# XuyangBai/D3Feat

Measured on AMD Instinct MI355X. Metric: fragments/sec (30k-pt clouds), higher is better.
Workload: dtype f32; 1 GPU; SURVEY §8d config #2: synthetic 3DMatch room fragment, 300k raw pts -> grid subsample 0.03 m (~29k pts per cloud) -> self-pair -> 5-level pyramid -> full KPFCNN forward (random-init weights (reference initialiser, seed 42), 14.1M params)...; points_per_cloud=29369, fragments_per_gpu=2141, parallelism=fragment-dp1, fragments_per_replay=12, engine_fallbacks=0, engine_isolated_replays=0

## Files before the change

### d3feat_amd/_lib.py

```python
import ctypes as C
import os

_HERE = os.path.dirname(os.path.abspath(__file__))
LIB_PATH = os.environ.get("D3FEAT_AMD_LIB") or os.path.join(_HERE, "lib", "libd3feat_amd.so")

D3F_OK = 0
ERRORS = {-1: "HIP runtime / kernel launch failure", -2: "workspace too small", -3: "invalid argument"}
ST_EMPTY_ELEMENT, ST_NEG_CELL, ST_KEY_RANGE, ST_HIT_OVERFLOW, ST_OUT_OVERFLOW, ST_KEY_WIDTH = 1, 2, 4, 8, 16, 32
PAD_NUM_SUPPORTS = -2147483648
NEIGHBOR_CAP = 1024
MAX_BATCH = 255
TOPK_MAX = 8192
PAIRS_KMAX = 1024
REPEAT_COUNTS_MAX = 16
MATCH_KMAX = 8192
VALIDATION_NMAX = 1024
SCENES_MAX = 256
GRID_RESET_MAX = 8
VP_INDEX_RANGE, VP_COUNT_RANGE = 1, 2

_vp, _sz, _i, _f = C.c_void_p, C.c_size_t, C.c_int, C.c_float

SIGNATURES = {
    "d3f_version": (_i, []),
    "d3f_trace_marker": (_i, [_i, _vp]),
    "d3f_pack_status": (_i, [_vp, _vp, _i, _vp, _i, _vp, _i, _vp, _i, _vp, _i, _i, _i, _vp]),
    "d3f_grid_subsample_workspace_bytes": (_sz, [_i, _i, _i, _i]),
    "d3f_batch_grid_subsample": (_i, [_vp, _i, _vp, _i, _f, _vp, _i, _vp, _i, _vp, _vp, _vp, _vp, _vp, _vp, _sz, _vp]),
    "d3f_batch_grid_subsample_async": (_i, [_vp, _i, _vp, _i, _f, _vp, _i, _i, _i, _vp, _vp, _vp, _sz, _vp]),
    "d3f_batch_grid_subsample_async_inplace": (_i, [_vp, _i, _vp, _i, _f, _vp, _i, _i, _vp, _vp, _vp, _sz, _vp]),
    "d3f_stack_self_pair": (_i, [_vp, _i, _vp, _i, _vp, _vp, _vp, _vp]),
    "d3f_radius_neighbors_workspace_bytes": (_sz, [_i, _i, _i]),
    "d3f_batch_radius_neighbors": (_i, [_vp, _i, _vp, _i, _vp, _vp, _i, _f, _vp, _i, _i, _i, _vp, _vp, _sz, _vp]),
    "d3f_neighbor_grid_bytes": (_sz, [_i, _i]),
    "d3f_neighbor_grid_order_offset": (_sz, [_i, _i]),
    "d3f_neighbor_grid_build": (_i, [_vp, _i, _vp, _i, _f, _vp, _sz, _vp]),
    "d3f_neighbor_grid_boxed_form": (_i, [_i, _i]),
    "d3f_geometry_reset": (_i, [_vp, _i, _vp, _vp, _vp, _vp, _i, _vp]),
    "d3f_neighbor_grid_build_boxed": (_i, [_vp, _i, _vp, _i, _f, _vp, _vp, _sz, _vp]),
    "d3f_stack_self_pair_boxed": (_i, [_vp, _i, _vp, _i, _vp, _vp, _vp, _vp, _vp, _vp]),
    "d3f_batch_grid_subsample_async_boxed": (_i, [_vp, _vp, _i, _vp, _i, _f, _vp, _i, _i, _i, _vp, _vp, _vp, _vp, _vp, _sz, _vp]),
    "d3f_neighbor_grid_search": (_i, [_vp, _sz, _i, _vp, _i, _vp, _i, _f, _i, _vp, _i, _i, _i, _i, _i, _f, _i, _vp, _vp]),
    "d3f_neighbor_grid_search_ordered": (_i, [_vp, _sz, _i, _vp, _i, _vp, _i, _f, _vp, _sz, _vp, _i, _i, _i, _i, _i, _f, _i, _vp, _vp]),
    "d3f_neighbor_grid_inv_offset": (_sz, [_i, _i]),
    "d3f_neighbor_grid_xyz_offset": (_sz, [_i, _i]),
    "d3f_row_positive": (_i, [_vp, _i, _i, _i, _vp, _vp, _i, _vp]),
    "d3f_kpconv_aggregate": (_i, [_vp, _i, _vp, _i, _vp, _i, _i, _vp, _i, _i, _vp, _vp, _i, _f, _i, _i, _vp, _vp, _vp, _vp,
                                  _vp, _i, _vp]),
    "d3f_kpconv_deform_aggregate": (_i, [_vp, _i, _vp, _i, _vp, _i, _i, _vp, _i, _i, _vp, _i, _f, _vp, _i, _i, _vp, _i, _f, _i, _i, _vp,
                                         _vp, _vp, _vp, _i, _vp]),
    "d3f_kpconv_fused_c1": (_i, [_vp, _i, _vp, _i, _vp, _i, _i, _vp, _i, _vp, _i, _f, _i, _i, _vp, _i, _vp, _vp, _vp, _i, _i,
                                 _f, _vp, _i, _vp, _vp, _vp, _i, _vp]),
    "d3f_kpconv_fused32": (_i, [_vp, _i, _vp, _i, _vp, _i, _i, _vp, _i, _vp, _vp, _i, _f, _i, _i, _vp, _vp, _vp, _vp, _i, _i, _f, _vp,
                                _i, _vp, _vp, _vp, _i, _vp]),
    "d3f_kpconv_fused_supported": (_i, [_i, _i, _i, _i, _i]),
    "d3f_kpconv_pack_weights": (_i, [_vp, _i, _i, _vp, _vp]),
    "d3f_kpconv_fused": (_i, [_vp, _i, _vp, _i, _vp, _i, _i, _vp, _i, _i, _vp, _vp, _i, _f, _i, _i, _vp, _i, _vp, _vp, _vp, _i, _i,
                              _f, _vp, _i, _vp, _vp, _vp, _i, _vp]),
    "d3f_kpconv_fused32_x3": (_i, [_vp, _i, _vp, _i, _vp, _i, _i, _vp, _i, _vp, _vp, _i, _f, _i, _i, _vp, _vp, _vp, _vp, _i, _i, _f, _vp,
                                   _i, _vp, _vp, _vp, _i, _vp]),
    "d3f_kpconv_packed_x3_bytes": (_sz, [_i, _i]),
    "d3f_kpconv_pack_weights_x3": (_i, [_vp, _i, _i, _vp, _vp]),
    "d3f_kpconv_fused_x3": (_i, [_vp, _i, _vp, _i, _vp, _i, _i, _vp, _i, _i, _vp, _vp, _i, _f, _i, _i, _vp, _i, _vp, _vp, _vp, _i, _i,
                                 _f, _vp, _i, _vp, _vp, _vp, _i, _vp]),
    "d3f_gemm_workspace_bytes": (_sz, [_i, _i, _i, _i]),
    "d3f_gemm_bf16_workspace_bytes": (_sz, [_i, _i, _i, _i]),
    "d3f_gemm_f32": (_i, [_vp, _i, _vp, _i, _vp, _i, _i, _i, _i, _vp, _vp, _vp, _vp, _i, _i, _f, _vp, _sz, _vp, _i, _vp]),
    "d3f_gemm_upsample_cat_f32": (_i, [_vp, _i, _i, _i, _vp, _i, _vp, _i, _i, _vp, _i, _vp, _i, _i, _i, _vp, _vp, _i, _f, _vp, _sz,
                                       _vp, _vp, _i, _vp]),
    "d3f_ind_max_pool": (_i, [_vp, _i, _i, _i, _vp, _i, _i, _i, _vp, _i, _vp, _vp, _vp, _vp, _i, _vp]),
    "d3f_closest_pool_cat": (_i, [_vp, _i, _i, _i, _vp, _i, _i, _vp, _i, _i, _vp, _i, _vp, _vp, _vp]),
    "d3f_affine_act": (_i, [_vp, _i, _i, _i, _vp, _vp, _vp, _i, _i, _f, _vp, _i, _vp, _vp]),
    "d3f_pack_descriptors": (_i, [_vp, _vp, _i, _i, _vp, _i, _vp, _i, _vp, _vp]),
    "d3f_pack_descriptors_to": (_i, [_vp, _vp, _i, _i, _vp, _i, _vp, _i, _vp, _vp, _i, _i, _i, _vp, _vp, _vp]),
    "d3f_topk_workspace_bytes": (_sz, [_i, _i, _i, _i]),
    "d3f_topk_records": (_i, [_vp, _i, _vp, _i, _i, _vp, _i, _i, _vp, _vp, _i, _i, _i, _vp, _i, _i, _vp, _i, _vp, _vp, _vp, _vp, _sz,
                              _vp]),
    "d3f_feature_nn_workspace_bytes": (_sz, [_i]),
    "d3f_feature_nn": (_i, [_vp, _i, _i, _vp, _i, _i, _i, _vp, _vp, _vp, _sz, _vp]),
    "d3f_mutual_matches_workspace_bytes": (_sz, [_i]),
    "d3f_mutual_matches": (_i, [_vp, _i, _vp, _i, _vp, _vp, _vp, _sz, _vp]),
    "d3f_ransac_hypotheses": (_i, [_vp, _i, _vp, _i, _vp, _i, _f, _f, C.c_uint64, C.c_uint64, _i, _vp, _vp, _vp]),
    "d3f_ransac_draw": (_i, [C.c_uint64, C.c_uint64, _i, _i]),
    "d3f_neighbor_grid_score": (_i, [_vp, _sz, _i, _vp, _i, _vp, _i, _f, _vp, _vp, _vp, _vp]),
    "d3f_register_pairs_workspace_bytes": (_sz, [_i, _i, _i, _i]),
    "d3f_register_pairs": (_i, [_vp, _i, _i, _i, _i, _vp, _vp, _i, _i, _f, _i, _f, _f, _i, _i, C.c_uint64, _vp, _f] + [_vp] * 11
                           + [_sz, _vp]),
    "d3f_repeatability_pairs": (_i, [_vp, _i, _i, _i, _vp, _vp, _i, _vp, _i, _vp, _vp, _i, _vp, _vp, _vp]),
    "d3f_match_pairs_workspace_bytes": (_sz, [_i, _vp, _i]),
    "d3f_match_pairs": (_i, [_vp, _i, _i, _i, _i, _vp, _vp, _i, _vp, _f, _vp, _i, _vp, _vp, _vp, _sz, _vp]),
    "d3f_register_pairs_counts_workspace_bytes": (_sz, [_i, _i, _i, _vp, _i, _i]),
    "d3f_register_pairs_counts": (_i, [_vp, _i, _i, _i, _i, _vp, _vp, _i, _vp, _i, _f, _i, _f, _f, _i, _i, C.c_uint64, _vp, _f] + [_vp] * 10
                                  + [_sz, _vp]),
    "d3f_overlap_pairs": (_i, [_vp, _sz, _i, _i, _vp, _i, _f, _vp, _vp, _i, _vp]),
    "d3f_validation_pairs_workspace_bytes": (_sz, [_i, _i]),
    "d3f_validation_pairs": (_i, [_vp, _i, _i, _vp, _i, _vp, _i, _i, _vp, _vp, _vp, _i, _vp, _i, _f, _i, _f, _f, _f, _f] + [_vp] * 5
                             + [_sz, _vp]),
    "d3f_loss_gradients_workspace_bytes": (_sz, [_i, _i, _i]),
    "d3f_loss_gradients": (_i, [_vp, _i, _i, _vp, _i, _vp, _i, _i, _vp, _vp, _vp, _i, _vp, _i, _f, _i, _f, _f, _f, _f, _i, _vp, _i, _vp, _i,
                                _vp, _vp, _vp, _sz, _vp]),
    "d3f_neighbor_transpose_workspace_bytes": (_sz, [_i, _i]),
    "d3f_neighbor_transpose": (_i, [_vp, _i, _i, _i, _vp, _i, _vp, _vp, _vp, _sz, _vp]),
    "d3f_detect_head_backward_workspace_bytes": (_sz, [_i, _i, _i]),
    "d3f_detect_head_backward": (_i, [_vp, _i, _i, _i, _vp, _i, _i, _vp, _vp, _i, _i, _vp, _vp, _vp, _i, _vp, _i, _vp, _i, _vp, _sz, _vp]),
    "d3f_neighbor_transpose_qs": (_i, [_vp, _i, _i, _i, _vp, _i, _vp, _vp, _vp, _vp, _sz, _vp]),
    "d3f_kpconv_backward_workspace_bytes": (_sz, [_i, _i, _i, _i, _i, _i]),
    "d3f_kpconv_backward": (_i, [_vp, _i, _vp, _i, _vp, _i, _i, _vp, _i, _i, _vp, _i, _f, _i, _i, _vp, _vp, _i, _i, _vp, _vp, _vp, _i, _vp,
                                 _vp, _vp, _vp, _i, _vp, _sz, _vp]),
    "d3f_gemm_tn_workspace_bytes": (_sz, [_i, _i, _i]),
    "d3f_gemm_tn_f32": (_i, [_vp, _i, _vp, _i, _i, _i, _i, _vp, _vp, _vp, _sz, _vp]),
    "d3f_batch_norm_workspace_bytes": (_sz, [_i, _i]),
    "d3f_batch_norm_train": (_i, [_vp, _i, _i, _i, _vp, _vp, _f, _f, _vp, _vp, _vp, _i, _i, _f, _vp, _i, _vp, _vp, _vp, _vp, _sz, _vp]),
    "d3f_batch_norm_backward": (_i, [_vp, _i, _vp, _i, _vp, _i, _i, _i, _vp, _vp, _vp, _i, _f, _vp, _i, _vp, _vp, _vp, _i, _vp, _vp, _sz,
                                     _vp]),
    "d3f_pose_errors": (_i, [_vp, _vp, _i, _i, _vp, _vp, _vp, _vp, _vp, _vp]),
    "d3f_sanitize_descriptors": (_i, [_vp, _i, _i, _i, _i, _vp]),
    "d3f_matching_summary": (_i, [_vp, _vp, _vp, _i, _i, _vp, _i, _vp, _vp, _vp, _vp]),
    "d3f_registration_recall": (_i, [_vp, _i, _vp, _vp, _vp, _vp, _vp, _i, _i, _vp, _i, _vp, _vp, _vp, _vp, _vp]),
    "d3f_icp_pairs_workspace_bytes": (_sz, [_i, _i]),
    "d3f_icp_pairs": (_i, [_vp, _sz, _i, _vp, _i, _vp, _i, _vp, _vp, _i, _i] + [_vp] * 9 + [_sz, _vp]),
    "d3f_gemm_pack_bf16": (_i, [_vp, _i, _i, _i, _vp, _vp]),
    "d3f_gemm_pack_f32t": (_i, [_vp, _i, _i, _i, _vp, _vp]),
    "d3f_gemm_f32t": (_i, [_vp, _i, _i, _i, _vp, _i, _vp, _i, _i, _vp, _vp, _i, _i, _i, _vp, _vp, _vp, _vp, _i, _i, _f, _vp, _sz,
                           _vp, _vp, _i, _vp]),
    "d3f_gemm_x3_packed_bytes": (_sz, [_i, _i]),
    "d3f_gemm_pack_x3": (_i, [_vp, _i, _i, _i, _vp, _vp]),
    "d3f_gemm_x3_workspace_bytes": (_sz, [_i, _i, _i, _i]),
    "d3f_gemm_x3_plan": (_i, [_i, _i, _i, _i, _vp, _vp, _vp]),
    "d3f_gemm_x3_resident": (_i, [_i, _i, _i, _i]),
    "d3f_gemm_x3": (_i, [_vp, _i, _i, _i, _vp, _i, _vp, _i, _i, _vp, _vp, _i, _i, _i, _vp, _vp, _vp, _vp, _i, _i, _f, _vp, _sz,
                         _vp, _vp, _i, _vp]),
    "d3f_gemm_x3_gres": (_i, [_vp, _i, _i, _i, _vp, _i, _vp, _i, _i, _vp, _vp, _i, _i, _i, _vp, _vp, _vp, _vp, _i, _vp, _i, _i, _vp, _i, _f,
                              _vp, _sz, _vp, _vp, _i, _vp]),
    "d3f_gemm_bf16": (_i, [_vp, _i, _i, _i, _vp, _i, _vp, _i, _i, _vp, _vp, _i, _i, _i, _vp, _vp, _vp, _vp, _i, _i, _f, _vp, _sz,
                           _vp, _vp, _i, _i, _i, _vp]),
    "d3f_decode_xyz_records": (_i, [_vp, _i, _i, _i, _i, _i, _i, _i, _vp, _vp]),
    "d3f_detect_head": (_i, [_vp, _i, _i, _i, _vp, _i, _i, _vp, _vp, _i, _i, _vp, _i, _vp, _vp, _vp, _vp]),
}

_lib = None


class D3FeatLibraryError(RuntimeError):
    pass


def load():
    global _lib
    if _lib is not None:
        return _lib
    if not os.path.exists(LIB_PATH):
        raise D3FeatLibraryError(
            "d3feat_amd: %s not found -- the HIP extension is the only compute path. Build it with "
            "`python -c 'import __graft_entry__ as g; g.build()'` or `make -C d3feat_amd/csrc`." % LIB_PATH)
    lib = C.CDLL(LIB_PATH)
    for name, (res, args) in SIGNATURES.items():
        fn = getattr(lib, name)
        fn.restype = res
        fn.argtypes = args
    _lib = lib
    return lib


def check(rc, what):
    if rc != D3F_OK:
        raise D3FeatLibraryError("d3feat_amd.%s failed: %s (code %d)" % (what, ERRORS.get(rc, "unknown"), rc))
```

### d3feat_amd/csrc/gemm_f32.hip

```cpp
#include "gemm_common.h"
#include <cstdio>
#include <cstdlib>

#define GM_SA (GM_BK + 1)

template <int WM, int WN>
__global__ void __launch_bounds__(256)
gemm_f32_kernel(const float* __restrict__ A, int lda, const float* __restrict__ B, int ldb, float* __restrict__ C, int ldc,
                int M, int N, int K, int vecA, int vecB, int tiles_per_split, float* __restrict__ slab, GemmEpi E,
                const int* __restrict__ M_dev, GemmGather G) {
    constexpr int BM = 32 * WM, BN = 32 * WN;
    constexpr int A_F4 = BM * GM_BK / 4 / 256;
    constexpr int B_F4 = GM_BK * BN / 4 / 256;
    static_assert(WM * WN == 4 && A_F4 >= 1 && B_F4 >= 1, "tile shape");
    const int Mcap = M;
    M = d3f_dyn(M, M_dev);
    if ((int)(blockIdx.z * BM) >= M) return;
    __shared__ float As[2][BM * GM_SA];
    __shared__ __attribute__((aligned(16))) float Bs[2][GM_BK * BN];

    const int tid = threadIdx.x, lane = tid & 63, wave = tid >> 6;
    const int wm = wave / WN, wn = wave % WN;
    const int m0 = blockIdx.z * BM, n0 = blockIdx.x * BN;
    const int nt_all = (K + GM_BK - 1) / GM_BK;
// ... 352 lines not shown
            if (bn == 32) gemm_fast_kernel<4, 1, EPI><<<grid, 256, lds, stream>>>(A, lda, B, ldb, C, ldc, M, N, K, tps, slab, E, M_dev, G);
            else gemm_fast_kernel<2, 2, EPI><<<grid, 256, lds, stream>>>(A, lda, B, ldb, C, ldc, M, N, K, tps, slab, E, M_dev, G);
        });
    } else if (bn == 32) {
        gemm_f32_kernel<4, 1><<<grid, 256, 0, stream>>>(A, lda, B, ldb, C, ldc, M, N, K, vecA, vecB, tps, slab, E, M_dev, G);
    } else {
        gemm_f32_kernel<2, 2><<<grid, 256, 0, stream>>>(A, lda, B, ldb, C, ldc, M, N, K, vecA, vecB, tps, slab, E, M_dev, G);
    }
    gemm_reduce(slab, S, M, N, C, ldc, E, M_dev, stream);
    D3F_LAUNCH_CHECK();
    return D3F_OK;
}

extern "C" int d3f_gemm_pack_f32t(const float* B, int ldb, int K, int N, float* Wt, void* stream_) {
    hipStream_t stream = (hipStream_t)stream_;
    if (K < 1 || N < 1 || ldb < N || !B || !Wt) return D3F_ERR_ARG;
    const int Kp = (K + GD_BK - 1) / GD_BK * GD_BK;
    gemm_pack_f32t_kernel<<<d3f_cdiv((long long)N * Kp, 256), 256, 0, stream>>>(B, ldb, K, N, Kp, Wt);
    D3F_LAUNCH_CHECK();
    return D3F_OK;
}

extern "C" int d3f_gemm_f32t(const float* A, int N1, int lda, int C1, const int* idx, int ld_idx, const float* skip, int lds, int C2,
                             const float* Wt, float* C, int ldc, int M, int N, const float* row_scale, const float* col_scale,
                             const float* col_shift, const float* residual, int ldr, int leaky, float alpha, void* workspace,
                             size_t workspace_bytes, const int* M_dev, const int* N1_dev, int M_hint, void* stream_) {
    hipStream_t stream = (hipStream_t)stream_;
    const int K = C1 + C2;
    bool empty;
    if (int rc = gemm_check_composite(true, 4, 15, M, N, N1, C1, C2, lda, ldc, lds, ldr, ld_idx, A, Wt, C, idx, skip, residual,
                                      col_scale, col_shift, empty))
        return rc;
    if (empty) return D3F_OK;
    const int Kp = (K + GD_BK - 1) / GD_BK * GD_BK;
    int bm, bn, S, tps;
    gemm_plan(M, N, K, M_hint, bm, bn, S, tps);
    float* slab;
    if (int rc = gemm_slab(S, M, N, workspace, workspace_bytes, slab)) return rc;
    GemmEpi E{row_scale, col_scale, col_shift, residual, ldr, leaky, alpha};
    GemmGather G{idx, ld_idx, N1, N1_dev, C2 > 0 ? skip : nullptr, lds, C1};
    static_assert((size_t)GD_STAGES * (128 + 32) * GD_BK * sizeof(float) <= 65536, "the ring needs an LDS opt-in (d3f_opt_in_lds)");
    const size_t lds_bytes = (size_t)GD_STAGES * (bm + bn) * GD_BK * sizeof(float);
    const long long items_cap = (long long)d3f_cdiv(N, bn) * S * d3f_cdiv(M, bm);
    const long long gsz = (items_cap + 7) / 8 * 8;
    if (gsz > 0x7fffffffll) return D3F_ERR_ARG;
    const dim3 grid((unsigned)gsz, 1, 1);
    gemm_with_epi(E, [&](auto epi) {
        constexpr int EPI = decltype(epi)::value;
        if (bn == 32) gemm_dma_kernel<4, 1, EPI><<<grid, 256, lds_bytes, stream>>>(A, lda, Wt, Kp, C, ldc, M, N, K, tps, S, slab, E, M_dev, G);
        else gemm_dma_kernel<2, 2, EPI><<<grid, 256, lds_bytes, stream>>>(A, lda, Wt, Kp, C, ldc, M, N, K, tps, S, slab, E, M_dev, G);
    });
    gemm_reduce(slab, S, M, N, C, ldc, E, M_dev, stream);
    D3F_LAUNCH_CHECK();
    return D3F_OK;
}

typedef __bf16 gb_bf16x8 __attribute__((ext_vector_type(8)));
#define GB_BK 32
#define GB_LS 40

__device__ __forceinline__ unsigned gb_pack2(float a, float b) { return d3f_bf16_rne(a) | (d3f_bf16_rne(b) << 16); }

__global__ void __launch_bounds__(256) gemm_pack_bf16_kernel(const float* __restrict__ B, int ldb, int K, int N, int Kp,
                                                             unsigned short* __restrict__ Wt) {
    const long long t = (long long)blockIdx.x * blockDim.x + threadIdx.x;
    if (t >= (long long)N * Kp) return;
    const int n = (int)(t / Kp), k = (int)(t % Kp);
    Wt[t] = (unsigned short)(k < K ? d3f_bf16_rne(B[(size_t)k * ldb + n]) : 0u);
}

extern "C" int d3f_gemm_pack_bf16(const float* B, int ldb, int K, int N, void* Wt, void* stream_) {
    hipStream_t stream = (hipStream_t)stream_;
    if (K < 1 || N < 1 || ldb < N || !B || !Wt) return D3F_ERR_ARG;
    const int Kp = (K + GB_BK - 1) / GB_BK * GB_BK;
    gemm_pack_bf16_kernel<<<d3f_cdiv((long long)N * Kp, 256), 256, 0, stream>>>(B, ldb, K, N, Kp, (unsigned short*)Wt);
    D3F_LAUNCH_CHECK();
    return D3F_OK;
}

template <bool ABF, bool CBF>
__global__ void __launch_bounds__(256)
gemm_bf16_kernel(const float* __restrict__ A, int lda, const unsigned short* __restrict__ Wt, int Kp, float* __restrict__ C,
                 int ldc, int M, int N, int K, int tiles_per_split, float* __restrict__ slab, GemmEpi E,
                 const int* __restrict__ M_dev, GemmGather G) {
    constexpr int BM = 64, BN = 64;
    const int Mcap = M;
    M = d3f_dyn(M, M_dev);
    if ((int)(blockIdx.z * BM) >= M) return;
    const unsigned gx_ = gridDim.x, gxy_ = gridDim.x * gridDim.y;
    const unsigned T_ = d3f_xcd_tile(blockIdx.x + gx_ * blockIdx.y + gxy_ * blockIdx.z, gxy_ * (unsigned)((M + BM - 1) / BM));
    const unsigned bz = T_ / gxy_, by = (T_ % gxy_) / gx_, bx = T_ % gx_;
    __shared__ __attribute__((aligned(16))) unsigned short As[2][BM * GB_LS];
    __shared__ __attribute__((aligned(16))) unsigned short Bs[2][BN * GB_LS];
    const int tid = threadIdx.x, lane = tid & 63, wave = tid >> 6;
    const int wm = wave >> 1, wn = wave & 1;
    const int m0 = bz * BM, n0 = bx * BN;
    const int nt_all = Kp / GB_BK;
    const int t_begin = by * tiles_per_split;
    const int t_end = min(nt_all, t_begin + tiles_per_split);
    int srow[2];
    {
        const int n1 = d3f_dyn(G.N1, G.N1_dev);
#pragma unroll
        for (int i = 0; i < 2; ++i) {
            const int gm = m0 + ((tid + i * 256) >> 3);
            int sr = gm < M ? gm : -1;
            if (G.gidx && sr >= 0) {
                sr = G.gidx[(size_t)gm * G.ld_gidx];
                if (sr < 0 || sr >= n1) sr = -1;
            }
            srow[i] = sr;
        }
    }
    const int brow = n0 + (tid >> 2);
    float4 ra[2];
    uint2 rh[2];
    uint4 rb;
    const unsigned short* Ah = (const unsigned short*)A;
    const unsigned short* A2h = (const unsigned short*)G.A2;
    auto load_tile = [&](int t) {
        const int k0 = t * GB_BK;
#pragma unroll
        for (int i = 0; i < 2; ++i) {
            const int e = tid + i * 256;
            const int gm = m0 + (e >> 3), k = k0 + ((e & 7) << 2);
            if (ABF) {
                uint2 v = make_uint2(0u, 0u);
                if (gm < M && k < K) {
                    if (G.A2 && k >= G.K1) v = *(const uint2*)(A2h + (size_t)gm * G.lda2 + (k - G.K1));
                    else if (srow[i] >= 0) v = *(const uint2*)(Ah + (size_t)srow[i] * lda + k);
                }
                rh[i] = v;
            } else {
                float4 v = make_float4(0.f, 0.f, 0.f, 0.f);
                if (gm < M && k < K) {
                    if (G.A2 && k >= G.K1) v = *(const float4*)(G.A2 + (size_t)gm * G.lda2 + (k - G.K1));
                    else if (srow[i] >= 0) v = *(const float4*)(A + (size_t)srow[i] * lda + k);
                }
                ra[i] = v;
            }
        }
        rb = (brow < N) ? *(const uint4*)(Wt + (size_t)brow * Kp + k0 + ((tid & 3) << 3)) : make_uint4(0u, 0u, 0u, 0u);
    };
    auto store_tile = [&](int buf) {
#pragma unroll
        for (int i = 0; i < 2; ++i) {
            const int e = tid + i * 256;
            const uint2 p = ABF ? rh[i] : make_uint2(gb_pack2(ra[i].x, ra[i].y), gb_pack2(ra[i].z, ra[i].w));
            *(uint2*)&As[buf][(e >> 3) * GB_LS + ((e & 7) << 2)] = p;
        }
        *(uint4*)&Bs[buf][(tid >> 2) * GB_LS + ((tid & 3) << 3)] = rb;
    };
    f32x16 acc;
#pragma unroll
    for (int r = 0; r < 16; ++r) acc[r] = 0.f;
    if (t_begin < t_end) {
        load_tile(t_begin);
        store_tile(0);
        __syncthreads();
        for (int t = t_begin; t < t_end; ++t) {
            const int buf = (t - t_begin) & 1;
            if (t + 1 < t_end) load_tile(t + 1);
            const unsigned short* ap = &As[buf][(32 * wm + (lane & 31)) * GB_LS + ((lane >> 5) << 3)];
            const unsigned short* bp = &Bs[buf][(32 * wn + (lane & 31)) * GB_LS + ((lane >> 5) << 3)];
            const uint4 a0 = *(const uint4*)ap, a1 = *(const uint4*)(ap + 16);
            const uint4 b0 = *(const uint4*)bp, b1 = *(const uint4*)(bp + 16);
            acc = __builtin_amdgcn_mfma_f32_32x32x16_bf16(__builtin_bit_cast(gb_bf16x8, a0), __builtin_bit_cast(gb_bf16x8, b0), acc, 0, 0, 0);
            acc = __builtin_amdgcn_mfma_f32_32x32x16_bf16(__builtin_bit_cast(gb_bf16x8, a1), __builtin_bit_cast(gb_bf16x8, b1), acc, 0, 0, 0);
            if (t + 1 < t_end) store_tile(buf ^ 1);
            __syncthreads();
        }
    }
    const int gn = n0 + 32 * wn + (lane & 31);
    if (gn >= N) return;
    float cs = 1.f, ch = 0.f;
    if (!slab) { cs = E.col_scale ? E.col_scale[gn] : 1.f; ch = E.col_shift ? E.col_shift[gn] : 0.f; }
#pragma unroll
    for (int r = 0; r < 16; ++r) {
        const int gm = m0 + 32 * wm + (r & 3) + 8 * (r >> 2) + 4 * (lane >> 5);
        if (gm >= M) continue;
        if (slab) { slab[((size_t)by * Mcap + gm) * N + gn] = acc[r]; continue; }
        float v = acc[r];
        if (E.row_scale) v *= E.row_scale[gm];
        v = v * cs + ch;
        if (E.residual)
            v += ABF ? d3f_bf16_f32(((const unsigned short*)E.residual)[(size_t)gm * E.ldr + gn]) : E.residual[(size_t)gm * E.ldr + gn];
        if (E.leaky) v = v > 0.f ? v : v * E.alpha;
        if (CBF) ((unsigned short*)C)[(size_t)gm * ldc + gn] = (unsigned short)d3f_bf16_rne(v);
        else C[(size_t)gm * ldc + gn] = v;
    }
}

static void gemm_bf16_split(int M, int N, int K, int M_hint, int& S, int& tps) {
    int bm, bn;
    gemm_plan(M, N > 32 ? N : 64, K, M_hint, bm, bn, S, tps);
    const int nt = ((K + GB_BK - 1) / GB_BK * GB_BK) / GB_BK;
    if (S > nt) S = nt;
    tps = d3f_cdiv(nt, S);
    S = d3f_cdiv(nt, tps);
}

extern "C" size_t d3f_gemm_bf16_workspace_bytes(int M, int N, int K, int M_hint) {
    if (M <= 0 || N <= 0 || K <= 0) return 256;
    int S, tps;
    gemm_bf16_split(M, N, K, M_hint, S, tps);
    return gemm_slab_bytes(S, M, N);
}

extern "C" int d3f_gemm_bf16(const void* A_, int N1, int lda, int C1, const int* idx, int ld_idx, const void* skip_, int lds,
                             int C2, const void* Wt, void* C_, int ldc, int M, int N, const float* row_scale,
                             const float* col_scale, const float* col_shift, const void* residual_, int ldr, int leaky,
                             float alpha, void* workspace, size_t workspace_bytes, const int* M_dev, const int* N1_dev,
                             int M_hint, int a_bf16, int c_bf16, void* stream_) {
    hipStream_t stream = (hipStream_t)stream_;
    const float* A = (const float*)A_;
    const float* skip = (const float*)skip_;
    const float* residual = (const float*)residual_;
    float* C = (float*)C_;
    const int K = C1 + C2;
    bool empty;
    if (int rc = gemm_check_composite(false, 4, a_bf16 ? 7 : 15, M, N, N1, C1, C2, lda, ldc, lds, ldr, ld_idx, A, Wt, C, idx, skip,
                                      residual, col_scale, col_shift, empty))
        return rc;
    if (empty) return D3F_OK;
    const int Kp = (K + GB_BK - 1) / GB_BK * GB_BK;
    int S, tps;
    gemm_bf16_split(M, N, K, M_hint, S, tps);
    float* slab;
    if (int rc = gemm_slab(S, M, N, workspace, workspace_bytes, slab)) return rc;
    if (d3f_cdiv(M, 64) > 65535) return D3F_ERR_ARG;
    GemmEpi E{row_scale, col_scale, col_shift, residual, ldr, leaky, alpha};
    GemmGather G{idx, ld_idx, N1, N1_dev, C2 > 0 ? skip : nullptr, lds, C1};
    dim3 grid(d3f_cdiv(N, 64), S, d3f_cdiv(M, 64));
#define D3F_GB(ABF_, CBF_) gemm_bf16_kernel<ABF_, CBF_><<<grid, 256, 0, stream>>>(A, lda, (const unsigned short*)Wt, Kp, C, ldc, M, N, K, tps, slab, E, M_dev, G)
    if (a_bf16) { if (c_bf16) D3F_GB(true, true); else D3F_GB(true, false); }
    else { if (c_bf16) D3F_GB(false, true); else D3F_GB(false, false); }
#undef D3F_GB
    gemm_reduce(slab, S, M, N, C, ldc, E, M_dev, stream, a_bf16, c_bf16);
    D3F_LAUNCH_CHECK();
    return D3F_OK;
}

#include "gemm_x3.h"

struct GemmX3Plan { int tn, waves, S, tps; };
static long long gemm_x3_cost(long long blocks, long long slots, int nt, int per_tile_x100, int& S) {
    long long best = -1;
    S = 1;
    for (int s = 1; s <= 64 && s * 4 <= nt; ++s) {
        const int t = d3f_cdiv(nt, s);
        if (d3f_cdiv(nt, t) != s) continue;
        const long long rounds = (blocks * s + slots - 1) / slots;
        const long long cost = rounds * (t + 12) * per_tile_x100 + (s > 1 ? 200ll * s : 0);
        if (best < 0 || cost < best) { best = cost; S = s; }
    }
    if (best < 0) best = ((blocks + slots - 1) / slots) * (nt + 12) * per_tile_x100;
    return best;
}
static GemmX3Plan gemm_x3_plan(int M, int N, int K, int M_hint) {
    if (M_hint > 0 && M_hint < M) M = M_hint;
    const int nt = K / GX_BK;
    GemmX3Plan p;
#ifdef D3F_GEMM_TUNING
    static const char* forced = getenv("D3F_X3_PLAN");
    if (forced) {
        int tn = 0, wv = 0, S = 0;
        if (sscanf(forced, "%d,%d,%d", &tn, &wv, &S) == 3 && ((tn == 1 && wv == 4) || (tn == 2 && wv == 4) || (tn == 4 && wv == 8)) && S >= 1 &&
            !(N <= 32 && tn != 1) && S * 4 <= (nt > 4 ? nt : 4)) {
            p.tn = tn; p.waves = wv; p.S = S < nt ? S : nt;
            p.tps = d3f_cdiv(nt, p.S);
            p.S = d3f_cdiv(nt, p.tps);
            return p;
        }
    }
#endif
    p.tn = N <= 32 ? 1 : 2;
    p.waves = 4;
    const long long c_small = gemm_x3_cost((long long)d3f_cdiv(M, 128) * d3f_cdiv(N, 32 * p.tn), 512, nt, 100, p.S);
    if (N >= 128) {
        int s_big;
        const long long c_big = gemm_x3_cost((long long)d3f_cdiv(M, 256) * d3f_cdiv(N, 128), 256, nt, 163, s_big);
        if (c_big < c_small) { p.tn = 4; p.waves = 8; p.S = s_big; }
    }
    p.tps = d3f_cdiv(nt, p.S);
    p.S = d3f_cdiv(nt, p.tps);
    return p;
}

extern "C" size_t d3f_gemm_x3_packed_bytes(int K, int N) {
    if (K < 1 || N < 1) return 0;
    return (size_t)d3f_cdiv(N, 32) * d3f_cdiv(K, GX_BK) * GX_CHUNK * sizeof(unsigned short);
}

extern "C" int d3f_gemm_pack_x3(const float* B, int ldb, int K, int N, void* Wx, void* stream_) {
    hipStream_t stream = (hipStream_t)stream_;
    if (K < 1 || N < 1 || ldb < N || !B || !Wx || ((uintptr_t)Wx & 15)) return D3F_ERR_ARG;
    const int nkt = d3f_cdiv(K, GX_BK);
    const long long total = (long long)d3f_cdiv(N, 32) * nkt * GX_CHUNK;
    gemm_pack_x3_kernel<<<d3f_cdiv(total, 256), 256, 0, stream>>>(B, ldb, K, N, nkt, total, (unsigned short*)Wx);
    D3F_LAUNCH_CHECK();
    return D3F_OK;
}

extern "C" int d3f_gemm_x3_plan(int M, int N, int K, int M_hint, int* rows, int* cols, int* slices) {
    if (M <= 0 || N <= 0 || K < GX_BK || (K % GX_BK)) return D3F_ERR_ARG;
    const GemmX3Plan p = gemm_x3_plan(M, N, K, M_hint);
    if (rows) *rows = 32 * p.waves;
    if (cols) *cols = 32 * p.tn;
    if (slices) *slices = p.S;
    return D3F_OK;
}

extern "C" size_t d3f_gemm_x3_workspace_bytes(int M, int N, int K, int M_hint) {
    if (M <= 0 || N <= 0 || K < GX_BK) return 256;
    const GemmX3Plan p = gemm_x3_plan(M, N, K, M_hint);
    return gemm_slab_bytes(p.S, M, N);
}

static size_t gemm_x3r_lds_bytes(int nkt, int NG) {
    return (size_t)nkt * NG * GX_CHUNK * sizeof(unsigned short) + GXR_PATCH_BYTES + GXR_EPI_BYTES;
}

extern "C" int d3f_gemm_x3_resident(int M, int N, int K, int M_hint) {
    if (N < 1 || K < GX_BK || (K % GX_BK)) return 0;
    const int NG = d3f_cdiv(N, 32), m_eff = (M_hint > 0 && M_hint < M) ? M_hint : M;
    return (NG == 1 || NG == 2 || NG == 4) && gemm_x3r_lds_bytes(K / GX_BK, NG) <= 160 * 1024 && m_eff >= 65536;
}

static int gemm_x3_run(const float* A, int N1, int lda, int C1, const int* idx, int ld_idx, const float* skip, int lds, int C2,
                       const void* Wx, float* C, int ldc, int M, int N, const float* row_scale, const float* col_scale,
                       const float* col_shift, const float* residual, int ldr, const int* res_idx, int ld_res_idx, int res_rows,
                       const int* res_rows_dev, int leaky, float alpha, void* workspace, size_t workspace_bytes, const int* M_dev,
                       const int* N1_dev, int M_hint, void* stream_) {
    hipStream_t stream = (hipStream_t)stream_;
    const int K = C1 + C2;
    bool empty;
    if (int rc = gemm_check_composite(true, GX_BK, 15, M, N, N1, C1, C2, lda, ldc, lds, ldr, ld_idx, A, Wx, C, idx, skip, residual,
                                      col_scale, col_shift, empty))
        return rc;
    if (res_idx && (ld_res_idx < 1 || res_rows < 0)) return D3F_ERR_ARG;
    if (empty) return D3F_OK;
    if (res_idx && !residual) return D3F_ERR_ARG;
    GemmEpi E{row_scale, col_scale, col_shift, residual, ldr, leaky, alpha, res_idx, ld_res_idx, res_rows, res_rows_dev};
    GemmGather G{idx, ld_idx, N1, N1_dev, C2 > 0 ? skip : nullptr, lds, C1};
    const int nkt = K / GX_BK, NG = d3f_cdiv(N, 32);
    if (!res_idx && d3f_gemm_x3_resident(M, N, K, M_hint)) {
        static std::atomic<int> cus_of[64];
        int dev = 0;
        if (hipGetDevice(&dev) != hipSuccess) return D3F_ERR_HIP;
        int cus = cus_of[dev & 63].load(std::memory_order_relaxed);
        if (!cus) {
            hipDeviceProp_t pr;
            if (hipGetDeviceProperties(&pr, dev) != hipSuccess) return D3F_ERR_HIP;
            cus = pr.multiProcessorCount > 0 ? pr.multiProcessorCount : 256;
            cus_of[dev & 63].store(cus, std::memory_order_relaxed);
        }
        static std::atomic<unsigned long long> lds_done{0};
        const void* const fns[3] = {(const void*)gemm_x3r_kernel<1>, (const void*)gemm_x3r_kernel<2>, (const void*)gemm_x3r_kernel<4>};
        if (d3f_opt_in_lds(lds_done, fns, 160 * 1024) != D3F_OK) return D3F_ERR_HIP;
        const int grid = std::min(cus, d3f_cdiv(d3f_cdiv(M, 32), 8));
#define D3F_GXR(TN_) gemm_x3r_kernel<TN_><<<grid, 512, gemm_x3r_lds_bytes(nkt, NG), stream>>>(A, lda, (const unsigned short*)Wx, nkt, C, ldc, M, N, E, M_dev, G)
        if (NG == 4) D3F_GXR(4);
        else if (NG == 2) D3F_GXR(2);
        else D3F_GXR(1);
#undef D3F_GXR
        D3F_LAUNCH_CHECK();
        return D3F_OK;
    }
    const GemmX3Plan pl = gemm_x3_plan(M, N, K, M_hint);
    const int S = pl.S, tps = pl.tps, bm = 32 * pl.waves;
    float* slab;
    if (int rc = gemm_slab(S, M, N, workspace, workspace_bytes, slab)) return rc;
    if (d3f_cdiv(M, bm) > 65535) return D3F_ERR_ARG;
    dim3 grid(d3f_cdiv(N, 32 * pl.tn), S, d3f_cdiv(M, bm));
#define D3F_GX(TN_, WV_) gemm_x3_kernel<TN_, WV_><<<grid, 64 * WV_, 0, stream>>>(A, lda, (const unsigned short*)Wx, nkt, NG, C, ldc, M, N, tps, slab, E, M_dev, G)
    if (pl.waves == 8) D3F_GX(4, 8);
    else if (pl.tn == 1) D3F_GX(1, 4);
    else D3F_GX(2, 4);
#undef D3F_GX
    gemm_reduce(slab, S, M, N, C, ldc, E, M_dev, stream);
    D3F_LAUNCH_CHECK();
    return D3F_OK;
}

extern "C" int d3f_gemm_x3(const float* A, int N1, int lda, int C1, const int* idx, int ld_idx, const float* skip, int lds, int C2,
                           const void* Wx, float* C, int ldc, int M, int N, const float* row_scale, const float* col_scale,
                           const float* col_shift, const float* residual, int ldr, int leaky, float alpha, void* workspace,
                           size_t workspace_bytes, const int* M_dev, const int* N1_dev, int M_hint, void* stream_) {
    return gemm_x3_run(A, N1, lda, C1, idx, ld_idx, skip, lds, C2, Wx, C, ldc, M, N, row_scale, col_scale, col_shift, residual, ldr,
                       nullptr, 0, 0, nullptr, leaky, alpha, workspace, workspace_bytes, M_dev, N1_dev, M_hint, stream_);
}

extern "C" int d3f_gemm_x3_gres(const float* A, int N1, int lda, int C1, const int* idx, int ld_idx, const float* skip, int lds, int C2,
                                const void* Wx, float* C, int ldc, int M, int N, const float* row_scale, const float* col_scale,
                                const float* col_shift, const float* residual, int ldr, const int* res_idx, int ld_res_idx,
                                int res_rows, const int* res_rows_dev, int leaky, float alpha, void* workspace, size_t workspace_bytes,
                                const int* M_dev, const int* N1_dev, int M_hint, void* stream_) {
    return gemm_x3_run(A, N1, lda, C1, idx, ld_idx, skip, lds, C2, Wx, C, ldc, M, N, row_scale, col_scale, col_shift, residual, ldr,
                       res_idx, ld_res_idx, res_rows, res_rows_dev, leaky, alpha, workspace, workspace_bytes, M_dev, N1_dev, M_hint,
                       stream_);
}
```

### d3feat_amd/csrc/gemm_x3.h

```cpp
#pragma once
#include "gemm_common.h"

#define GX_BK 32
#define GX_LS 40
#define GX_CHUNK (3 * 32 * GX_LS)

__device__ __forceinline__ unsigned gx_cvt_pk(float lo, float hi) {
    unsigned r;
    asm("v_cvt_pk_bf16_f32 %0, %1, %2" : "=v"(r) : "v"(lo), "v"(hi));
    return r;
}

typedef float gx_f4 __attribute__((ext_vector_type(4)));
__device__ __forceinline__ void gx_ld16(gx_f4& r, const void* p) { asm volatile("global_load_dwordx4 %0, %1, off" : "=v"(r) : "v"(p) : "memory"); }
template <int OFF> __device__ __forceinline__ void gx_ld16o(gx_f4& r, const void* p) {
    asm volatile("global_load_dwordx4 %0, %1, off offset:%2" : "=v"(r) : "v"(p), "n"(OFF) : "memory");
}

__device__ __forceinline__ float gx_sub(float a, float b) {
    float r;
    asm("v_sub_f32 %0, %1, %2" : "=v"(r) : "v"(a), "v"(b));
    return r;
}
__device__ __forceinline__ void gx_split8(const gx_f4& x0, const gx_f4& x1, uint4 (&pl)[3]) {
    const float v[8] = {x0[0], x0[1], x0[2], x0[3], x1[0], x1[1], x1[2], x1[3]};
    unsigned p[3][4];
#pragma unroll
    for (int i = 0; i < 4; ++i) {
        float a = v[2 * i], b = v[2 * i + 1];
        p[0][i] = gx_cvt_pk(a, b);
        a = gx_sub(a, __uint_as_float(p[0][i] << 16));
        b = gx_sub(b, __uint_as_float(p[0][i] & 0xffff0000u));
        p[1][i] = gx_cvt_pk(a, b);
        a = gx_sub(a, __uint_as_float(p[1][i] << 16));
        b = gx_sub(b, __uint_as_float(p[1][i] & 0xffff0000u));
        p[2][i] = gx_cvt_pk(a, b);
    }
#pragma unroll
    for (int s = 0; s < 3; ++s) pl[s] = make_uint4(p[s][0], p[s][1], p[s][2], p[s][3]);
}

__global__ void __launch_bounds__(256) gemm_pack_x3_kernel(const float* __restrict__ B, int ldb, int K, int N, int nkt, long long total,
                                                           unsigned short* __restrict__ Wx) {
    const long long t = (long long)blockIdx.x * blockDim.x + threadIdx.x;
    if (t >= total) return;
    const int kk = (int)(t % GX_LS);
    long long q = t / GX_LS;
    const int r = (int)(q % 32); q /= 32;
    const int p = (int)(q % 3); q /= 3;
    const int kt = (int)(q % nkt);
    const int ng = (int)(q / nkt);
    const int k = kt * GX_BK + kk, n = ng * 32 + r;
    unsigned out = 0u;
    if (kk < GX_BK && k < K && n < N) {
        float w = B[(size_t)k * ldb + n];
        unsigned h = d3f_bf16_rne(w);
        if (p > 0) { w -= __uint_as_float(h << 16); h = d3f_bf16_rne(w); }
        if (p > 1) { w -= __uint_as_float(h << 16); h = d3f_bf16_rne(w); }
        out = h;
    }
    Wx[t] = (unsigned short)out;
}

template <int NB, int STRIDE>
__device__ __forceinline__ void gx_dma_round(const void* sbase, unsigned dst, const unsigned (&vo)[4]) {
    unsigned keep;
    if constexpr (NB == 2)
        asm volatile("s_mov_b32 %0, m0\n\ts_mov_b32 m0, %2\n\ts_nop 0\n\tglobal_load_lds_dwordx4 %3, %1\n\t"
                     "s_add_u32 m0, m0, %5\n\ts_nop 0\n\tglobal_load_lds_dwordx4 %4, %1\n\ts_mov_b32 m0, %0"
                     : "=&s"(keep) : "s"(sbase), "s"(dst), "v"(vo[0]), "v"(vo[1]), "n"(STRIDE) : "memory", "scc");
    else if constexpr (NB == 4)
        asm volatile("s_mov_b32 %0, m0\n\ts_mov_b32 m0, %2\n\ts_nop 0\n\tglobal_load_lds_dwordx4 %3, %1\n\t"
                     "s_add_u32 m0, m0, %7\n\ts_nop 0\n\tglobal_load_lds_dwordx4 %4, %1\n\t"
                     "s_add_u32 m0, m0, %7\n\ts_nop 0\n\tglobal_load_lds_dwordx4 %5, %1\n\t"
                     "s_add_u32 m0, m0, %7\n\ts_nop 0\n\tglobal_load_lds_dwordx4 %6, %1\n\ts_mov_b32 m0, %0"
                     : "=&s"(keep) : "s"(sbase), "s"(dst), "v"(vo[0]), "v"(vo[1]), "v"(vo[2]), "v"(vo[3]), "n"(STRIDE) : "memory", "scc");
    else static_assert(NB < 0, "add the round");
}

template <int TN, int WAVES>
__global__ void __launch_bounds__(64 * WAVES) __attribute__((amdgpu_waves_per_eu(2, 2)))
gemm_x3_kernel(const float* __restrict__ A, int lda, const unsigned short* __restrict__ Wx, int nkt, int NG, float* __restrict__ C,
               int ldc, int M, int N, int tiles_per_split, float* __restrict__ slab, GemmEpi E, const int* __restrict__ M_dev,
               GemmGather G) {
    constexpr int BM = 32 * WAVES, BN = 32 * TN, NTH = 64 * WAVES;
    constexpr int NB = (480 * TN + NTH - 1) / NTH;
    constexpr int SB = NB * NTH * 16;
    constexpr int WAITN = 4 + NB;
    static_assert((TN == 1 || TN == 2 || TN == 4) && (WAVES == 4 || WAVES == 8), "tile shape");
    const int Mcap = M;
    M = d3f_dyn(M, M_dev);
    if ((int)(blockIdx.z * BM) >= M) return;
    const unsigned gx_ = gridDim.x, gxy_ = gridDim.x * gridDim.y;
    const unsigned T_ = d3f_xcd_tile(blockIdx.x + gx_ * blockIdx.y + gxy_ * blockIdx.z, gxy_ * (unsigned)((M + BM - 1) / BM));
    const unsigned bz = T_ / gxy_, by = (T_ % gxy_) / gx_, bx = T_ % gx_;
    __shared__ __attribute__((aligned(16))) unsigned char Bs[3 * SB];
    const int tid = threadIdx.x, lane = tid & 63, wave = tid >> 6;
    const int m0 = bz * BM, n0 = bx * BN;
    const int t_begin = by * tiles_per_split;
    const int t_end = min(nkt, t_begin + tiles_per_split);
    const int t_last = t_end - 1;

    const int gm_a = m0 + 32 * wave + (lane & 31);
    const float* arow = gd_zero_line;
    const float* a2row = gd_zero_line;
    unsigned amask = 0u, a2mask = 0u;
    if (gm_a < M) {
        int sr = gm_a;
        if (G.gidx) {
            const int n1 = d3f_dyn(G.N1, G.N1_dev);
            sr = G.gidx[(size_t)gm_a * G.ld_gidx];
            if (sr < 0 || sr >= n1) sr = -1;
        }
        if (sr >= 0) { arow = A + (size_t)sr * lda; amask = 0xffffffffu; }
        if (G.A2) { a2row = G.A2 + (size_t)gm_a * G.lda2; a2mask = 0xffffffffu; }
    }
    const int kofs = (lane >> 5) << 3;
    const int K1 = G.K1;
    const float* pa;
    unsigned astep;
    int treq = t_begin;
    auto a_rebase = [&](int t) {
        const bool first = t * GX_BK < K1;
        const unsigned msk = first ? amask : a2mask;
        pa = (first ? arow : a2row) + ((unsigned)((first ? t * GX_BK : t * GX_BK - K1) + kofs) & msk);
        astep = (unsigned)GX_BK & msk;
    };
    a_rebase(t_begin);

    unsigned wofs[4];
#pragma unroll
    for (int i = 0; i < 4; ++i) {
        const int e = tid + NTH * (i < NB ? i : 0);
        const int c = e / 480, o = e - 480 * c;
        const int ng = min((int)bx * TN + c, NG - 1);
        wofs[i] = (unsigned)ng * (unsigned)nkt * (unsigned)(GX_CHUNK * 2) + (unsigned)o * 16u;
    }
    const unsigned lds_wave = (unsigned)__builtin_amdgcn_readfirstlane(
        (int)((unsigned)(unsigned long long)(gd_lptr)Bs + (unsigned)wave * 1024u));

    gx_f4 rA0, rA1, rA2, rA3, rB0, rB1, rB2, rB3, rC0, rC1, rC2, rC3;
    uint4 ap0[2][3], ap1[2][3];
    auto request_w = [&](int t, int slot) {
        gx_dma_round<NB, WAVES * 1024>((const char*)Wx + (size_t)t * (GX_CHUNK * 2), lds_wave + (unsigned)slot * (unsigned)SB, wofs);
    };
    auto request_a = [&](gx_f4& r0, gx_f4& r1, gx_f4& r2, gx_f4& r3) {
        gx_ld16(r0, pa);
        gx_ld16o<16>(r1, pa);
        gx_ld16o<64>(r2, pa);
        gx_ld16o<80>(r3, pa);
        if (treq < t_last) {
            ++treq;
            if (treq * GX_BK == K1) a_rebase(treq);
            else pa += astep;
        }
    };

    f32x16 acc[TN];
#pragma unroll
    for (int j = 0; j < TN; ++j)
#pragma unroll
        for (int r = 0; r < 16; ++r) acc[j][r] = 0.f;

    auto tile = [&](int slot, const uint4 (&cur)[2][3], uint4 (&nxt)[2][3], const gx_f4& r0, const gx_f4& r1, const gx_f4& r2,
                    const gx_f4& r3) {
        const unsigned short* bp = (const unsigned short*)(Bs + slot * SB) + (lane & 31) * GX_LS + kofs;
        constexpr int NM = 12 * TN, NOPS = 88;
        constexpr int PA[2][6] = {{2, 1, 0, 1, 0, 0}, {0, 1, 0, 2, 1, 0}}, PB[2][6] = {{0, 1, 2, 0, 1, 0}, {2, 1, 1, 0, 0, 0}};
        uint4 b[TN][3];
#pragma unroll
        for (int j = 0; j < TN; ++j)
#pragma unroll
            for (int p = 0; p < 3; ++p) b[j][p] = *(const uint4*)(bp + j * GX_CHUNK + p * (32 * GX_LS));
        float x[16] = {r0[0], r0[1], r0[2], r0[3], r1[0], r1[1], r1[2], r1[3], r2[0], r2[1], r2[2], r2[3], r3[0], r3[1], r3[2], r3[3]};
        float hl[16];
        unsigned P[3][8];
        __builtin_amdgcn_sched_barrier(0);
#pragma unroll
        for (int m = 0; m < NM; ++m) {
            const int s = m / (6 * TN), prod = (m % (6 * TN)) / TN, j = m % TN;
            acc[j] = __builtin_amdgcn_mfma_f32_32x32x16_bf16(__builtin_bit_cast(gb_bf16x8, b[j][PB[s][prod]]),
                                                             __builtin_bit_cast(gb_bf16x8, cur[s][PA[s][prod]]), acc[j], 0, 0, 0);
            if (s == 0 && (prod == 2 || prod >= 4)) {
                const int p = prod == 2 ? 2 : prod == 4 ? 1 : 0;
                b[j][p] = *(const uint4*)(bp + j * GX_CHUNK + p * (32 * GX_LS) + 16);
            }
#pragma unroll
            for (int k = m * NOPS / NM; k < (m + 1) * NOPS / NM; ++k) {
                const int lvl = k < 8 ? 0 : k < 24 ? 1 : k < 40 ? 2 : k < 48 ? 3 : k < 64 ? 4 : k < 80 ? 5 : 6;
                if (lvl == 0) P[0][k] = gx_cvt_pk(x[2 * k], x[2 * k + 1]);
                else if (lvl == 3) P[1][k - 40] = gx_cvt_pk(x[2 * (k - 40)], x[2 * (k - 40) + 1]);
                else if (lvl == 6) P[2][k - 80] = gx_cvt_pk(x[2 * (k - 80)], x[2 * (k - 80) + 1]);
                else if (lvl == 1 || lvl == 4) {
                    const int e = k - (lvl == 1 ? 8 : 48);
                    const unsigned pk = P[lvl == 1 ? 0 : 1][e >> 1];
                    hl[e] = __uint_as_float((e & 1) ? (pk & 0xffff0000u) : (pk << 16));
                } else {
                    const int e = k - (lvl == 2 ? 24 : 64);
                    x[e] = gx_sub(x[e], hl[e]);
                }
            }
            __builtin_amdgcn_sched_barrier(0);
        }
#pragma unroll
        for (int s = 0; s < 2; ++s)
#pragma unroll
            for (int p = 0; p < 3; ++p) nxt[s][p] = make_uint4(P[p][4 * s], P[p][4 * s + 1], P[p][4 * s + 2], P[p][4 * s + 3]);
    };
    auto landed = [&](gx_f4& r0, gx_f4& r1, gx_f4& r2, gx_f4& r3) {
        if constexpr (WAITN == 6) asm volatile("s_waitcnt vmcnt(6)" : "+v"(r0), "+v"(r1), "+v"(r2), "+v"(r3) : : "memory");
        else asm volatile("s_waitcnt vmcnt(8)" : "+v"(r0), "+v"(r1), "+v"(r2), "+v"(r3) : : "memory");
        static_assert(WAITN == 6 || WAITN == 8, "wait count");
    };

    if (t_begin < t_end) {
        int wslot = 0, cslot = 0;
        auto next = [&](int sl) { return sl + 1 == 3 ? 0 : sl + 1; };
        request_w(t_begin, wslot); wslot = next(wslot);
        request_a(rA0, rA1, rA2, rA3);
        request_a(rB0, rB1, rB2, rB3);
        request_w(min(t_begin + 1, t_last), wslot); wslot = next(wslot);
        request_a(rC0, rC1, rC2, rC3);
        if constexpr (NB == 2) asm volatile("s_waitcnt vmcnt(10)" : "+v"(rA0), "+v"(rA1), "+v"(rA2), "+v"(rA3) : : "memory");
        else asm volatile("s_waitcnt vmcnt(12)" : "+v"(rA0), "+v"(rA1), "+v"(rA2), "+v"(rA3) : : "memory");
        gx_split8(rA0, rA1, ap0[0]);
        gx_split8(rA2, rA3, ap0[1]);
#define GX_STEP(I_, CUR_, NXT_, C0_, C1_, C2_, C3_, Q0_, Q1_, Q2_, Q3_)                                                          \
        if (t + I_ < t_end) {                                                                                                  \
            landed(C0_, C1_, C2_, C3_);                                                                                        \
            __syncthreads();                                                                                                   \
            request_w(min(t + I_ + 2, t_last), wslot); wslot = next(wslot);                                                    \
            request_a(Q0_, Q1_, Q2_, Q3_);                                                                                     \
            tile(cslot, CUR_, NXT_, C0_, C1_, C2_, C3_); cslot = next(cslot);                                                  \
        }
        for (int t = t_begin; t < t_end; t += 6) {
            GX_STEP(0, ap0, ap1, rB0, rB1, rB2, rB3, rA0, rA1, rA2, rA3)
            GX_STEP(1, ap1, ap0, rC0, rC1, rC2, rC3, rB0, rB1, rB2, rB3)
            GX_STEP(2, ap0, ap1, rA0, rA1, rA2, rA3, rC0, rC1, rC2, rC3)
            GX_STEP(3, ap1, ap0, rB0, rB1, rB2, rB3, rA0, rA1, rA2, rA3)
            GX_STEP(4, ap0, ap1, rC0, rC1, rC2, rC3, rB0, rB1, rB2, rB3)
            GX_STEP(5, ap1, ap0, rA0, rA1, rA2, rA3, rC0, rC1, rC2, rC3)
        }
#undef GX_STEP
        asm volatile("s_waitcnt vmcnt(0)" : "+v"(rA0), "+v"(rA1), "+v"(rA2), "+v"(rA3), "+v"(rB0), "+v"(rB1), "+v"(rB2), "+v"(rB3), "+v"(rC0),
                     "+v"(rC1), "+v"(rC2), "+v"(rC3) : : "memory");
    }
    __syncthreads();

    const bool mok = gm_a < M;
    float rs = 1.f;
    if (!slab && E.row_scale && mok) rs = E.row_scale[gm_a];
    float* dst = slab ? slab + ((size_t)by * Mcap + (mok ? gm_a : 0)) * N : C + (size_t)(mok ? gm_a : 0) * ldc;
    const float* rrow = (!slab && E.residual && mok) ? gemm_residual_row(E, gm_a) : nullptr;
    static_assert(3 * SB >= WAVES * 32 * 36 * 4, "the output patches must fit the ring");
    float* patch = (float*)Bs + wave * (32 * 36);
#pragma unroll
    for (int j = 0; j < TN; ++j) {
        if (!slab) {
#pragma unroll
            for (int q = 0; q < 4; ++q) {
                const int gn = n0 + 32 * j + 8 * q + 4 * (lane >> 5);
                float v[4] = {acc[j][4 * q], acc[j][4 * q + 1], acc[j][4 * q + 2], acc[j][4 * q + 3]};
                if (mok && gn < N) {
                    const float4 c4 = E.col_scale ? *(const float4*)&E.col_scale[gn] : make_float4(1.f, 1.f, 1.f, 1.f);
                    const float4 h4 = E.col_shift ? *(const float4*)&E.col_shift[gn] : make_float4(0.f, 0.f, 0.f, 0.f);
                    const float4 r4 = rrow ? *(const float4*)&rrow[gn] : make_float4(0.f, 0.f, 0.f, 0.f);
                    const float c[4] = {c4.x, c4.y, c4.z, c4.w}, h[4] = {h4.x, h4.y, h4.z, h4.w}, rr[4] = {r4.x, r4.y, r4.z, r4.w};
#pragma unroll
                    for (int e = 0; e < 4; ++e) {
                        float t = (v[e] * rs) * c[e] + h[e];
                        t += rr[e];
                        v[e] = (E.leaky && !(t > 0.f)) ? t * E.alpha : t;
                    }
                }
                *(float4*)&patch[(lane & 31) * 36 + 8 * q + 4 * (lane >> 5)] = make_float4(v[0], v[1], v[2], v[3]);
            }
            __builtin_amdgcn_fence(__ATOMIC_RELEASE, "wavefront");
            __builtin_amdgcn_wave_barrier();
            const int cc = n0 + 32 * j + 4 * (lane & 7);
#pragma unroll
            for (int i = 0; i < 4; ++i) {
                const int r = (lane >> 3) + 8 * i;
                const float4 o = *(const float4*)&patch[r * 36 + 4 * (lane & 7)];
                const int gm = m0 + 32 * wave + r;
                if (gm < M && cc < N) *(float4*)&C[(size_t)gm * ldc + cc] = o;
            }
            __builtin_amdgcn_fence(__ATOMIC_ACQUIRE, "wavefront");
            __builtin_amdgcn_wave_barrier();
            continue;
        }
#pragma unroll
        for (int q = 0; q < 4; ++q) {
            const int gn = n0 + 32 * j + 8 * q + 4 * (lane >> 5);
            if (!mok || gn >= N) continue;
            float v[4] = {acc[j][4 * q], acc[j][4 * q + 1], acc[j][4 * q + 2], acc[j][4 * q + 3]};
            if (!slab) {
                const float4 c4 = E.col_scale ? *(const float4*)&E.col_scale[gn] : make_float4(1.f, 1.f, 1.f, 1.f);
                const float4 h4 = E.col_shift ? *(const float4*)&E.col_shift[gn] : make_float4(0.f, 0.f, 0.f, 0.f);
                const float4 r4 = rrow ? *(const float4*)&rrow[gn] : make_float4(0.f, 0.f, 0.f, 0.f);
                const float c[4] = {c4.x, c4.y, c4.z, c4.w}, h[4] = {h4.x, h4.y, h4.z, h4.w}, rr[4] = {r4.x, r4.y, r4.z, r4.w};
#pragma unroll
                for (int e = 0; e < 4; ++e) {
                    float t = (v[e] * rs) * c[e] + h[e];
                    t += rr[e];
                    v[e] = (E.leaky && !(t > 0.f)) ? t * E.alpha : t;
                }
            }
            *(float4*)&dst[gn] = make_float4(v[0], v[1], v[2], v[3]);
        }
    }
}

#define GXR_PS 36
#define GXR_PATCH_BYTES (8 * 32 * GXR_PS * 4)
#define GXR_EPI_BYTES (2 * 128 * 4)
template <int TN>
__global__ void __launch_bounds__(512) __attribute__((amdgpu_waves_per_eu(2, 2)))
gemm_x3r_kernel(const float* __restrict__ A, int lda, const unsigned short* __restrict__ Wx, int nkt, float* __restrict__ C, int ldc,
                int M, int N, GemmEpi E, const int* __restrict__ M_dev, GemmGather G) {
    extern __shared__ __attribute__((aligned(16))) unsigned char gxr_w[];
    static_assert(TN == 1 || TN == 2 || TN == 4, "column groups per row tile");
    M = d3f_dyn(M, M_dev);
    const int tid = threadIdx.x, lane = tid & 63, wave = tid >> 6;
    {
        const int total = nkt * TN * 480;
        const uint4* src = (const uint4*)Wx;
        uint4* dst = (uint4*)gxr_w;
        for (int e = tid; e < total; e += 512) {
            const int c = e / 480, o = e - 480 * c;
            const int kt = c / TN, j = c - kt * TN;
            dst[e] = src[(size_t)(j * nkt + kt) * 480 + o];
        }
        float* ep = (float*)(gxr_w + (size_t)nkt * TN * (GX_CHUNK * 2) + GXR_PATCH_BYTES);
        for (int c = tid; c < 32 * TN; c += 512) {
            ep[c] = (E.col_scale && c < N) ? E.col_scale[c] : 1.f;
            ep[32 * TN + c] = (E.col_shift && c < N) ? E.col_shift[c] : 0.f;
        }
    }
    __syncthreads();
    const float* ep_scale = (const float*)(gxr_w + (size_t)nkt * TN * (GX_CHUNK * 2) + GXR_PATCH_BYTES);
    const float* ep_shift = ep_scale + 32 * TN;
    const int ntiles = (M + 31) >> 5;
    auto kofs_now = [&]() -> int {
        unsigned l;
        asm volatile("v_mbcnt_lo_u32_b32 %0, -1, 0\n\tv_mbcnt_hi_u32_b32 %0, -1, %0" : "=v"(l));
        return (int)((l >> 5) << 3);
    };
    const int K1 = G.K1;
    const int n1 = G.gidx ? d3f_dyn(G.N1, G.N1_dev) : 0;
    const int tstride = 8 * (int)gridDim.x;
    const int rt0 = wave * (int)gridDim.x + (int)blockIdx.x;
    if (rt0 >= ntiles) return;
    const int ntl = (ntiles - rt0 + tstride - 1) / tstride;
    const int total = ntl * nkt;
    int rq_tile = rt0, rq_kt = 0;
    const float* arow;
    const float* a2row;
    unsigned amask, a2mask;
    const float* pa;
    unsigned astep;
    auto a_rebase = [&](int t) {
        const bool first = t * GX_BK < K1;
        const unsigned msk = first ? amask : a2mask;
        pa = (first ? arow : a2row) + ((unsigned)((first ? t * GX_BK : t * GX_BK - K1) + kofs_now()) & msk);
        astep = (unsigned)GX_BK & msk;
    };
    auto rq_rows = [&](int rt) {
        const int gm = rt * 32 + (lane & 31);
        arow = gd_zero_line; a2row = gd_zero_line; amask = 0u; a2mask = 0u;
        if (rt < ntiles && gm < M) {
            int sr = gm;
            if (G.gidx) {
                sr = G.gidx[(size_t)gm * G.ld_gidx];
                if (sr < 0 || sr >= n1) sr = -1;
            }
            if (sr >= 0) { arow = A + (size_t)sr * lda; amask = 0xffffffffu; }
            if (G.A2) { a2row = G.A2 + (size_t)gm * G.lda2; a2mask = 0xffffffffu; }
        }
        a_rebase(0);
    };
    rq_rows(rq_tile);
    gx_f4 rA0, rA1, rA2, rA3, rB0, rB1, rB2, rB3, rC0, rC1, rC2, rC3;
    uint4 ap0[2][3], ap1[2][3];
    auto request_a = [&](gx_f4& r0, gx_f4& r1, gx_f4& r2, gx_f4& r3) {
        gx_ld16(r0, pa);
        gx_ld16o<16>(r1, pa);
        gx_ld16o<64>(r2, pa);
        gx_ld16o<80>(r3, pa);
        if (++rq_kt == nkt) {
            rq_kt = 0;
            rq_tile += tstride;
            rq_rows(rq_tile);
        } else if (rq_kt * GX_BK == K1) a_rebase(rq_kt);
        else pa += astep;
    };
    f32x16 acc[TN];
#pragma unroll
    for (int j = 0; j < TN; ++j)
#pragma unroll
        for (int r = 0; r < 16; ++r) acc[j][r] = 0.f;
    auto tile = [&](int kt, const uint4 (&cur)[2][3], uint4 (&nxt)[2][3], const gx_f4& r0, const gx_f4& r1, const gx_f4& r2,
                    const gx_f4& r3) {
        const unsigned short* bp = (const unsigned short*)gxr_w + (size_t)kt * (TN * GX_CHUNK) + (lane & 31) * GX_LS + kofs_now();
        constexpr int NM = 12 * TN, NOPS = 88;
        constexpr int PA[2][6] = {{2, 1, 0, 1, 0, 0}, {0, 1, 0, 2, 1, 0}}, PB[2][6] = {{0, 1, 2, 0, 1, 0}, {2, 1, 1, 0, 0, 0}};
        uint4 b[TN][3];
#pragma unroll
        for (int j = 0; j < TN; ++j)
#pragma unroll
            for (int p = 0; p < 3; ++p) b[j][p] = *(const uint4*)(bp + j * GX_CHUNK + p * (32 * GX_LS));
        float x[16] = {r0[0], r0[1], r0[2], r0[3], r1[0], r1[1], r1[2], r1[3], r2[0], r2[1], r2[2], r2[3], r3[0], r3[1], r3[2], r3[3]};
        float hl[16];
        unsigned P[3][8];
        __builtin_amdgcn_sched_barrier(0);
#pragma unroll
        for (int m = 0; m < NM; ++m) {
            const int s = m / (6 * TN), prod = (m % (6 * TN)) / TN, j = m % TN;
            acc[j] = __builtin_amdgcn_mfma_f32_32x32x16_bf16(__builtin_bit_cast(gb_bf16x8, b[j][PB[s][prod]]),
                                                             __builtin_bit_cast(gb_bf16x8, cur[s][PA[s][prod]]), acc[j], 0, 0, 0);
            if (s == 0 && (prod == 2 || prod >= 4)) {
                const int p = prod == 2 ? 2 : prod == 4 ? 1 : 0;
                b[j][p] = *(const uint4*)(bp + j * GX_CHUNK + p * (32 * GX_LS) + 16);
            }
#pragma unroll
            for (int k = m * NOPS / NM; k < (m + 1) * NOPS / NM; ++k) {
                const int lvl = k < 8 ? 0 : k < 24 ? 1 : k < 40 ? 2 : k < 48 ? 3 : k < 64 ? 4 : k < 80 ? 5 : 6;
                if (lvl == 0) P[0][k] = gx_cvt_pk(x[2 * k], x[2 * k + 1]);
                else if (lvl == 3) P[1][k - 40] = gx_cvt_pk(x[2 * (k - 40)], x[2 * (k - 40) + 1]);
                else if (lvl == 6) P[2][k - 80] = gx_cvt_pk(x[2 * (k - 80)], x[2 * (k - 80) + 1]);
                else if (lvl == 1 || lvl == 4) {
                    const int e = k - (lvl == 1 ? 8 : 48);
                    const unsigned pk = P[lvl == 1 ? 0 : 1][e >> 1];
                    hl[e] = __uint_as_float((e & 1) ? (pk & 0xffff0000u) : (pk << 16));
                } else {
                    const int e = k - (lvl == 2 ? 24 : 64);
                    x[e] = gx_sub(x[e], hl[e]);
                }
            }
            __builtin_amdgcn_sched_barrier(0);
        }
#pragma unroll
        for (int s = 0; s < 2; ++s)
#pragma unroll
            for (int p = 0; p < 3; ++p) nxt[s][p] = make_uint4(P[p][4 * s], P[p][4 * s + 1], P[p][4 * s + 2], P[p][4 * s + 3]);
    };
    int c_tile = rt0, c_kt = 0;
    float* patch = (float*)(gxr_w + (size_t)nkt * TN * (GX_CHUNK * 2)) + wave * (32 * GXR_PS);
    auto finish_tile = [&]() {
        const int gm_a = c_tile * 32 + (lane & 31);
        const bool mok = gm_a < M;
        float rs = 1.f;
        if (E.row_scale && mok) rs = E.row_scale[gm_a];
#pragma unroll
        for (int j = 0; j < TN; ++j) {
#pragma unroll
            for (int q = 0; q < 4; ++q) {
                const int gn = 32 * j + 8 * q + 4 * (lane >> 5);
                float v[4] = {acc[j][4 * q], acc[j][4 * q + 1], acc[j][4 * q + 2], acc[j][4 * q + 3]};
                if (mok && gn < N) {
                    const float4 c4 = *(const float4*)&ep_scale[gn];
                    const float4 h4 = *(const float4*)&ep_shift[gn];
                    const float4 r4 = E.residual ? *(const float4*)&E.residual[(size_t)gm_a * E.ldr + gn] : make_float4(0.f, 0.f, 0.f, 0.f);
                    const float c[4] = {c4.x, c4.y, c4.z, c4.w}, h[4] = {h4.x, h4.y, h4.z, h4.w}, rr[4] = {r4.x, r4.y, r4.z, r4.w};
#pragma unroll
                    for (int e = 0; e < 4; ++e) {
                        float tt = (v[e] * rs) * c[e] + h[e];
                        tt += rr[e];
                        v[e] = (E.leaky && !(tt > 0.f)) ? tt * E.alpha : tt;
                    }
                }
                *(float4*)&patch[(lane & 31) * GXR_PS + 8 * q + 4 * (lane >> 5)] = make_float4(v[0], v[1], v[2], v[3]);
                acc[j][4 * q] = acc[j][4 * q + 1] = acc[j][4 * q + 2] = acc[j][4 * q + 3] = 0.f;
            }
            __builtin_amdgcn_fence(__ATOMIC_RELEASE, "wavefront");
            __builtin_amdgcn_wave_barrier();
            const int cc = 32 * j + 4 * (lane & 7);
#pragma unroll
            for (int i = 0; i < 4; ++i) {
                const int r = (lane >> 3) + 8 * i;
                const float4 o = *(const float4*)&patch[r * GXR_PS + 4 * (lane & 7)];
                const int gm = c_tile * 32 + r;
                if (gm < M && cc < N) *(float4*)&C[(size_t)gm * ldc + cc] = o;
            }
            __builtin_amdgcn_fence(__ATOMIC_ACQUIRE, "wavefront");
            __builtin_amdgcn_wave_barrier();
        }
        c_tile += tstride;
    };
    auto landed = [&](gx_f4& r0, gx_f4& r1, gx_f4& r2, gx_f4& r3) {
        asm volatile("s_waitcnt vmcnt(4)" : "+v"(r0), "+v"(r1), "+v"(r2), "+v"(r3) : : "memory");
    };
    request_a(rA0, rA1, rA2, rA3);
    request_a(rB0, rB1, rB2, rB3);
    request_a(rC0, rC1, rC2, rC3);
    asm volatile("s_waitcnt vmcnt(8)" : "+v"(rA0), "+v"(rA1), "+v"(rA2), "+v"(rA3) : : "memory");
    gx_split8(rA0, rA1, ap0[0]);
    gx_split8(rA2, rA3, ap0[1]);
#define GXR_STEP(I_, CUR_, NXT_, C0_, C1_, C2_, C3_, Q0_, Q1_, Q2_, Q3_)                                                         \
    if (it + I_ < total) {                                                                                                     \
        landed(C0_, C1_, C2_, C3_);                                                                                            \
        request_a(Q0_, Q1_, Q2_, Q3_);                                                                                         \
        tile(c_kt, CUR_, NXT_, C0_, C1_, C2_, C3_);                                                                            \
        if (++c_kt == nkt) { c_kt = 0; finish_tile(); }                                                                        \
    }
    for (int it = 0; it < total; it += 6) {
        GXR_STEP(0, ap0, ap1, rB0, rB1, rB2, rB3, rA0, rA1, rA2, rA3)
        GXR_STEP(1, ap1, ap0, rC0, rC1, rC2, rC3, rB0, rB1, rB2, rB3)
        GXR_STEP(2, ap0, ap1, rA0, rA1, rA2, rA3, rC0, rC1, rC2, rC3)
        GXR_STEP(3, ap1, ap0, rB0, rB1, rB2, rB3, rA0, rA1, rA2, rA3)
        GXR_STEP(4, ap0, ap1, rC0, rC1, rC2, rC3, rB0, rB1, rB2, rB3)
        GXR_STEP(5, ap1, ap0, rA0, rA1, rA2, rA3, rC0, rC1, rC2, rC3)
    }
#undef GXR_STEP
    asm volatile("s_waitcnt vmcnt(0)" : "+v"(rA0), "+v"(rA1), "+v"(rA2), "+v"(rA3), "+v"(rB0), "+v"(rB1), "+v"(rB2), "+v"(rB3), "+v"(rC0),
                 "+v"(rC1), "+v"(rC2), "+v"(rC3) : : "memory");
}
```

### d3feat_amd/models/network_blocks.py

```python
import contextlib

import numpy as np
import torch

from .. import ops
from ..kernels import convolution_ops as conv_ops
from ..kernels.autograd import batch_norm_trainable, kpconv_trainable, unary_trainable
from ..kernels.kernel_points import create_kernel_points

_STORE = None


@contextlib.contextmanager
def use_variables(store):
    global _STORE
    prev, _STORE = _STORE, store
    try:
        yield store
    finally:
        _STORE = prev


def _vs():
    if _STORE is None:
        raise RuntimeError('no VariableStore active: wrap the call in network_blocks.use_variables(store)')
    return _STORE


def variable_scope(name):
    return _vs().variable_scope(name)



def weight_variable(shape):
    vs = _vs()
    return vs.tensor(vs.weight_variable(shape))


def ind_max_pool(x, inds):
    return ops.ind_max_pool(x, inds)


def closest_pool(x, inds):
    return ops.closest_pool_cat(x, inds)


def _bn(channels, use_batch_norm=True):
    vs = _vs()
    if use_batch_norm:
        return vs.folded_bn(vs.batch_norm_variables(channels))
    return None, vs.tensor(vs.offset_variable(channels))


def _bn_train(x, use_batch_norm, momentum, leaky=False, residual=None):
    vs = _vs()
    channels = int(x.shape[1])
    if not use_batch_norm:
        return batch_norm_trainable(x, None, vs.parameter(vs.offset_variable(channels)), residual, leaky, 0.2)
    gamma, beta, mean, var = vs.batch_norm_variables(channels)
    return batch_norm_trainable(x, vs.parameter(gamma), vs.parameter(beta), residual, leaky, 0.2, vs.tensor(mean), vs.tensor(var),
                                momentum, 1e-6)


def batch_norm(x, use_batch_norm=True, momentum=0.99, training=False):
    if training:
        _check_trainable(x, 'batch_norm')
        return _bn_train(x, use_batch_norm, momentum)
    scale, shift = _bn(int(x.shape[1]), use_batch_norm)
    return ops.affine_act(x, scale, shift)


def leaky_relu(features, alpha=0.2):
    return ops.affine_act(features, leaky=True, alpha=alpha)


def _epilogue(channels, config, leaky, residual=None):
    scale, shift = _bn(channels, config.use_batch_norm)
    return dict(col_scale=scale, col_shift=shift, residual=residual, leaky=leaky, alpha=0.2)


def _kernel_points(config, extent):
    vs = _vs()
    k = config.num_kernel_points

    def init():
        pts = create_kernel_points(1.5 * extent, k, num_kernels=1, dimension=3, fixed=config.fixed_kernel_points,
                                   rng=vs.rng)
        return pts.reshape((k, 3))
    name = vs.get('kernel_points', (k, 3), init)
    return vs.values[name]


def KPConv(query_points, support_points, neighbors_indices, features, K_values, radius, config, epilogue=None):
    extent = config.KP_extent * radius / config.density_parameter
    K_points = _kernel_points(config, extent)
    return conv_ops.KPConv(query_points, support_points, neighbors_indices, features, K_values,
                           fixed=config.fixed_kernel_points, KP_extent=extent, KP_influence=config.KP_influence,
                           aggregation_mode=config.convolution_mode, K_points=K_points,
                           epilogue=epilogue() if callable(epilogue) else epilogue)


def KPConv_deformable(query_points, support_points, neighbors_indices, features, K_values, radius, config, epilogue=None):
    extent = config.KP_extent * radius / config.density_parameter
    K_points = _kernel_points(config, extent)
    vs = _vs()
    k, cin = int(K_values.shape[0]), int(K_values.shape[1])
    offset_dim = (4 if config.modulated else 3) * k
    w0 = vs.tensor(vs.get('offset_conv_weights', (k, cin, offset_dim), lambda: np.zeros((k, cin, offset_dim))))
    b0 = vs.tensor(vs.get('offset_conv_bias', (offset_dim,), lambda: np.zeros(offset_dim)))
    epilogue = epilogue() if callable(epilogue) else epilogue
    return conv_ops.KPConv_deformable(query_points, support_points, neighbors_indices, features, K_values,
                                      fixed=config.fixed_kernel_points, KP_extent=extent, KP_influence=config.KP_influence,
                                      aggregation_mode=config.convolution_mode, modulated=config.modulated, K_points=K_points,
                                      offset_weights=w0, offset_bias=b0, epilogue=epilogue)


def _check_inference(training, what):
    if training:
        raise NotImplementedError('training=True: %s' % what)


def _check_trainable(features, block):
    if isinstance(features, ops.UpsampleCat):
        raise NotImplementedError('training=True: %s on a pending nearest-upsample concatenation needs the backward of the nearest '
                                  'upsampling, which is not built' % block)
    if ops.BF16_FEATURES or features.dtype != torch.float32:
        raise NotImplementedError('training=True: %s under bf16 feature storage: the trainable operators take float32 rows only' % block)



def last_unary_block(layer_ind, inputs, features, radius, fdim, config, training):
    w = weight_variable([int(features.shape[1]), 32])
    with ops.f32_output():
        return conv_ops.unary_convolution(features, w)


def unary_block(layer_ind, inputs, features, radius, fdim, config, training):
    if training:
        _check_trainable(features, 'unary_block')
        vs = _vs()
        w = vs.parameter(vs.weight_variable([int(features.shape[1]), fdim]))
        return _bn_train(unary_trainable(features, w), config.use_batch_norm, config.batch_norm_momentum, leaky=True)
    if isinstance(features, ops.UpsampleCat):
        vs = _vs()
        w = vs.weight_variable([int(features.shape[1]), fdim])
        if ops.upsample_split_ok(features, fdim):
            if config.use_batch_norm:
                w1, w2, shift = vs.split_decoder(w, vs.batch_norm_variables(fdim), int(features.x.shape[1]))
            else:
                (w1, w2, _), shift = vs.split_decoder(w, None, int(features.x.shape[1])), _bn(fdim, False)[1]
            return ops.gemm_upsample_split(features, w1, w2, col_shift=shift, leaky=True, alpha=0.2)
        e = _epilogue(fdim, config, True)
        return ops.gemm_upsample_cat(features, vs.tensor(w), col_scale=e['col_scale'], col_shift=e['col_shift'], leaky=True, alpha=0.2)
    w = weight_variable([int(features.shape[1]), fdim])
    return conv_ops.unary_convolution(features, w, epilogue=_epilogue(fdim, config, True))


def simple_block(layer_ind, inputs, features, radius, fdim, config, training):
    if training:
        _check_trainable(features, 'simple_block')
        vs = _vs()
        w = vs.parameter(vs.weight_variable([config.num_kernel_points, int(features.shape[1]), fdim]))
        pts = inputs['points'][layer_ind]
        x = _kpconv_train(pts, pts, inputs['neighbors'][layer_ind], features, w, radius, config)
        return _bn_train(x, config.use_batch_norm, config.batch_norm_momentum, leaky=True)
    w = weight_variable([config.num_kernel_points, int(features.shape[1]), fdim])
    return KPConv(inputs['points'][layer_ind], inputs['points'][layer_ind], inputs['neighbors'][layer_ind], features, w,
                  radius, config, epilogue=lambda: _epilogue(fdim, config, True))


def _kpconv_train(query_points, support_points, neighbors_indices, features, K_values, radius, config):
    extent = config.KP_extent * radius / config.density_parameter
    K_points = _kernel_points(config, extent)
    return kpconv_trainable(query_points, support_points, neighbors_indices, features, K_points, K_values, extent, config.KP_influence,
                            config.convolution_mode)


def _resnetb_train(layer_ind, inputs, features, radius, fdim, config):
    _check_trainable(features, 'resnetb_block')
    vs = _vs()
    bn, momentum = config.use_batch_norm, config.batch_norm_momentum
    cin = int(features.shape[1])
    with variable_scope('conv1'):
        w = vs.parameter(vs.weight_variable([cin, fdim // 2]))
        x = _bn_train(unary_trainable(features, w), bn, momentum, leaky=True)
    with variable_scope('conv2'):
        w = vs.parameter(vs.weight_variable([config.num_kernel_points, fdim // 2, fdim // 2]))
        pts = inputs['points'][layer_ind]
        x = _bn_train(_kpconv_train(pts, pts, inputs['neighbors'][layer_ind], x, w, radius, config), bn, momentum, leaky=True)
    with variable_scope('conv3'):
        w3 = vs.parameter(vs.weight_variable([fdim // 2, 2 * fdim]))
        if bn:
            vs.batch_norm_variables(2 * fdim)
        else:
            vs.offset_variable(2 * fdim)
    shortcut = features
    if cin != 2 * fdim:
        with variable_scope('shortcut'):
            w = vs.parameter(vs.weight_variable([cin, 2 * fdim]))
            shortcut = _bn_train(unary_trainable(features, w), bn, momentum)
    with variable_scope('conv3'):
        return _bn_train(unary_trainable(x, w3), bn, momentum, leaky=True, residual=shortcut)


def _resnetb(layer_ind, inputs, features, radius, fdim, config, strided, deformable=False):
    cin = int(features.shape[1])
    with variable_scope('conv1'):
        w = weight_variable([cin, fdim // 2])
        x = conv_ops.unary_convolution(features, w, epilogue=_epilogue(fdim // 2, config, True))
    with variable_scope('conv2'):
        w = weight_variable([config.num_kernel_points, fdim // 2, fdim // 2])
        if strided:
            q, s, nb = inputs['points'][layer_ind + 1], inputs['points'][layer_ind], inputs['pools'][layer_ind]
        else:
            q, s, nb = inputs['points'][layer_ind], inputs['points'][layer_ind], inputs['neighbors'][layer_ind]
        x = (KPConv_deformable if deformable else KPConv)(q, s, nb, x, w, radius, config,
                                                          epilogue=lambda: _epilogue(fdim // 2, config, True))
    with variable_scope('conv3'):
        vs = _vs()
        w3 = vs.weight_variable([fdim // 2, 2 * fdim])
        bn3 = None
        if config.use_batch_norm:
            bn3 = vs.batch_norm_variables(2 * fdim)
        else:
            vs.offset_variable(2 * fdim)
    with variable_scope('shortcut'):
        shortcut = ind_max_pool(features, inputs['pools'][layer_ind]) if strided else features
        need_sc = int(shortcut.shape[1]) != 2 * fdim
        fuse = need_sc and config.use_batch_norm and (fdim // 2) % 4 == 0
        sc_w = sc_bn = None
        if need_sc:
            vs = _vs()
            sc_w = vs.weight_variable([int(shortcut.shape[1]), 2 * fdim])
            if fuse:
                sc_bn = vs.batch_norm_variables(2 * fdim)
            else:
                shortcut = conv_ops.unary_convolution(shortcut, vs.tensor(sc_w), epilogue=_epilogue(2 * fdim, config, False))
    with variable_scope('conv3'):
        vs = _vs()
        if fuse:
            W, shift = vs.stacked_branches(w3, bn3, sc_w, sc_bn)
            return ops.gemm_cat2(x, shortcut, W, col_shift=shift, leaky=True, alpha=0.2)
        return conv_ops.unary_convolution(x, vs.tensor(w3), epilogue=_epilogue(2 * fdim, config, True, residual=shortcut))


def resnetb_block(layer_ind, inputs, features, radius, fdim, config, training):
    if training:
        return _resnetb_train(layer_ind, inputs, features, radius, fdim, config)
    return _resnetb(layer_ind, inputs, features, radius, fdim, config, False)


def resnetb_strided_block(layer_ind, inputs, features, radius, fdim, config, training):
    _check_inference(training, 'resnetb_strided_block needs the backward of the max pooling of its shortcut, which is not built')
    return _resnetb(layer_ind, inputs, features, radius, fdim, config, True)


def resnetb_deformable_block(layer_ind, inputs, features, radius, fdim, config, training):
    _check_inference(training, 'resnetb_deformable_block needs the backward of the deformable KPConv, which is not built')
    return _resnetb(layer_ind, inputs, features, radius, fdim, config, False, deformable=True)


def resnetb_deformable_strided_block(layer_ind, inputs, features, radius, fdim, config, training):
    _check_inference(training, 'resnetb_deformable_strided_block needs the backward of the deformable KPConv and of the max pooling, '
                     'which are not built')
    return _resnetb(layer_ind, inputs, features, radius, fdim, config, True, deformable=True)


def nearest_upsample_block(layer_ind, inputs, features, radius, fdim, config, training):
    with variable_scope('nearest_upsample'):
        return closest_pool(features, inputs['upsamples'][layer_ind - 1])


def _materialized(block_fn):
    def wrapped(layer_ind, inputs, features, radius, fdim, config, training):
        if isinstance(features, ops.UpsampleCat):
            features = features.materialize()
        return block_fn(layer_ind, inputs, features, radius, fdim, config, training)
    wrapped.__name__ = block_fn.__name__
    wrapped.__doc__ = block_fn.__doc__
    return wrapped


def get_block_ops(block_name):
    table = {'unary': unary_block, 'last_unary': last_unary_block, 'simple': simple_block, 'resnetb': resnetb_block,
             'resnetb_strided': resnetb_strided_block, 'resnetb_deformable': resnetb_deformable_block,
             'resnetb_deformable_strided': resnetb_deformable_strided_block, 'nearest_upsample': nearest_upsample_block}
    if block_name in table:
        return table[block_name] if block_name == 'unary' else _materialized(table[block_name])
    known_unsupported = ('simple_strided', 'resnet', 'resnetb_light', 'inception_deformable',
                         'resnetb_light_strided', 'inception_deformable_strided', 'vgg',
                         'max_pool', 'max_pool_wide', 'global_average', 'simple_upsample', 'resnetb_upsample')
    if block_name in known_unsupported:
        raise NotImplementedError('block "%s" is not used by any released D3Feat model and is not implemented'
                                  % block_name)
    raise ValueError('Unknown block name in the architecture definition : ' + block_name)


def assemble_CNN_blocks(inputs, config, dropout_prob):
    r = config.first_subsampling_dl * config.density_parameter
    layer = 0
    fdim = config.first_features_dim
    features = inputs['features']
    F = []
    training = dropout_prob < 0.99
    block_in_layer = 0
    for block in config.architecture:
        if any(tmp in block for tmp in ('pool', 'strided', 'upsample', 'global')):
            F += [features]
        if 'upsample' in block:
            break
        with variable_scope('layer_{:d}/{:s}_{:d}'.format(layer, block.replace('_deformable', ''), block_in_layer)):
            features = get_block_ops(block)(layer, inputs, features, r, fdim, config, training)
        block_in_layer += 1
        if 'pool' in block or 'strided' in block:
            layer += 1
            r *= 2
            fdim *= 2
            block_in_layer = 0
        if 'global' in block:
            F += [features]
    return F
```

### d3feat_amd/ops.py

```python
import ctypes

import os

import numpy as np
import torch

from . import _lib

_WS = {}

PROFILE = None


class _timed:
    def __init__(self, name, info, device):
        self.on = PROFILE is not None
        self.name, self.info, self.device = name, info, device

    def __enter__(self):
        if self.on:
            self.start = torch.cuda.Event(enable_timing=True)
            self.end = torch.cuda.Event(enable_timing=True)
            self.start.record(torch.cuda.current_stream(self.device))
        return self
# ... 420 lines not shown
        global BF16_CONTRACTION, BF16_FEATURES
        self.prev, BF16_CONTRACTION = BF16_CONTRACTION, self.on
        self.prevf, BF16_FEATURES = BF16_FEATURES, self.features
        return self

    def __exit__(self, *exc):
        global BF16_CONTRACTION, BF16_FEATURES
        BF16_CONTRACTION, BF16_FEATURES = self.prev, self.prevf
        return False


class f32_output:

    def __enter__(self):
        global F32_OUTPUT
        self.prev, F32_OUTPUT = F32_OUTPUT, True
        return self

    def __exit__(self, *exc):
        global F32_OUTPUT
        F32_OUTPUT = self.prev
        return False


def _feat(t, name, ndim=None):
    if isinstance(t, torch.Tensor) and t.dtype == torch.bfloat16:
        return _req(t, torch.bfloat16, name, ndim)
    return _req(t, torch.float32, name, ndim)


def _h(t):
    return 1 if (t is not None and t.dtype == torch.bfloat16) else 0


def _out_dtype():
    return torch.bfloat16 if (BF16_CONTRACTION and BF16_FEATURES and not F32_OUTPUT) else torch.float32


def _packed_on_tensor(W, slot, make):
    base = W._base if W._base is not None else W
    store = getattr(base, slot, None)
    if store is None:
        store = {}
        setattr(base, slot, store)
    key = (W.storage_offset(), tuple(W.shape), tuple(W.stride()))
    hit = store.get(key)
    if hit is None:
        hit = store[key] = [base._version, make(None)]
    elif hit[0] != base._version:
        make(hit[1])
        hit[0] = base._version
    return hit[1]


def refresh_packed_weights(tensors):
    n = 0
    for t in tensors:
        if not isinstance(t, torch.Tensor):
            continue
        base = t._base if t._base is not None else t
        for slot, fn in _PACKERS:
            for (off, shape, strides), hit in list((getattr(base, slot, None) or {}).items()):
                if hit[0] != base._version:
                    fn(base.as_strided(shape, strides, off))
                    n += 1
    return n


def _packed_weights(W, slot, alloc, pack, what):
    def make(t):
        K, N = W.shape
        if t is None:
            t = alloc(K, N)
        _lib.check(pack(W.data_ptr(), int(W.stride(0)), K, N, t.data_ptr(), _stream(W.device)), what)
        return t
    return _packed_on_tensor(W, slot, make)


def packed_bf16_weights(W):
    return _packed_weights(W, "_d3f_bf16t", lambda K, N: torch.empty((N, (K + 31) // 32 * 32), dtype=torch.int16, device=W.device),
                           _lib.load().d3f_gemm_pack_bf16, "gemm_pack_bf16")


def packed_f32t_weights(W):
    return _packed_weights(W, "_d3f_f32t", lambda K, N: torch.empty((N, (K + 31) // 32 * 32), dtype=torch.float32, device=W.device),
                           _lib.load().d3f_gemm_pack_f32t, "gemm_pack_f32t")


GEMM_X3 = os.environ.get("D3F_GEMM_X3", "1") != "0"


def packed_x3_weights(W):
    lib = _lib.load()
    return _packed_weights(W, "_d3f_x3", lambda K, N: torch.empty((int(lib.d3f_gemm_x3_packed_bytes(K, N)) // 2,), dtype=torch.int16,
                                                                  device=W.device), lib.d3f_gemm_pack_x3, "gemm_pack_x3")


X3_MAX_ROWS = 65535 * 128


def _x3_resident(M, N, K, hint):
    return bool(_lib.load().d3f_gemm_x3_resident(M, N, K, hint))


def _x3_ok(C1, C2, N, rows=0):
    fits = GEMM_X3 and (C1 + C2) % 32 == 0 and (C2 == 0 or C1 % 32 == 0)
    return fits and (N > 32 or _x3_resident(rows, N, C1 + C2, 0))


def _route(M, plain, bf16, bf16_ok, f32t_ok, x3, resident):
    if bf16 and bf16_ok:
        return "d3f_gemm_bf16", "gemm_bf16"
    if not f32t_ok:
        return ("d3f_gemm_f32" if plain else "d3f_gemm_upsample_cat_f32"), "gemm_f32"
    if x3 and M <= X3_MAX_ROWS:
        return "d3f_gemm_x3", "gemm_x3r" if resident else "gemm_x3"
    return "d3f_gemm_f32t", "gemm_f32"


def _f32t_ok(N, ldc, out, residual, ldr, vectors, *operands):
    if N % 4 or ldc % 4 or out.data_ptr() % 16:
        return False
    if residual is not None and (ldr % 4 or residual.data_ptr() % 16):
        return False
    if any(v is not None and v.data_ptr() % 16 for v in vectors):
        return False
    for t, ld, cols in operands:
        if t is not None and (cols % 4 or ld % 4 or t.data_ptr() % 16 or cols < 4):
            return False
    return True


def _bf16_ok(*operands):
    for t, ld, cols in operands:
        if t is None:
            continue
        if cols % 4 or ld % 4 or t.data_ptr() % (8 if t.dtype == torch.bfloat16 else 16):
            return False
    return True


def _contract(what, A, N1, lda, C1, idx, ld_idx, skip, lds, C2, W, ldb, out, ldc, m_dev, n1_dev, hint, row_scale=None, col_scale=None,
              col_shift=None, residual=None, ldr=0, leaky=False, alpha=0.2):
    lib = _lib.load()
    (M, N), K, dev = out.shape, C1 + C2, out.device
    operands = ((A, lda, C1), (skip, lds, C2))
    entry, name = _route(M, idx is None and skip is None, BF16_CONTRACTION,
                         K >= 4 and ldc == N and W.is_contiguous() and _bf16_ok(*operands),
                         W.is_contiguous() and _f32t_ok(N, ldc, out, residual, ldr, (col_scale, col_shift), *operands),
                         _x3_ok(C1, C2, N, hint if 0 < hint < M else M), _x3_resident(M, N, K, hint))
    if entry != "d3f_gemm_bf16" and (_h(A) or _h(skip) or _h(out)):
        raise TypeError("%s: bfloat16 operands that the bf16 contraction cannot address (K %d, lda %d)" % (what, K, lda))
    flags = [1 if leaky else 0, float(alpha)]
    if entry == "d3f_gemm_f32":
        ws = workspace(lib.d3f_gemm_workspace_bytes(M, N, K, hint), dev)
        args = [A.data_ptr(), lda, W.data_ptr(), ldb, out.data_ptr(), ldc, M, N, K, _ptr(row_scale), _ptr(col_scale), _ptr(col_shift),
                _ptr(residual), ldr] + flags + [ws.data_ptr(), ws.numel(), m_dev, hint]
    else:
        head = [A.data_ptr(), N1, lda, C1, _ptr(idx), ld_idx, _ptr(skip), lds, C2]
        if entry == "d3f_gemm_upsample_cat_f32":
            ws = workspace(lib.d3f_gemm_workspace_bytes(M, N, K, hint), dev)
            args = head + [W.data_ptr(), ldb, out.data_ptr(), ldc, M, N, _ptr(col_scale), _ptr(col_shift)] + flags
        else:
            pack, ws_bytes = {"d3f_gemm_bf16": (packed_bf16_weights, lib.d3f_gemm_bf16_workspace_bytes),
                              "d3f_gemm_f32t": (packed_f32t_weights, lib.d3f_gemm_workspace_bytes),
                              "d3f_gemm_x3": (packed_x3_weights, lib.d3f_gemm_x3_workspace_bytes)}[entry]
            Wp = pack(W)
            ws = workspace(ws_bytes(M, N, K, hint), dev)
            args = head + [Wp.data_ptr(), out.data_ptr(), ldc, M, N, _ptr(row_scale), _ptr(col_scale), _ptr(col_shift), _ptr(residual),
                           ldr] + flags
        args += [ws.data_ptr(), ws.numel(), m_dev, n1_dev, hint]
    if entry == "d3f_gemm_bf16":
        if out.data_ptr() % 16 or (residual is not None and (residual.data_ptr() % 8 or ldr % 4)):
            raise ValueError("gemm (bf16): output / residual must be 16 / 8-byte aligned with a leading dimension of 4 k")
        args += [_h(A), _h(out)]
    with _timed(name, dict(M=M, N=N, K=K), dev):
        rc = getattr(lib, entry)(*args, _stream(dev))
    _lib.check(rc, entry[4:])


def gemm(A, Bm, row_scale=None, col_scale=None, col_shift=None, residual=None, leaky=False, alpha=0.2, out=None):
    A, lda = _rows(_feat(A, "A"), "A")
    Bm, ldb = _rows(_req(Bm, torch.float32, "B"), "B")
    M, K = A.shape
    if Bm.shape[0] != K:
        raise ValueError("gemm: A is %s, B is %s" % (tuple(A.shape), tuple(Bm.shape)))
    N = Bm.shape[1]
    if out is None:
        out = torch.empty((M, N), dtype=_out_dtype(), device=A.device)
    out, ldc = _rows(out, "out")
    ldr = 0
    if residual is not None:
        residual, ldr = _rows(_feat(residual, "residual"), "residual")
    if (_h(A) or _h(out) or _h(residual)) and not (BF16_CONTRACTION and (residual is None or _h(residual) == _h(A))):
        raise TypeError("gemm: bfloat16 feature tensors need ops.bf16_contraction(features=True)")
    for v, n, name in ((row_scale, M, "row_scale"), (col_scale, N, "col_scale"), (col_shift, N, "col_shift")):
        if v is not None:
            _req(v, torch.float32, name)
            if v.numel() != n or not v.is_contiguous():
                raise ValueError("%s must be a contiguous vector of %d" % (name, n))
    _contract("gemm", A, M, lda, K, None, 0, None, 0, 0, Bm, ldb, out, ldc, _nd(A), None, int(getattr(A, "n_hint", 0) or 0),
              row_scale, col_scale, col_shift, residual, ldr, leaky, alpha)
    return _tag(out, A)


class UpsampleCat:

    def __init__(self, x, inds, skip=None):
        self.x, self.inds, self.skip = x, inds, skip
        self.shape = (inds.shape[0], x.shape[1] + (skip.shape[1] if skip is not None else 0))
        self.device = x.device
        _tag(self, inds)

    def materialize(self):
        return closest_pool_cat(self.x, self.inds, self.skip)


def gemm_upsample_cat(u, W, col_scale=None, col_shift=None, leaky=False, alpha=0.2):
    x, ldx = _rows(_feat(u.x, "x"), "x")
    inds, ldi = _rows(_req(u.inds, torch.int32, "inds"), "inds")
    W, ldb = _rows(_req(W, torch.float32, "W"), "W")
    C1, C2, lds, skip = x.shape[1], 0, 0, None
    if u.skip is not None:
        skip, lds = _rows(_feat(u.skip, "skip"), "skip")
        C2 = skip.shape[1]
    M, N = inds.shape[0], W.shape[1]
    if W.shape[0] != C1 + C2:
        raise ValueError("gemm_upsample_cat: W has %d rows, operands %d + %d columns" % (W.shape[0], C1, C2))
    if C2 and (C1 % 4 or lds % 4 or skip.data_ptr() % 16) and not _h(x):
        return gemm(u.materialize(), W, col_scale=col_scale, col_shift=col_shift, leaky=leaky, alpha=alpha)
    out = torch.empty((M, N), dtype=_out_dtype(), device=x.device)
    _contract("gemm_upsample_cat", x, x.shape[0], ldx, C1, inds, ldi, skip, lds, C2, W, ldb, out, N, _nd(inds), _nd(x),
              int(getattr(inds, "n_hint", 0) or 0), col_scale=col_scale, col_shift=col_shift, leaky=leaky, alpha=alpha)
    return _tag(out, inds)


DECODER_SPLIT = os.environ.get("D3F_DECODER_SPLIT", "1") != "0"


def _split_ok(M, C1, C2, N, hint=0, f32=True, f32t_ok=True):
    if not DECODER_SPLIT or BF16_CONTRACTION or not f32 or C2 <= 0 or C1 <= 0 or C1 % 32 or C2 % 32:
        return False
    resident = _x3_resident(M, N, C1 + C2, hint)
    entry, _ = _route(M, False, False, False, f32t_ok, _x3_ok(C1, C2, N, hint if 0 < hint < M else M), resident)
    return entry == "d3f_gemm_x3" and not resident


def upsample_split_ok(u, N):
    if u.skip is None or u.x.dim() != 2 or u.skip.dim() != 2 or u.inds.dim() != 2:
        return False
    f32 = u.x.dtype == torch.float32 and u.skip.dtype == torch.float32
    aligned = all(t.stride(1) == 1 and t.stride(0) % 4 == 0 and t.data_ptr() % 16 == 0 for t in (u.x, u.skip))
    return _split_ok(u.inds.shape[0], u.x.shape[1], u.skip.shape[1], N, int(getattr(u.inds, "n_hint", 0) or 0), f32, aligned and N % 4 == 0)


def gemm_upsample_split(u, W1, W2, col_shift=None, leaky=False, alpha=0.2, out=None):
    lib = _lib.load()
    x, _ = _rows(_req(u.x, torch.float32, "x"), "x")
    inds, ldi = _rows(_req(u.inds, torch.int32, "inds"), "inds")
    if u.skip is None:
        raise ValueError("gemm_upsample_split: no skip operand (use gemm_upsample_cat)")
    skip, lds = _rows(_req(u.skip, torch.float32, "skip"), "skip")
    W1, _ = _rows(_req(W1, torch.float32, "W1"), "W1")
    W2, _ = _rows(_req(W2, torch.float32, "W2"), "W2")
    C1, C2, M, N = x.shape[1], skip.shape[1], inds.shape[0], W2.shape[1]
    if W1.shape != (C1, N) or W2.shape[0] != C2 or skip.shape[0] != M or not (W1.is_contiguous() and W2.is_contiguous()):
        raise ValueError("gemm_upsample_split: operands %s | %s, W1 %s, W2 %s" % (tuple(x.shape), tuple(skip.shape), tuple(W1.shape),
                                                                                   tuple(W2.shape)))
    if not upsample_split_ok(u, N):
        raise ValueError("gemm_upsample_split: not a call of the split form (ops.upsample_split_ok): use gemm_upsample_cat")
    Y = gemm(x, W1)
    dev, hint = x.device, int(getattr(inds, "n_hint", 0) or 0)
    if out is None:
        out = torch.empty((M, N), dtype=torch.float32, device=dev)
    elif out.dtype != torch.float32 or tuple(out.shape) != (M, N) or not out.is_contiguous() or out.data_ptr() % 16:
        raise ValueError("gemm_upsample_split: out must be a contiguous, 16-byte aligned float32 [%d, %d]" % (M, N))
    if col_shift is not None and (col_shift.data_ptr() % 16 or col_shift.numel() != N):
        raise ValueError("gemm_upsample_split: col_shift must be a 16-byte aligned vector of %d" % N)
    Wp = packed_x3_weights(W2)
    ws = workspace(lib.d3f_gemm_x3_workspace_bytes(M, N, C2, hint), dev)
    with _timed("gemm_x3", dict(M=M, N=N, K=C2), dev):
        rc = lib.d3f_gemm_x3_gres(skip.data_ptr(), M, lds, C2, None, 0, None, 0, 0, Wp.data_ptr(), out.data_ptr(), N, M, N, None, None,
                                  _ptr(col_shift), Y.data_ptr(), N, inds.data_ptr(), ldi, x.shape[0], _nd(x), 1 if leaky else 0,
                                  float(alpha), ws.data_ptr(), ws.numel(), _nd(inds), None, hint, _stream(dev))
    _lib.check(rc, "gemm_x3_gres")
    return _tag(out, inds)


def gemm_cat2(A1, A2, W, col_scale=None, col_shift=None, leaky=False, alpha=0.2):
    A1, ld1 = _rows(_feat(A1, "A1"), "A1")
    A2, ld2 = _rows(_feat(A2, "A2"), "A2")
    W, ldb = _rows(_req(W, torch.float32, "W"), "W")
    M, C1, C2, N = A1.shape[0], A1.shape[1], A2.shape[1], W.shape[1]
    if A2.shape[0] != M or W.shape[0] != C1 + C2:
        raise ValueError("gemm_cat2: operands %s | %s, W %s" % (tuple(A1.shape), tuple(A2.shape), tuple(W.shape)))
    if (C1 % 4 or ld2 % 4 or A2.data_ptr() % 16) and not _h(A1):
        return gemm(torch.cat([A1, A2], 1), W, col_scale=col_scale, col_shift=col_shift, leaky=leaky, alpha=alpha)
    out = torch.empty((M, N), dtype=_out_dtype(), device=A1.device)
    _contract("gemm_cat2", A1, M, ld1, C1, None, 0, A2, ld2, C2, W, ldb, out, N, _nd(A1), _nd(A1), int(getattr(A1, "n_hint", 0) or 0),
              col_scale=col_scale, col_shift=col_shift, leaky=leaky, alpha=alpha)
    return _tag(out, A1)


def _kp_front(what, query_points, support_points, neighbors_indices, features, K_points, K_values, KP_extent, KP_influence,
              aggregation_mode, col_scale=None, col_shift=None, residual=None, leaky=False, alpha=0.2, row_pos=True, feat=_feat):
    lib = _lib.load()
    q = _req(query_points, torch.float32, "query_points", 2).contiguous()
    s = _req(support_points, torch.float32, "support_points", 2).contiguous()
    idx, ld_idx = _rows(_req(neighbors_indices, torch.int32, "neighbors_indices"), "neighbors_indices")
    f, ldf = _rows(feat(features, "features"), "features")
    if KP_influence not in _INFLUENCE:
        raise ValueError("Unknown influence function type (config.KP_influence)")
    if aggregation_mode not in _AGGREGATION:
        raise ValueError("Unknown convolution mode. Should be 'closest' or 'sum'")
    if K_values is not None and f.shape[1] != K_values.shape[1]:
        raise ValueError("%s: features have %d channels, K_values expects %d" % (what, f.shape[1], K_values.shape[1]))
    kp = _kp_host(K_points)
    Nq, Ns = q.shape[0], s.shape[0]
    nq_dev, ns_dev = _nd(query_points), _nd(support_points)
    if ns_dev is None:
        ns_dev = _nd(features)
    rpos = None
    if row_pos:
        rpos = torch.empty((max(Ns, 1),), dtype=torch.uint8, device=q.device)
        _lib.check(lib.d3f_row_positive(f.data_ptr(), Ns, ldf, f.shape[1], rpos.data_ptr(), ns_dev, _h(f), _stream(q.device)),
                   "row_positive")
    ldr = 0
    if residual is not None:
        residual, ldr = _rows(_req(residual, torch.float32, "residual"), "residual")
    return ((q, Nq, s, Ns, idx, ld_idx, idx.shape[1], f, ldf),
            (kp, kp.shape[0], float(KP_extent), _INFLUENCE[KP_influence], _AGGREGATION[aggregation_mode]), rpos,
            (col_scale, col_shift, residual, ldr, 1 if leaky else 0, float(alpha)), (nq_dev, ns_dev, _order(query_points)), f)


def _arg(v):
    if isinstance(v, torch.Tensor):
        return v.data_ptr()
    return v.ctypes.data if isinstance(v, np.ndarray) else v


def kpconv_aggregate(query_points, support_points, neighbors_indices, features, K_points, KP_extent,
                     KP_influence="linear", aggregation_mode="sum"):
    lib = _lib.load()
    if neighbors_indices.shape[0] != query_points.shape[0] or features.shape[0] != support_points.shape[0]:
        raise ValueError("KPConv: %d queries / %d index rows, %d supports / %d feature rows" %
                         (query_points.shape[0], neighbors_indices.shape[0], support_points.shape[0], features.shape[0]))
    gather, kpar, row_pos, _, tail, f = _kp_front("KPConv", query_points, support_points, neighbors_indices, features, K_points, None,
                                                  KP_extent, KP_influence, aggregation_mode)
    Nq, Ns, K, Cin = gather[1], gather[3], gather[6], f.shape[1]
    wf = torch.empty((Nq, kpar[1] * Cin), dtype=torch.float32, device=f.device)
    inv_cnt = torch.empty((Nq,), dtype=torch.float32, device=f.device)
    with _timed("kpconv_aggregate", dict(Nq=Nq, Ns=Ns, K=K, Cin=Cin), f.device):
        rc = lib.d3f_kpconv_aggregate(*map(_arg, (*gather, Cin, row_pos, *kpar, wf, inv_cnt, *tail, _h(f), _stream(f.device))))
    _lib.check(rc, "kpconv_aggregate")
    return _tag(wf, query_points), _tag(inv_cnt, query_points)


def kpconv_deform_aggregate(query_points, support_points, neighbors_indices, features, K_points, offsets, KP_extent,
                            KP_influence="linear", aggregation_mode="sum", modulations=None, raw=False):
    lib = _lib.load()
    if neighbors_indices.shape[0] != query_points.shape[0] or features.shape[0] != support_points.shape[0]:
        raise ValueError("KPConv_deformable: %d queries / %d index rows, %d supports / %d feature rows" %
                         (query_points.shape[0], neighbors_indices.shape[0], support_points.shape[0], features.shape[0]))
    if isinstance(features, torch.Tensor) and features.dtype == torch.bfloat16:
        raise TypeError("KPConv_deformable reads float32 feature rows only: d3f_kpconv_deform_aggregate has no bfloat16 "
                        "feature-storage form")
    gather, kpar, _, _, tail, f = _kp_front("KPConv_deformable", query_points, support_points, neighbors_indices, features, K_points,
                                            None, KP_extent, KP_influence, aggregation_mode, row_pos=False,
                                            feat=lambda t, name: _req(t, torch.float32, name))
    Nq, Ns, K, Cin, num_kp = gather[1], gather[3], gather[6], f.shape[1], kpar[1]
    _req(offsets, torch.float32, "offsets")
    if offsets.dim() == 3:
        offsets = offsets.reshape(offsets.shape[0], -1)
    off, ld_off = _rows(offsets, "offsets")
    mod, ld_mod = None, 0
    if raw:
        if modulations is not None or tuple(off.shape) not in ((Nq, 3 * num_kp), (Nq, 4 * num_kp)):
            raise ValueError("KPConv_deformable: raw offsets are %s, expected (%d, %d) or (%d, %d) and no modulations"
                             % (tuple(off.shape), Nq, 3 * num_kp, Nq, 4 * num_kp))
        if off.shape[1] == 4 * num_kp:
            mod, ld_mod = off[:, 3 * num_kp:], ld_off
    else:
        if tuple(off.shape) != (Nq, 3 * num_kp):
            raise ValueError("KPConv_deformable: offsets are %s, expected (%d, %d, 3)" % (tuple(offsets.shape), Nq, num_kp))
        if modulations is not None:
            mod, ld_mod = _rows(_req(modulations, torch.float32, "modulations"), "modulations")
            if tuple(mod.shape) != (Nq, num_kp):
                raise ValueError("KPConv_deformable: modulations are %s, expected (%d, %d)" % (tuple(mod.shape), Nq, num_kp))
    wf = torch.empty((Nq, num_kp * Cin), dtype=torch.float32, device=f.device)
    with _timed("kpconv_deform_aggregate", dict(Nq=Nq, Ns=Ns, K=K, Cin=Cin), f.device):
        rc = lib.d3f_kpconv_deform_aggregate(*map(_arg, (*gather, Cin, off, ld_off, float(KP_extent) if raw else 1.0, mod, ld_mod,
                                                         1 if raw else 0, *kpar, wf, *tail, 0, _stream(f.device))))
    _lib.check(rc, "kpconv_deform_aggregate")
    return _tag(wf, query_points)


def kpconv_deformable(query_points, support_points, neighbors_indices, features, K_points, K_values, offset_weights, offset_bias,
                      KP_extent, KP_influence="linear", aggregation_mode="sum", modulated=False, col_scale=None, col_shift=None,
                      residual=None, leaky=False, alpha=0.2):
    num_kp, cin, cout = K_values.shape
    D = (4 if modulated else 3) * num_kp
    if tuple(offset_weights.shape) != (num_kp, cin, D) or tuple(offset_bias.shape) != (D,):
        raise ValueError("KPConv_deformable: offset_conv_weights %s / offset_conv_bias %s, expected (%d, %d, %d) / (%d,)" %
                         (tuple(offset_weights.shape), tuple(offset_bias.shape), num_kp, cin, D, D))
    if features.shape[1] != cin:
        raise ValueError("KPConv_deformable: features have %d channels, K_values expects %d" % (features.shape[1], cin))
    with f32_output():
        wf0, inv_cnt = kpconv_aggregate(query_points, support_points, neighbors_indices, features, K_points, KP_extent, KP_influence,
                                        aggregation_mode)
        offsets = gemm(wf0, offset_weights.reshape(num_kp * cin, D), row_scale=inv_cnt, col_shift=offset_bias)
    wf = kpconv_deform_aggregate(query_points, support_points, neighbors_indices, features, K_points, offsets, KP_extent,
                                 KP_influence, aggregation_mode, raw=True)
    return gemm(wf, K_values.reshape(num_kp * cin, cout), col_scale=col_scale, col_shift=col_shift, residual=residual, leaky=leaky,
                alpha=alpha)


def kpconv_fused_supported(cin, cout, num_kp, KP_influence, aggregation_mode, available=False):
    r = _lib.load().d3f_kpconv_fused_supported(int(cin), int(cout), int(num_kp), _INFLUENCE.get(KP_influence, -1),
                                               _AGGREGATION.get(aggregation_mode, -1))
    return r >= 1 if available else r == 1


def _packed_kpconv(K_values, slot, alloc, pack, what):
    def make(t):
        num_kp, cin, cout = K_values.shape
        W = _req(K_values, torch.float32, "K_values").reshape(num_kp * cin, cout).contiguous()
        if t is None:
            t = alloc(W)
        _lib.check(pack(W.data_ptr(), num_kp * cin, cout, t.data_ptr(), _stream(W.device)), what)
        return t
    return _packed_on_tensor(K_values, slot, make)


def packed_kpconv_weights(K_values):
    return _packed_kpconv(K_values, "_d3f_packed", torch.empty_like, _lib.load().d3f_kpconv_pack_weights, "kpconv_pack_weights")


def packed_kpconv_weights_x3(K_values):
    lib = _lib.load()
    return _packed_kpconv(K_values, "_d3f_packed_x3",
                          lambda W: torch.empty((int(lib.d3f_kpconv_packed_x3_bytes(*W.shape)) // 2,), dtype=torch.int16, device=W.device),
                          lib.d3f_kpconv_pack_weights_x3, "kpconv_pack_weights_x3")


_PACKERS = (("_d3f_bf16t", packed_bf16_weights), ("_d3f_f32t", packed_f32t_weights), ("_d3f_x3", packed_x3_weights),
            ("_d3f_packed", packed_kpconv_weights), ("_d3f_packed_x3", packed_kpconv_weights_x3))


KP_X3 = os.environ.get("D3F_KP_X3", "1") != "0"


def _kpconv_fused(what, query_points, support_points, neighbors_indices, features, K_points, K_values, KP_extent, KP_influence,
                  aggregation_mode, col_scale, col_shift, residual, leaky, alpha):
    lib = _lib.load()
    num_kp, cin, cout = K_values.shape
    gather, kpar, row_pos, epi, tail, f = _kp_front(what, query_points, support_points, neighbors_indices, features, K_points, K_values,
                                                    KP_extent, KP_influence, aggregation_mode, col_scale, col_shift, residual, leaky,
                                                    alpha)
    level0 = what == "kpconv_fused32"
    x3 = KP_X3 and (num_kp * cin) % 32 == 0 and (level0 or cout % 16 == 0)
    if x3:
        W = packed_kpconv_weights_x3(K_values)
    elif level0:
        W = _req(K_values, torch.float32, "K_values").reshape(num_kp * cin, cout).contiguous()
    else:
        W = packed_kpconv_weights(K_values)
    out = torch.empty((gather[1], cout), dtype=f.dtype, device=f.device)
    with _timed(what, dict(Nq=gather[1], Ns=gather[3], K=gather[6], Cin=cin, Cout=cout), f.device):
        if level0:
            rc = (lib.d3f_kpconv_fused32_x3 if x3 else lib.d3f_kpconv_fused32)(
                *map(_arg, (*gather, row_pos, *kpar, W, *epi, out, cout, *tail, _h(f), _stream(f.device))))
        else:
            rc = (lib.d3f_kpconv_fused_x3 if x3 else lib.d3f_kpconv_fused)(
                *map(_arg, (*gather, cin, row_pos, *kpar, W, cout, *epi, out, cout, *tail, _h(f), _stream(f.device))))
    _lib.check(rc, what)
    return _tag(out, query_points)


def kpconv_fused32(query_points, support_points, neighbors_indices, features, K_points, K_values, KP_extent,
                   KP_influence="linear", aggregation_mode="sum", col_scale=None, col_shift=None, residual=None,
                   leaky=False, alpha=0.2):
    if tuple(K_values.shape[1:]) != (32, 32):
        raise ValueError("kpconv_fused32 needs Cin == Cout == 32")
    return _kpconv_fused("kpconv_fused32", query_points, support_points, neighbors_indices, features, K_points, K_values, KP_extent,
                         KP_influence, aggregation_mode, col_scale, col_shift, residual, leaky, alpha)


def kpconv_fused(query_points, support_points, neighbors_indices, features, K_points, K_values, KP_extent,
                 KP_influence="linear", aggregation_mode="sum", col_scale=None, col_shift=None, residual=None,
                 leaky=False, alpha=0.2):
    return _kpconv_fused("kpconv_fused", query_points, support_points, neighbors_indices, features, K_points, K_values, KP_extent,
                         KP_influence, aggregation_mode, col_scale, col_shift, residual, leaky, alpha)


def kpconv_fused_c1(query_points, support_points, neighbors_indices, features, K_points, K_values, KP_extent,
                    KP_influence="linear", aggregation_mode="sum", col_scale=None, col_shift=None, residual=None,
                    leaky=False, alpha=0.2):
    lib = _lib.load()
    num_kp, cin, cout = K_values.shape
    if cin != 1:
        raise ValueError("kpconv_fused_c1 needs Cin == 1")
    gather, kpar, _, epi, tail, f = _kp_front("kpconv_fused_c1", query_points, support_points, neighbors_indices, features, K_points,
                                              K_values, KP_extent, KP_influence, aggregation_mode, col_scale, col_shift, residual,
                                              leaky, alpha, row_pos=False, feat=lambda t, name: _req(t, torch.float32, name))
    W = _req(K_values, torch.float32, "K_values").reshape(num_kp, cout).contiguous()
    out = torch.empty((gather[1], cout), dtype=torch.bfloat16 if BF16_FEATURES else torch.float32, device=f.device)
    with _timed("kpconv_fused_c1", dict(Nq=gather[1], Ns=gather[3], K=gather[6], Cin=1, Cout=cout), f.device):
        rc = lib.d3f_kpconv_fused_c1(*map(_arg, (*gather, *kpar, W, cout, *epi, out, cout, *tail, _h(out), _stream(f.device))))
    _lib.check(rc, "kpconv_fused_c1")
    return _tag(out, query_points)


def ind_max_pool(x, inds):
    lib = _lib.load()
    x, ldx = _rows(_feat(x, "x"), "x")
    inds, ldi = _rows(_req(inds, torch.int32, "inds"), "inds")
    dev = x.device
    out = torch.empty((inds.shape[0], x.shape[1]), dtype=x.dtype, device=dev)
    with _timed("ind_max_pool", dict(N1=x.shape[0], N2=inds.shape[0], K=inds.shape[1], C=x.shape[1]), dev):
        rc = lib.d3f_ind_max_pool(x.data_ptr(), x.shape[0], ldx, x.shape[1], inds.data_ptr(), inds.shape[0], ldi,
                                  inds.shape[1], out.data_ptr(), x.shape[1], None, _nd(x), _nd(inds), _order(inds),
                                  _h(x), _stream(dev))
    _lib.check(rc, "ind_max_pool")
    return _tag(out, inds)


def closest_pool_cat(x, inds, skip=None):
    lib = _lib.load()
    x, ldx = _rows(_req(x, torch.float32, "x"), "x")
    inds, ldi = _rows(_req(inds, torch.int32, "inds"), "inds")
    dev = x.device
    C1 = x.shape[1]
    C2 = lds = 0
    if skip is not None:
        skip, lds = _rows(_req(skip, torch.float32, "skip"), "skip")
        C2 = skip.shape[1]
        if skip.shape[0] != inds.shape[0]:
            raise ValueError("closest_pool_cat: %d index rows, %d skip rows" % (inds.shape[0], skip.shape[0]))
    out = torch.empty((inds.shape[0], C1 + C2), dtype=torch.float32, device=dev)
    rc = lib.d3f_closest_pool_cat(x.data_ptr(), x.shape[0], ldx, C1, inds.data_ptr(), inds.shape[0], ldi,
                                  _ptr(skip), lds, C2, out.data_ptr(), C1 + C2,
                                  _nd(x), _nd(inds), _stream(dev))
    _lib.check(rc, "closest_pool_cat")
    return _tag(out, inds)


def detect_head(x, neighbors, stack_lengths_dev, include_zero_dev, stack_group=0):
    lib = _lib.load()
    x, ldx = _rows(_req(x, torch.float32, "x"), "x")
    nb, ldi = _rows(_req(neighbors, torch.int32, "neighbors"), "neighbors")
    dev = x.device
    N, Cc = x.shape
    B = stack_lengths_dev.numel()
    desc = torch.empty((N, Cc), dtype=torch.float32, device=dev)
    score = torch.empty((N, 1), dtype=torch.float32, device=dev)
    scratch = torch.empty((2 * B + 2 + (N + 3) // 4,), dtype=torch.int32, device=dev)
    with _timed("detect_head", dict(N=N, K=nb.shape[1], C=Cc), dev):
        rc = lib.d3f_detect_head(x.data_ptr(), N, ldx, Cc, nb.data_ptr(), ldi, nb.shape[1],
                                 stack_lengths_dev.data_ptr(),
                                 _ptr(include_zero_dev),
                                 int(stack_group), B, desc.data_ptr(), Cc, score.data_ptr(), scratch.data_ptr(), _order(nb),
                                 _stream(dev))
    _lib.check(rc, "detect_head")
    return _tag(desc, x), _tag(score, x)


def _typed(t, dtype, name, ndim=None):
    if not isinstance(t, torch.Tensor):
        raise TypeError("%s must be a torch.Tensor on a GPU (got %s)" % (name, type(t)))
    if t.dtype != dtype:
        raise TypeError("%s must be %s (got %s)" % (name, dtype, t.dtype))
    if ndim is not None and t.dim() != ndim:
        raise ValueError("%s must be %d-D (got shape %s)" % (name, ndim, tuple(t.shape)))
    return t


def _head_arguments(what, x, neighbors, stack_lengths_dev):
    nb, ldi = _rows(_typed(neighbors, torch.int32, "neighbors"), "neighbors")
    lens = _typed(stack_lengths_dev, torch.int32, "stack_lengths_dev", 1)
    if not lens.is_contiguous():
        raise ValueError("%s: stack_lengths_dev must be contiguous" % what)
    if not 1 <= lens.numel() <= 255:
        raise ValueError("%s: %d clouds (1 .. 255)" % (what, lens.numel()))
    if nb.shape[0] * nb.shape[1] > (1 << 31) - 8192:
        raise ValueError("%s: %d x %d neighbour slots (at most 2^31 - 8192)" % (what, nb.shape[0], nb.shape[1]))
    if x is not None and x.shape[0] != nb.shape[0]:
        raise ValueError("%s: %d feature rows, %d neighbour rows" % (what, x.shape[0], nb.shape[0]))
    return nb, ldi, lens


def _on_device(what, **tensors):
    for name, t in tensors.items():
        if t is not None and not t.is_cuda:
            raise _lib.D3FeatLibraryError("%s: %s is on %s: d3feat_amd has no CPU path" % (what, name, t.device))


def neighbor_transpose(neighbors, stack_lengths_dev):
    lib = _lib.load()
    nb, ldi, lens = _head_arguments("neighbor_transpose", None, neighbors, stack_lengths_dev)
    _on_device("neighbor_transpose", neighbors=nb, stack_lengths_dev=lens)
    dev = nb.device
    N, K = nb.shape
    start = torch.empty((N + 1,), dtype=torch.int32, device=dev)
    edges = torch.empty((max(N * K, 1),), dtype=torch.int32, device=dev)
    nbytes = lib.d3f_neighbor_transpose_workspace_bytes(N, K)
    ws = workspace(nbytes, dev)
    with _timed("neighbor_transpose", dict(N=N, K=K), dev):
        rc = lib.d3f_neighbor_transpose(nb.data_ptr(), N, ldi, K, lens.data_ptr(), lens.numel(), start.data_ptr(), edges.data_ptr(),
                                        ws.data_ptr(), nbytes, _stream(dev))
    _lib.check(rc, "neighbor_transpose")
    return start, edges[:N * K]


def detect_head_backward(x, neighbors, stack_lengths_dev, include_zero_dev, grad_desc, grad_score, stack_group=0, transpose=None,
                         out=None):
    lib = _lib.load()
    x, ldx = _rows(_typed(x, torch.float32, "x"), "x")
    nb, ldi, lens = _head_arguments("detect_head_backward", x, neighbors, stack_lengths_dev)
    dev = x.device
    N, Cc = x.shape
    if not 1 <= Cc <= 128:
        raise ValueError("detect_head_backward: C = %d (1 .. 128)" % Cc)
    if int(stack_group) < 0:
        raise ValueError("detect_head_backward: stack_group = %r" % (stack_group,))
    gd = ldg = gs = ldgs = None
    if grad_desc is not None:
        gd, ldg = _rows(_typed(grad_desc, torch.float32, "grad_desc"), "grad_desc")
        if tuple(gd.shape) != (N, Cc):
            raise ValueError("detect_head_backward: grad_desc is %s, x %s" % (tuple(gd.shape), (N, Cc)))
    if grad_score is not None:
        gs = _typed(grad_score, torch.float32, "grad_score")
        if gs.dim() == 1:
            gs = gs.unsqueeze(1)
        if gs.dim() != 2 or tuple(gs.shape) != (N, 1):
            raise ValueError("detect_head_backward: grad_score is %s, wanted %d rows of one column" % (tuple(grad_score.shape), N))
        ldgs = int(max(gs.stride(0), 1)) if N > 1 else 1
    if include_zero_dev is not None:
        include_zero_dev = _typed(include_zero_dev, torch.int32, "include_zero_dev", 1)
        if include_zero_dev.numel() != lens.numel() or not include_zero_dev.is_contiguous():
            raise ValueError("detect_head_backward: include_zero_dev must be contiguous, one entry per cloud")
    if out is not None:
        out, ldo = _rows(_typed(out, torch.float32, "out"), "out")
        if tuple(out.shape) != (N, Cc):
            raise ValueError("detect_head_backward: out is %s, x %s" % (tuple(out.shape), (N, Cc)))
    _on_device("detect_head_backward", x=x, neighbors=nb, stack_lengths_dev=lens, include_zero_dev=include_zero_dev, grad_desc=gd,
               grad_score=gs, out=out)
    if transpose is None:
        transpose = neighbor_transpose(nb, lens)
    start = _typed(transpose[0], torch.int32, "transpose[0]", 1)
    edges = _typed(transpose[1], torch.int32, "transpose[1]", 1)
    if start.numel() != N + 1 or edges.numel() < N * nb.shape[1] or not (start.is_contiguous() and edges.is_contiguous()):
        raise ValueError("detect_head_backward: transpose must be (start i32[N + 1], edges i32[N * K]) of the same neighbours")
    _on_device("detect_head_backward", start=start, edges=edges)
    if out is None:
        out, ldo = torch.empty((N, Cc), dtype=torch.float32, device=dev), Cc
    B = lens.numel()
    nbytes = lib.d3f_detect_head_backward_workspace_bytes(N, Cc, B)
    ws = workspace(nbytes, dev)
    with _timed("detect_head_backward", dict(N=N, K=nb.shape[1], C=Cc), dev):
        rc = lib.d3f_detect_head_backward(x.data_ptr(), N, ldx, Cc, nb.data_ptr(), ldi, nb.shape[1], lens.data_ptr(), _ptr(include_zero_dev),
                                          int(stack_group), B, start.data_ptr(), edges.data_ptr(), _ptr(gd), ldg or 0, _ptr(gs), ldgs or 0,
                                          out.data_ptr(), ldo, ws.data_ptr(), nbytes, _stream(dev))
    _lib.check(rc, "detect_head_backward")
    return _tag(out, x)


def _count(t, name):
    if t is not None:
        _typed(t, torch.int32, name)
        if t.numel() != 1:
            raise ValueError("%s must hold one int32 (got shape %s)" % (name, tuple(t.shape)))
    return t


def neighbor_transpose_supports(neighbors, num_supports, nq_dev=None, ns_dev=None):
    lib = _lib.load()
    nb, ldi = _rows(_typed(neighbors, torch.int32, "neighbors"), "neighbors")
    Ns = int(num_supports)
    if Ns < 0:
        raise ValueError("neighbor_transpose_supports: num_supports = %d" % Ns)
    Nq, K = nb.shape
    if Nq * K > (1 << 31) - 8192:
        raise ValueError("neighbor_transpose_supports: %d x %d neighbour slots (at most 2^31 - 8192)" % (Nq, K))
    if nq_dev is None:
        nq_dev = getattr(neighbors, "n_dev", None)
    nq_dev, ns_dev = _count(nq_dev, "nq_dev"), _count(ns_dev, "ns_dev")
    _on_device("neighbor_transpose_supports", neighbors=nb, nq_dev=nq_dev, ns_dev=ns_dev)
    dev = nb.device
    start = torch.empty((Ns + 1,), dtype=torch.int32, device=dev)
    edges = torch.empty((max(Nq * K, 1),), dtype=torch.int32, device=dev)
    nbytes = lib.d3f_neighbor_transpose_workspace_bytes(Nq, K)
    ws = workspace(nbytes, dev)
    with _timed("neighbor_transpose_supports", dict(Nq=Nq, Ns=Ns, K=K), dev):
        rc = lib.d3f_neighbor_transpose_qs(nb.data_ptr(), Nq, ldi, K, _ptr(nq_dev), Ns, _ptr(ns_dev), start.data_ptr(), edges.data_ptr(),
                                           ws.data_ptr(), nbytes, _stream(dev))
    _lib.check(rc, "neighbor_transpose_supports")
    return start, edges[:Nq * K]


def kpconv_backward(query_points, support_points, neighbors_indices, features, K_points, K_values, grad_out, KP_extent,
                    KP_influence="linear", aggregation_mode="sum", transpose=None, need_features=True, need_weights=True,
                    out_features=None, out_weights=None):
    lib = _lib.load()
    q = _typed(query_points, torch.float32, "query_points", 2)
    s = _typed(support_points, torch.float32, "support_points", 2)
    idx, ld_idx = _rows(_typed(neighbors_indices, torch.int32, "neighbors_indices"), "neighbors_indices")
    f, ldf = _rows(_typed(features, torch.float32, "features"), "features")
    W = _typed(K_values, torch.float32, "K_values", 3)
    g, ldg = _rows(_typed(grad_out, torch.float32, "grad_out"), "grad_out")
    if KP_influence not in _INFLUENCE:
        raise ValueError("Unknown influence function type (config.KP_influence)")
    if aggregation_mode not in _AGGREGATION:
        raise ValueError("Unknown convolution mode. Should be 'closest' or 'sum'")
    if q.shape[1] != 3 or s.shape[1] != 3:
        raise ValueError("kpconv_backward: points must be [n, 3] (got %s, %s)" % (tuple(q.shape), tuple(s.shape)))
    Nq, Ns, K = q.shape[0], s.shape[0], idx.shape[1]
    num_kp, Cin, Cout = W.shape
    kp = _kp_host(K_points)
    if kp.ndim != 2 or kp.shape != (num_kp, 3) or not 1 <= num_kp <= 15:
        raise ValueError("kpconv_backward: K_points is %s, K_values %s (1 .. 15 kernel points)" % (tuple(kp.shape), tuple(W.shape)))
    if Cin < 1 or Cout < 1:
        raise ValueError("kpconv_backward: K_values is %s" % (tuple(W.shape),))
    if idx.shape[0] != Nq or f.shape[0] != Ns:
        raise ValueError("kpconv_backward: %d queries / %d index rows, %d supports / %d feature rows" % (Nq, idx.shape[0], Ns, f.shape[0]))
    if f.shape[1] != Cin:
        raise ValueError("kpconv_backward: features have %d channels, K_values expects %d" % (f.shape[1], Cin))
    if tuple(g.shape) != (Nq, Cout):
        raise ValueError("kpconv_backward: grad_out is %s, wanted %s" % (tuple(g.shape), (Nq, Cout)))
    if not (need_features or need_weights):
        raise ValueError("kpconv_backward: neither gradient is wanted")
    if Nq * K > (1 << 31) - 8192:
        raise ValueError("kpconv_backward: %d x %d neighbour slots (at most 2^31 - 8192)" % (Nq, K))
    if Ns == 0 and Nq > 0:
        raise ValueError("kpconv_backward: %d queries and no support" % Nq)
    if not float(KP_extent) > 0:
        raise ValueError("kpconv_backward: KP_extent = %r" % (KP_extent,))
    gf = ldgf = gW = None
    if need_features and out_features is not None:
        gf, ldgf = _rows(_typed(out_features, torch.float32, "out_features"), "out_features")
        if tuple(gf.shape) != (Ns, Cin):
            raise ValueError("kpconv_backward: out_features is %s, wanted %s" % (tuple(gf.shape), (Ns, Cin)))
    if need_weights and out_weights is not None:
        gW = _typed(out_weights, torch.float32, "out_weights", 3)
        if tuple(gW.shape) != (num_kp, Cin, Cout) or not gW.is_contiguous():
            raise ValueError("kpconv_backward: out_weights must be contiguous %s" % ((num_kp, Cin, Cout),))
    start = edges = None
    if need_features and transpose is not None:
        start = _typed(transpose[0], torch.int32, "transpose[0]", 1)
# ... 271 lines not shown
```

### include/d3feat_amd.h

```cpp
#ifndef D3FEAT_AMD_H
#define D3FEAT_AMD_H

#include <stddef.h>
#include <stdint.h>

#ifdef __cplusplus
extern "C" {
#endif

#define D3F_OK 0
#define D3F_ERR_HIP (-1)
#define D3F_ERR_WORKSPACE (-2)
#define D3F_ERR_ARG (-3)

#define D3F_ST_EMPTY_ELEMENT 1
#define D3F_ST_NEG_CELL 2
#define D3F_ST_KEY_RANGE 4
#define D3F_ST_HIT_OVERFLOW 8
#define D3F_ST_OUT_OVERFLOW 16
#define D3F_ST_KEY_WIDTH 32

#define D3F_NB_NO_KMAX 2
#define D3F_PAD_NUM_SUPPORTS (-2147483647 - 1)

#define D3F_MAX_BATCH 255
#define D3F_NEIGHBOR_CAP 1024
#define D3F_TOPK_MAX 8192
#define D3F_PAIRS_KMAX 1024
#define D3F_REPEAT_COUNTS_MAX 16
#define D3F_SCENES_MAX 256
#define D3F_MATCH_KMAX 8192
#define D3F_VALIDATION_NMAX 1024
#define D3F_NUM_KP_MAX 16

int d3f_version(void);

int d3f_trace_marker(int id, void* stream);
int d3f_pack_status(int* dst, const int* a, int na, const int* b, int nb, const int* c, int nc, const int* d, int nd,
                    int* clear, int nclear, int clear_first, int clear_step, void* stream);


size_t d3f_grid_subsample_workspace_bytes(int N, int B, int fdim, int ldim);
int d3f_batch_grid_subsample_async(const float* points, int N_cap, const int* lens_dev, int B, float dl,
                                   float* sub_points, int M_cap, int elem_cap, int elem_points_cap, int* sub_lens_dev,
                                   int* status_dev, void* workspace, size_t workspace_bytes, void* stream);
int d3f_batch_grid_subsample_async_inplace(const float* const* clouds_dev, int N_cap, const int* lens_dev, int B, float dl,
                                           float* sub_points, int M_cap, int elem_cap, int* sub_lens_dev, int* status_dev,
                                           void* workspace, size_t workspace_bytes, void* stream);

int d3f_stack_self_pair(const float* pts, int M_cap, const int* lens_in_dev, int B, float* out, int* lens_out_dev,
                        int* total_dev, void* stream);
int d3f_stack_self_pair_boxed(const float* pts, int M_cap, const int* lens_in_dev, int B, float* out, int* lens_out_dev,
                              int* total_dev, const unsigned* bbox_in_dev, unsigned* bbox_out_dev, void* stream);
int d3f_batch_grid_subsample_async_boxed(const float* points, const float* const* clouds_dev, int N_cap, const int* lens_dev,
                                         int B, float dl, float* sub_points, int M_cap, int elem_cap, int elem_points_cap,
                                         int* sub_lens_dev, int* status_dev, const unsigned* bbox_in_dev,
                                         unsigned* bbox_out_dev, void* workspace, size_t workspace_bytes, void* stream);
int d3f_batch_grid_subsample(const float* points, int N, const int* lens_dev, int B, float dl,
                             const float* features, int fdim, const int* classes, int ldim,
                             float* sub_points, float* sub_features, int* sub_classes, int* sub_lens_dev,
                             int* status_host, void* workspace, size_t workspace_bytes, void* stream);

size_t d3f_radius_neighbors_workspace_bytes(int Nq, int Ns, int B);
int d3f_batch_radius_neighbors(const float* queries, int Nq, const float* supports, int Ns,
                               const int* q_lens_dev, const int* s_lens_dev, int B, float radius,
                               int* out, int ld, int width, int pad_value, int* status_dev,
                               void* workspace, size_t workspace_bytes, void* stream);

size_t d3f_neighbor_grid_bytes(int Ns, int B);
size_t d3f_neighbor_grid_order_offset(int Ns, int B);
int d3f_neighbor_grid_build(const float* supports, int Ns, const int* s_lens_dev, int B, float radius,
                            void* grid, size_t grid_bytes, void* stream);
#define D3F_GRID_RESET_MAX 8
int d3f_neighbor_grid_boxed_form(int Ns, int B);
int d3f_geometry_reset(unsigned* boxes_dev, int n_boxes, const void* const* grids, const size_t* grid_bytes, const int* Ns,
                       const int* B, int n_grids, void* stream);
int d3f_neighbor_grid_build_boxed(const float* supports, int Ns, const int* s_lens_dev, int B, float radius,
                                  const unsigned* bbox_dev, void* grid, size_t grid_bytes, void* stream);
int d3f_neighbor_grid_search(const void* grid, size_t grid_bytes, int Ns, const float* queries, int Nq,
                             const int* q_lens_dev, int B, float radius, int queries_are_supports,
                             int* out, int ld, int width, int pad_value, int cap, int first_only, float nn_hint,
                             int reset_status, int* status_dev, void* stream);
#define D3F_NB_INTERNAL 4
int d3f_neighbor_grid_search_ordered(const void* grid, size_t grid_bytes, int Ns, const float* queries, int Nq,
                                     const int* q_lens_dev, int B, float radius, const void* query_grid, size_t query_grid_bytes,
                                     int* out, int ld, int width, int pad_value, int cap, int first_only, float nn_hint, int flags,
                                     int* status_dev, void* stream);
size_t d3f_neighbor_grid_inv_offset(int Ns, int B);
size_t d3f_neighbor_grid_xyz_offset(int Ns, int B);



int d3f_row_positive(const void* f, int Ns, int ldf, int Cin, unsigned char* row_pos, const int* Ns_dev, int feat_bf16,
                     void* stream);
int d3f_kpconv_aggregate(const float* q, int Nq, const float* s, int Ns, const int* idx, int ld_idx, int K,
                         const void* f, int ldf, int Cin, const unsigned char* row_pos, const float* kp_host,
                         int num_kp, float KP_extent, int influence, int aggregation, float* wf, float* inv_cnt,
                         const int* Nq_dev, const int* Ns_dev, const int* q_order, int feat_bf16, void* stream);

int d3f_kpconv_deform_aggregate(const float* q, int Nq, const float* s, int Ns, const int* idx, int ld_idx, int K,
                                const void* f, int ldf, int Cin, const float* offsets, int ld_off, float offset_scale,
                                const float* modulations, int ld_mod, int mod_logits, const float* kp_host, int num_kp,
                                float KP_extent, int influence, int aggregation, float* wf, const int* Nq_dev, const int* Ns_dev,
                                const int* q_order, int feat_bf16, void* stream);

int d3f_kpconv_fused_c1(const float* q, int Nq, const float* s, int Ns, const int* idx, int ld_idx, int K,
                        const float* f, int ldf, const float* kp_host, int num_kp, float KP_extent, int influence,
                        int aggregation, const float* W, int Cout, const float* col_scale, const float* col_shift,
                        const float* residual, int ldr, int leaky, float alpha, void* out, int ldo,
                        const int* Nq_dev, const int* Ns_dev, const int* q_order, int out_bf16, void* stream);

int d3f_kpconv_fused32(const float* q, int Nq, const float* s, int Ns, const int* idx, int ld_idx, int K,
                       const void* f, int ldf, const unsigned char* row_pos, const float* kp_host, int num_kp,
                       float KP_extent, int influence, int aggregation, const float* W, const float* col_scale,
                       const float* col_shift, const float* residual, int ldr, int leaky, float alpha, void* out, int ldo,
                       const int* Nq_dev, const int* Ns_dev, const int* q_order, int feat_bf16, void* stream);

int d3f_kpconv_fused_supported(int Cin, int Cout, int num_kp, int influence, int aggregation);
int d3f_kpconv_pack_weights(const float* W, int K, int N, float* W_packed, void* stream);
size_t d3f_kpconv_packed_x3_bytes(int K, int N);
int d3f_kpconv_pack_weights_x3(const float* W, int K, int N, void* W_planes, void* stream);
int d3f_kpconv_fused32_x3(const float* q, int Nq, const float* s, int Ns, const int* idx, int ld_idx, int K,
                          const void* f, int ldf, const unsigned char* rowpos, const float* kp_host, int num_kp,
                          float KP_extent, int influence, int aggregation, const float* W_planes, const float* col_scale,
                          const float* col_shift, const float* residual, int ldr, int leaky, float alpha, void* out,
                          int ldo, const int* Nq_dev, const int* Ns_dev, const int* q_order, int feat_bf16, void* stream);
int d3f_kpconv_fused_x3(const float* q, int Nq, const float* s, int Ns, const int* idx, int ld_idx, int K,
                        const void* f, int ldf, int Cin, const unsigned char* rowpos, const float* kp_host, int num_kp,
                        float KP_extent, int influence, int aggregation, const float* W_planes, int Cout,
                        const float* col_scale, const float* col_shift, const float* residual, int ldr, int leaky,
                        float alpha, void* out, int ldo, const int* Nq_dev, const int* Ns_dev, const int* q_order,
                        int feat_bf16, void* stream);
int d3f_kpconv_fused(const float* q, int Nq, const float* s, int Ns, const int* idx, int ld_idx, int K,
                     const void* f, int ldf, int Cin, const unsigned char* rowpos, const float* kp_host, int num_kp,
                     float KP_extent, int influence, int aggregation, const float* W_packed, int Cout,
                     const float* col_scale, const float* col_shift, const float* residual, int ldr, int leaky,
                     float alpha, void* out, int ldo, const int* Nq_dev, const int* Ns_dev, const int* q_order,
                     int feat_bf16, void* stream);

size_t d3f_gemm_workspace_bytes(int M, int N, int K, int M_hint);
int d3f_gemm_f32(const float* A, int lda, const float* B, int ldb, float* C, int ldc, int M, int N, int K,
                 const float* row_scale, const float* col_scale, const float* col_shift,
                 const float* residual, int ldr, int leaky, float alpha,
                 void* workspace, size_t workspace_bytes, const int* M_dev, int M_hint, void* stream);

int d3f_gemm_upsample_cat_f32(const float* x, int N1, int ldx, int C1, const int* idx, int ld_idx,
                              const float* skip, int lds, int C2, const float* W, int ldb, float* C, int ldc,
                              int M, int N, const float* col_scale, const float* col_shift, int leaky, float alpha,
                              void* workspace, size_t workspace_bytes, const int* M_dev, const int* N1_dev,
                              int M_hint, void* stream);

int d3f_ind_max_pool(const void* x, int N1, int ldx, int C, const int* idx, int N2, int ld_idx, int K,
                     void* out, int ldo, float* col_min_dev, const int* N1_dev, const int* N2_dev, const int* row_order,
                     int feat_bf16, void* stream);
int d3f_closest_pool_cat(const float* x, int N1, int ldx, int C1, const int* idx, int N2, int ld_idx,
                         const float* skip, int lds, int C2, float* out, int ldo, const int* N1_dev, const int* N2_dev,
                         void* stream);

int d3f_affine_act(const float* x, int ldx, int M, int N, const float* col_scale, const float* col_shift,
                   const float* residual, int ldr, int leaky, float alpha, float* out, int ldo, const int* M_dev,
                   void* stream);

int d3f_detect_head(const float* x, int N, int ldx, int C, const int* idx, int ld_idx, int K,
                    const int* lens_dev, const int* include_zero_dev, int stack_group, int B, float* desc, int ldd,
                    float* score, int* scratch_dev, const int* row_order, void* stream);

int d3f_pack_descriptors(const float* xyz, const float* desc, int ldd, int C, const float* score, int N, float* out,
                         int ldo, const int* N_dev, void* stream);
int d3f_pack_descriptors_to(const float* xyz, const float* desc, int ldd, int C, const float* score, int N, float* out,
                            int ldo, const int* N_dev, const int* lens_dev, int B, int group, int keep,
                            const long long* dst_ptrs_dev, const int* row_map_dev, void* stream);

size_t d3f_topk_workspace_bytes(int N, int B, int n_cap, int K);
int d3f_topk_records(const float* xyz, int ldx, const float* desc, int ldd, int C, const float* score, int lds, int N,
                     const int* N_dev, const int* lens_dev, int B, int group, int keep, const int* row_map_dev, int n_cap, int K,
                     float* out, int ldo, int* idx_out, int* count_dev, int* tickets_dev, void* workspace, size_t workspace_bytes,
                     void* stream);

int d3f_gemm_pack_f32t(const float* W, int ldb, int K, int N, float* Wt, void* stream);
int d3f_gemm_f32t(const float* A, int N1, int lda, int C1, const int* idx, int ld_idx, const float* skip, int lds, int C2,
                  const float* Wt, float* C, int ldc, int M, int N, const float* row_scale, const float* col_scale,
                  const float* col_shift, const float* residual, int ldr, int leaky, float alpha, void* workspace,
                  size_t workspace_bytes, const int* M_dev, const int* N1_dev, int M_hint, void* stream);

size_t d3f_gemm_x3_packed_bytes(int K, int N);
int d3f_gemm_pack_x3(const float* W, int ldb, int K, int N, void* Wx, void* stream);
size_t d3f_gemm_x3_workspace_bytes(int M, int N, int K, int M_hint);
int d3f_gemm_x3_plan(int M, int N, int K, int M_hint, int* rows, int* cols, int* slices);
int d3f_gemm_x3_resident(int M, int N, int K, int M_hint);
int d3f_gemm_x3(const float* A, int N1, int lda, int C1, const int* idx, int ld_idx, const float* skip, int lds, int C2,
                const void* Wx, float* C, int ldc, int M, int N, const float* row_scale, const float* col_scale,
                const float* col_shift, const float* residual, int ldr, int leaky, float alpha, void* workspace,
                size_t workspace_bytes, const int* M_dev, const int* N1_dev, int M_hint, void* stream);
int d3f_gemm_x3_gres(const float* A, int N1, int lda, int C1, const int* idx, int ld_idx, const float* skip, int lds, int C2,
                     const void* Wx, float* C, int ldc, int M, int N, const float* row_scale, const float* col_scale,
                     const float* col_shift, const float* residual, int ldr, const int* res_idx, int ld_res_idx, int res_rows,
                     const int* res_rows_dev, int leaky, float alpha, void* workspace, size_t workspace_bytes, const int* M_dev,
                     const int* N1_dev, int M_hint, void* stream);

size_t d3f_gemm_bf16_workspace_bytes(int M, int N, int K, int M_hint);
int d3f_gemm_pack_bf16(const float* W, int ldb, int K, int N, void* W_packed, void* stream);
int d3f_gemm_bf16(const void* A, int N1, int lda, int C1, const int* idx, int ld_idx, const void* skip, int lds, int C2,
                  const void* W_packed, void* C, int ldc, int M, int N, const float* row_scale, const float* col_scale,
                  const float* col_shift, const void* residual, int ldr, int leaky, float alpha, void* workspace,
                  size_t workspace_bytes, const int* M_dev, const int* N1_dev, int M_hint, int a_bf16, int c_bf16, void* stream);

int d3f_decode_xyz_records(const void* raw, int n, int stride, int off_x, int off_y, int off_z, int is_f64, int big_endian,
                           float* out, void* stream);


size_t d3f_feature_nn_workspace_bytes(int Na);
int d3f_feature_nn(const float* A, int Na, int lda, const float* B, int Nb, int ldb, int C, int* idx, float* d2_out,
                   void* workspace, size_t workspace_bytes, void* stream);

size_t d3f_mutual_matches_workspace_bytes(int Na);
int d3f_mutual_matches(const int* ab, int Na, const int* ba, int Nb, int* pairs, int* count_dev, void* workspace,
                       size_t workspace_bytes, void* stream);

int d3f_ransac_hypotheses(const float* src, int Ns, const float* tgt, int Nt, const int* nn, int ransac_n,
                          float edge_similarity, float checker_distance, uint64_t seed, uint64_t it0,
                          int H, float* T_out, unsigned char* valid_out, void* stream);
int d3f_ransac_draw(uint64_t seed, uint64_t iteration, int d, int n);

int d3f_neighbor_grid_score(const void* grid, size_t grid_bytes, int Nt, const float* src, int Ns, const float* T, int V,
                            float radius, int* count_dev, uint64_t* sumd2_dev, int* nearest_dev, void* stream);

size_t d3f_register_pairs_workspace_bytes(int P, int K, int num_keypts, int max_validation);
int d3f_register_pairs(const float* kp, int n_blocks, int K, int ld, int C, const int* count_dev, const int* pairs_dev, int P,
                       int num_keypts, float max_correspondence_distance, int ransac_n, float edge_similarity,
                       float checker_distance, int max_iteration, int max_validation, uint64_t seed, const float* gt,
                       float distance_threshold, float* T_out, int* inliers, uint64_t* sumd2, int* validations, int* iterations,
                       int* best_iteration, int* mutual_count, int* nearest, int* mutual, int* gt_inliers, void* workspace,
                       size_t workspace_bytes, void* stream);

int d3f_repeatability_pairs(const float* kp, int n_blocks, int K, int ld, const int* count_dev, const int* pairs_dev, int P,
                            const double* gt_dev, int moved, const double* threshold_host, const int* num_keypts_host,
                            int n_counts, int* repeat_dev, int64_t* totals_dev, void* stream);

size_t d3f_match_pairs_workspace_bytes(int P, const int* num_keypts_host, int n_counts);
int d3f_match_pairs(const float* kp, int n_blocks, int K, int ld, int C, const int* count_dev, const int* pairs_dev, int P,
                    const float* gt, float distance_threshold, const int* num_keypts_host, int n_counts, int* mutual_count,
                    int* gt_inliers, void* workspace, size_t workspace_bytes, void* stream);

size_t d3f_register_pairs_counts_workspace_bytes(int P, int n_blocks, int K, const int* num_keypts_host, int n_counts,
                                                 int max_validation);
int d3f_register_pairs_counts(const float* kp, int n_blocks, int K, int ld, int C, const int* count_dev, const int* pairs_dev, int P,
                              const int* num_keypts_host, int n_counts, float max_correspondence_distance, int ransac_n,
                              float edge_similarity, float checker_distance, int max_iteration, int max_validation, uint64_t seed,
                              const float* gt, float distance_threshold, float* T_out, int* inliers, uint64_t* sumd2,
                              int* validations, int* iterations, int* best_iteration, int* mutual_count, int* gt_inliers,
                              int* nearest, void* workspace, size_t workspace_bytes, void* stream);

int d3f_overlap_pairs(const void* grid, size_t grid_bytes, int N, int B, const int* pairs_dev, int P, float threshold,
                      int* count_dev, int* nearest_dev, int ld_nearest, void* stream);

size_t d3f_validation_pairs_workspace_bytes(int P, int ld_idx);
int d3f_validation_pairs(const float* desc, int ldd, int C, const float* score, int lds, const float* points, int ldp, int n_rows,
                         const int* row0_dev, const int* anc_dev, const int* pos_dev, int ld_idx, const int* n_dev, int P,
                         float safe_radius, int keypts_num, float det_loss_weight, float pos_margin, float neg_margin,
                         float log_scale, float* values, int* status_dev, double* sums_dev, int64_t* counts_dev, void* workspace,
                         size_t workspace_bytes, void* stream);

size_t d3f_loss_gradients_workspace_bytes(int P, int ld_idx, int C);
int d3f_loss_gradients(const float* desc, int ldd, int C, const float* score, int lds, const float* points, int ldp, int n_rows,
                       const int* row0_dev, const int* anc_dev, const int* pos_dev, int ld_idx, const int* n_dev, int P,
                       float safe_radius, int keypts_num, float det_loss_weight, float pos_margin, float neg_margin, float log_scale,
                       int contrastive, float* grad_desc, int ldg, float* grad_score, int ldgs, float* values, int* status_dev,
                       void* workspace, size_t workspace_bytes, void* stream);

size_t d3f_neighbor_transpose_workspace_bytes(int N, int K);
int d3f_neighbor_transpose(const int* idx, int N, int ld_idx, int K, const int* lens_dev, int B, int* start, int* edges, void* workspace,
                           size_t workspace_bytes, void* stream);

size_t d3f_detect_head_backward_workspace_bytes(int N, int C, int B);
int d3f_detect_head_backward(const float* x, int N, int ldx, int C, const int* idx, int ld_idx, int K, const int* lens_dev,
                             const int* include_zero_dev, int stack_group, int B, const int* start, const int* edges,
                             const float* gdesc, int ldg, const float* gscore, int ldgs, float* gx, int ldgx, void* workspace,
                             size_t workspace_bytes, void* stream);

int d3f_neighbor_transpose_qs(const int* idx, int Nq, int ld_idx, int K, const int* Nq_dev, int Ns, const int* Ns_dev, int* start,
                              int* edges, void* workspace, size_t workspace_bytes, void* stream);

size_t d3f_kpconv_backward_workspace_bytes(int Nq, int Ns, int K, int Cin, int Cout, int num_kp);
int d3f_kpconv_backward(const float* q, int Nq, const float* s, int Ns, const int* idx, int ld_idx, int K, const void* f, int ldf,
                        int Cin, const float* kp_host, int num_kp, float KP_extent, int influence, int aggregation, const float* W,
                        const float* gout, int ldg, int Cout, const int* start, const int* edges, float* gf, int ldgf, float* gW,
                        const int* Nq_dev, const int* Ns_dev, const int* q_order, int feat_bf16, void* workspace,
                        size_t workspace_bytes, void* stream);

size_t d3f_gemm_tn_workspace_bytes(int M, int Ca, int Cb);
int d3f_gemm_tn_f32(const float* A, int lda, const float* B, int ldb, int M, int Ca, int Cb, float* out, const int* M_dev,
                    void* workspace, size_t workspace_bytes, void* stream);

size_t d3f_batch_norm_workspace_bytes(int M, int C);
int d3f_batch_norm_train(const float* x, int ldx, int M, int C, const float* gamma, const float* beta, float eps, float momentum,
                         float* moving_mean, float* moving_var, const float* residual, int ldr, int leaky, float alpha, float* y, int ldy,
                         float* mean, float* rstd, const int* M_dev, void* workspace, size_t workspace_bytes, void* stream);
int d3f_batch_norm_backward(const float* x, int ldx, const float* y, int ldy, const float* gy, int ldg, int M, int C, const float* gamma,
                            const float* mean, const float* rstd, int leaky, float alpha, float* gx, int ldgx, float* ggamma,
                            float* gbeta, float* gres, int ldgr, const int* M_dev, void* workspace, size_t workspace_bytes, void* stream);

int d3f_pose_errors(const float* T_est, const float* gt, int P, int per_pair, const double* thresholds_host, double* rte_dev,
                    double* rre_deg_dev, int* flags_dev, double* meters_dev, void* stream);

int d3f_sanitize_descriptors(float* kp, int n_blocks, int K, int ld, int C, void* stream);

int d3f_matching_summary(const int* mutual_count, const int* gt_inliers, const int* gt_flag, int P, int n, const int* scene_start_host,
                         int S, const double* inlier_ratio_host, int* ratio_e8, long long* figures, void* stream);

int d3f_registration_recall(const void* T_est, int logged, const double* gt, const double* info, const int* gt_flag,
                            const int* result_flag, const int* ids, int P, int n, const int* scene_start_host, int S,
                            const double* err2_host, double* error, int* flags, long long* figures, void* stream);

size_t d3f_icp_pairs_workspace_bytes(int N_src, int B);
int d3f_icp_pairs(const void* grid, size_t grid_bytes, int N_tgt, const float* src, int N_src, const int* src_lens_dev, int B,
                  const double* init, const double* criteria_host, int max_iteration, int check_every, double* T, int* count,
                  double* sumd2, double* fitness, double* rmse, int* iterations, int* converged, int* nearest, void* workspace,
                  size_t workspace_bytes, void* stream);

#ifdef __cplusplus
}
#endif
#endif
```

Before: 1957 fragments/s.

## Chain second unary GEMM into resident x3 GEMM epilogue for resnetb and upsample

```diff
diff --git a/d3feat_amd/_lib.py b/d3feat_amd/_lib.py
--- a/d3feat_amd/_lib.py
+++ b/d3feat_amd/_lib.py
@@ -132,6 +132,10 @@
                          _vp, _vp, _i, _vp]),
     "d3f_gemm_x3_gres": (_i, [_vp, _i, _i, _i, _vp, _i, _vp, _i, _i, _vp, _vp, _i, _i, _i, _vp, _vp, _vp, _vp, _i, _vp, _i, _i, _vp, _i, _f,
                               _vp, _sz, _vp, _vp, _i, _vp]),
+    "d3f_gemm_pack_x3_chain": (_i, [_vp, _i, _i, _i, _vp, _vp]),
+    "d3f_gemm_x3_chain_ok": (_i, [_i, _i, _i, _i, _i]),
+    "d3f_gemm_x3_chain": (_i, [_vp, _i, _i, _i, _vp, _i, _vp, _i, _i, _vp, _vp, _i, _i, _i, _vp, _vp, _vp, _vp, _i, _i, _f, _vp,
+                               _vp, _vp, _i, _f, _vp, _i, _vp, _vp, _vp]),
     "d3f_gemm_bf16": (_i, [_vp, _i, _i, _i, _vp, _i, _vp, _i, _i, _vp, _vp, _i, _i, _i, _vp, _vp, _vp, _vp, _i, _i, _f, _vp, _sz,
                            _vp, _vp, _i, _i, _i, _vp]),
     "d3f_decode_xyz_records": (_i, [_vp, _i, _i, _i, _i, _i, _i, _i, _vp, _vp]),
diff --git a/d3feat_amd/csrc/gemm_f32.hip b/d3feat_amd/csrc/gemm_f32.hip
--- a/d3feat_amd/csrc/gemm_f32.hip
+++ b/d3feat_amd/csrc/gemm_f32.hip
@@ -678,6 +678,16 @@
     return D3F_OK;
 }
 
+extern "C" int d3f_gemm_pack_x3_chain(const float* B, int ldb, int K, int N, void* Wx, void* stream_) {
+    hipStream_t stream = (hipStream_t)stream_;
+    if ((K != 64 && K != 128) || N != 32 || ldb < N || !B || !Wx || ((uintptr_t)Wx & 15)) return D3F_ERR_ARG;
+    const int nkt = K / GX_BK;
+    const long long total = (long long)nkt * GX_CHUNK;
+    gemm_pack_x3_kernel<<<d3f_cdiv(total, 256), 256, 0, stream>>>(B, ldb, K, N, nkt, total, (unsigned short*)Wx, 1);
+    D3F_LAUNCH_CHECK();
+    return D3F_OK;
+}
+
 extern "C" int d3f_gemm_x3_plan(int M, int N, int K, int M_hint, int* rows, int* cols, int* slices) {
     if (M <= 0 || N <= 0 || K < GX_BK || (K % GX_BK)) return D3F_ERR_ARG;
     const GemmX3Plan p = gemm_x3_plan(M, N, K, M_hint);
@@ -701,6 +711,29 @@
     if (N < 1 || K < GX_BK || (K % GX_BK)) return 0;
     const int NG = d3f_cdiv(N, 32), m_eff = (M_hint > 0 && M_hint < M) ? M_hint : M;
     return (NG == 1 || NG == 2 || NG == 4) && gemm_x3r_lds_bytes(K / GX_BK, NG) <= 160 * 1024 && m_eff >= 65536;
+}
+
+static size_t gemm_x3r_chain_lds_bytes(int nkt, int NG, int store_first) {
+    return (size_t)(nkt + 1) * NG * GX_CHUNK * sizeof(unsigned short) + (store_first ? GXR_PATCH_BYTES : 0) + GXR_EPI_BYTES + GXR_EPI2_BYTES;
+}
+
+extern "C" int d3f_gemm_x3_chain_ok(int M, int N, int K, int store_first, int M_hint) {
+    if (!d3f_gemm_x3_resident(M, N, K, M_hint) || (N != 64 && N != 128)) return 0;
+    return gemm_x3r_chain_lds_bytes(K / GX_BK, N / 32, store_first) <= 160 * 1024;
+}
+
+static int gemm_cus() {
+    static std::atomic<int> cus_of[64];
+    int dev = 0;
+    if (hipGetDevice(&dev) != hipSuccess) return 0;
+    int cus = cus_of[dev & 63].load(std::memory_order_relaxed);
+    if (!cus) {
+        hipDeviceProp_t pr;
+        if (hipGetDeviceProperties(&pr, dev) != hipSuccess) return 0;
+        cus = pr.multiProcessorCount > 0 ? pr.multiProcessorCount : 256;
+        cus_of[dev & 63].store(cus, std::memory_order_relaxed);
+    }
+    return cus;
 }
 
 static int gemm_x3_run(const float* A, int N1, int lda, int C1, const int* idx, int ld_idx, const float* skip, int lds, int C2,
@@ -721,16 +754,8 @@
     GemmGather G{idx, ld_idx, N1, N1_dev, C2 > 0 ? skip : nullptr, lds, C1};
     const int nkt = K / GX_BK, NG = d3f_cdiv(N, 32);
     if (!res_idx && d3f_gemm_x3_resident(M, N, K, M_hint)) {
-        static std::atomic<int> cus_of[64];
-        int dev = 0;
-        if (hipGetDevice(&dev) != hipSuccess) return D3F_ERR_HIP;
-        int cus = cus_of[dev & 63].load(std::memory_order_relaxed);
-        if (!cus) {
-            hipDeviceProp_t pr;
-            if (hipGetDeviceProperties(&pr, dev) != hipSuccess) return D3F_ERR_HIP;
-            cus = pr.multiProcessorCount > 0 ? pr.multiProcessorCount : 256;
-            cus_of[dev & 63].store(cus, std::memory_order_relaxed);
-        }
+        const int cus = gemm_cus();
+        if (!cus) return D3F_ERR_HIP;
         static std::atomic<unsigned long long> lds_done{0};
         const void* const fns[3] = {(const void*)gemm_x3r_kernel<1>, (const void*)gemm_x3r_kernel<2>, (const void*)gemm_x3r_kernel<4>};
         if (d3f_opt_in_lds(lds_done, fns, 160 * 1024) != D3F_OK) return D3F_ERR_HIP;
@@ -776,3 +801,38 @@
                        res_idx, ld_res_idx, res_rows, res_rows_dev, leaky, alpha, workspace, workspace_bytes, M_dev, N1_dev, M_hint,
                        stream_);
 }
+
+extern "C" int d3f_gemm_x3_chain(const float* A, int N1, int lda, int C1, const int* idx, int ld_idx, const float* skip, int lds, int C2cols,
+                                 const void* Wx, float* C, int ldc, int M, int N, const float* row_scale, const float* col_scale,
+                                 const float* col_shift, const float* residual, int ldr, int leaky, float alpha, const void* W2x,
+                                 const float* col_scale2, const float* col_shift2, int leaky2, float alpha2, float* C2, int ldc2,
+                                 const int* M_dev, const int* N1_dev, void* stream_) {
+    hipStream_t stream = (hipStream_t)stream_;
+    const int K = C1 + C2cols, store = C != nullptr;
+    bool empty;
+    if (int rc = gemm_check_composite(true, GX_BK, 15, M, N, N1, C1, C2cols, lda, store ? ldc : N, lds, ldr, ld_idx, A, Wx, store ? C : C2,
+                                      idx, skip, residual, col_scale, col_shift, empty))
+        return rc;
+    if ((N != 64 && N != 128) || ldc2 < 32 || (ldc2 % 4)) return D3F_ERR_ARG;
+    const int nkt = K / GX_BK, NG = N / 32;
+    const size_t lds_bytes = gemm_x3r_chain_lds_bytes(nkt, NG, store);
+    if (lds_bytes > 160 * 1024) return D3F_ERR_ARG;
+    if (empty) return D3F_OK;
+    if (!C2 || !W2x || (((uintptr_t)C2 | (uintptr_t)W2x) & 15)) return D3F_ERR_ARG;
+    GemmEpi E{row_scale, col_scale, col_shift, residual, ldr, leaky, alpha, nullptr, 0, 0, nullptr};
+    GemmGather G{idx, ld_idx, N1, N1_dev, C2cols > 0 ? skip : nullptr, lds, C1};
+    GemmChain H{(const unsigned short*)W2x, col_scale2, col_shift2, leaky2, alpha2, C2, ldc2};
+    const int cus = gemm_cus();
+    if (!cus) return D3F_ERR_HIP;
+    static std::atomic<unsigned long long> lds_done{0};
+    const void* const fns[4] = {(const void*)gemm_x3r_chain_kernel<2, true>, (const void*)gemm_x3r_chain_kernel<2, false>,
+                                (const void*)gemm_x3r_chain_kernel<4, true>, (const void*)gemm_x3r_chain_kernel<4, false>};
+    if (d3f_opt_in_lds(lds_done, fns, 160 * 1024) != D3F_OK) return D3F_ERR_HIP;
+    const int grid = std::min(cus, d3f_cdiv(d3f_cdiv(M, 32), 8));
+#define D3F_GXC(TN_, ST_) gemm_x3r_chain_kernel<TN_, ST_><<<grid, 512, lds_bytes, stream>>>(A, lda, (const unsigned short*)Wx, nkt, C, ldc, M, N, E, M_dev, G, H)
+    if (NG == 4) { if (store) D3F_GXC(4, true); else D3F_GXC(4, false); }
+    else { if (store) D3F_GXC(2, true); else D3F_GXC(2, false); }
+#undef D3F_GXC
+    D3F_LAUNCH_CHECK();
+    return D3F_OK;
+}
diff --git a/d3feat_amd/csrc/gemm_x3.h b/d3feat_amd/csrc/gemm_x3.h
--- a/d3feat_amd/csrc/gemm_x3.h
+++ b/d3feat_amd/csrc/gemm_x3.h
@@ -41,7 +41,7 @@
 }
 
 __global__ void __launch_bounds__(256) gemm_pack_x3_kernel(const float* __restrict__ B, int ldb, int K, int N, int nkt, long long total,
-                                                           unsigned short* __restrict__ Wx) {
+                                                           unsigned short* __restrict__ Wx, int chain = 0) {
     const long long t = (long long)blockIdx.x * blockDim.x + threadIdx.x;
     if (t >= total) return;
     const int kk = (int)(t % GX_LS);
@@ -50,7 +50,12 @@
     const int p = (int)(q % 3); q /= 3;
     const int kt = (int)(q % nkt);
     const int ng = (int)(q / nkt);
-    const int k = kt * GX_BK + kk, n = ng * 32 + r;
+    int ks = kk;
+    if (chain && kk < GX_BK) {
+        const int h = (kk >> 3) & 1, i = kk & 7;
+        ks = (kk & 16) + (i < 4 ? 4 * h + i : 8 + 4 * h + i - 4);
+    }
+    const int k = kt * GX_BK + ks, n = ng * 32 + r;
     unsigned out = 0u;
     if (kk < GX_BK && k < K && n < N) {
         float w = B[(size_t)k * ldb + n];
@@ -314,12 +319,26 @@
 #define GXR_PS 36
 #define GXR_PATCH_BYTES (8 * 32 * GXR_PS * 4)
 #define GXR_EPI_BYTES (2 * 128 * 4)
-template <int TN>
-__global__ void __launch_bounds__(512) __attribute__((amdgpu_waves_per_eu(2, 2)))
-gemm_x3r_kernel(const float* __restrict__ A, int lda, const unsigned short* __restrict__ Wx, int nkt, float* __restrict__ C, int ldc,
-                int M, int N, GemmEpi E, const int* __restrict__ M_dev, GemmGather G) {
+#define GXR_EPI2_BYTES (2 * 32 * 4)
+struct GemmChain {
+    const unsigned short* W2x;
+    const float* col_scale;
+    const float* col_shift;
+    int leaky;
+    float alpha;
+    float* C2;
+    int ldc2;
+};
+template <int TN, int CH>
+__device__ __forceinline__ void gemm_x3r_body(const float* __restrict__ A, int lda, const unsigned short* __restrict__ Wx, int nkt,
+                                              float* __restrict__ C, int ldc, int M, int N, const GemmEpi& E,
+                                              const int* __restrict__ M_dev, const GemmGather& G, const GemmChain& H) {
     extern __shared__ __attribute__((aligned(16))) unsigned char gxr_w[];
     static_assert(TN == 1 || TN == 2 || TN == 4, "column groups per row tile");
+    static_assert(CH == 0 || TN > 1, "the chained form contracts 64 or 128 columns");
+    const size_t w2_ofs = (size_t)nkt * TN * (GX_CHUNK * 2);
+    const size_t patch_ofs = w2_ofs + (CH ? (size_t)TN * (GX_CHUNK * 2) : 0);
+    const size_t ep_ofs = patch_ofs + (CH == 2 ? 0 : GXR_PATCH_BYTES);
     M = d3f_dyn(M, M_dev);
     const int tid = threadIdx.x, lane = tid & 63, wave = tid >> 6;
     {
@@ -331,21 +350,31 @@
             const int kt = c / TN, j = c - kt * TN;
             dst[e] = src[(size_t)(j * nkt + kt) * 480 + o];
         }
-        float* ep = (float*)(gxr_w + (size_t)nkt * TN * (GX_CHUNK * 2) + GXR_PATCH_BYTES);
+        float* ep = (float*)(gxr_w + ep_ofs);
         for (int c = tid; c < 32 * TN; c += 512) {
             ep[c] = (E.col_scale && c < N) ? E.col_scale[c] : 1.f;
             ep[32 * TN + c] = (E.col_shift && c < N) ? E.col_shift[c] : 0.f;
         }
+        if constexpr (CH != 0) {
+            const uint4* src2 = (const uint4*)H.W2x;
+            uint4* dst2 = (uint4*)(gxr_w + w2_ofs);
+            for (int e = tid; e < TN * 480; e += 512) dst2[e] = src2[e];
+            if (tid < 32) {
+                ep[64 * TN + tid] = H.col_scale ? H.col_scale[tid] : 1.f;
+                ep[64 * TN + 32 + tid] = H.col_shift ? H.col_shift[tid] : 0.f;
+            }
+        }
     }
     __syncthreads();
-    const float* ep_scale = (const float*)(gxr_w + (size_t)nkt * TN * (GX_CHUNK * 2) + GXR_PATCH_BYTES);
+    const float* ep_scale = (const float*)(gxr_w + ep_ofs);
     const float* ep_shift = ep_scale + 32 * TN;
     const int ntiles = (M + 31) >> 5;
-    auto kofs_now = [&]() -> int {
+    auto lane_now = [&]() -> int {
         unsigned l;
         asm volatile("v_mbcnt_lo_u32_b32 %0, -1, 0\n\tv_mbcnt_hi_u32_b32 %0, -1, %0" : "=v"(l));
-        return (int)((l >> 5) << 3);
-    };
+        return (int)l;
+    };
+    auto kofs_now = [&]() -> int { return (int)(((unsigned)lane_now() >> 5) << 3); };
     const int K1 = G.K1;
     const int n1 = G.gidx ? d3f_dyn(G.N1, G.N1_dev) : 0;
     const int tstride = 8 * (int)gridDim.x;
@@ -445,21 +474,28 @@
             for (int p = 0; p < 3; ++p) nxt[s][p] = make_uint4(P[p][4 * s], P[p][4 * s + 1], P[p][4 * s + 2], P[p][4 * s + 3]);
     };
     int c_tile = rt0, c_kt = 0;
-    float* patch = (float*)(gxr_w + (size_t)nkt * TN * (GX_CHUNK * 2)) + wave * (32 * GXR_PS);
+    float* patch = (float*)(gxr_w + patch_ofs) + wave * (32 * GXR_PS);
     auto finish_tile = [&]() {
         const int gm_a = c_tile * 32 + (lane & 31);
         const bool mok = gm_a < M;
         float rs = 1.f;
         if (E.row_scale && mok) rs = E.row_scale[gm_a];
+        f32x16 acc2;
+        if constexpr (CH != 0) {
+#pragma unroll
+            for (int r = 0; r < 16; ++r) acc2[r] = 0.f;
+        }
 #pragma unroll
         for (int j = 0; j < TN; ++j) {
+            float fv[16];
 #pragma unroll
             for (int q = 0; q < 4; ++q) {
                 const int gn = 32 * j + 8 * q + 4 * (lane >> 5);
                 float v[4] = {acc[j][4 * q], acc[j][4 * q + 1], acc[j][4 * q + 2], acc[j][4 * q + 3]};
-                if (mok && gn < N) {
-                    const float4 c4 = *(const float4*)&ep_scale[gn];
-                    const float4 h4 = *(const float4*)&ep_shift[gn];
+                if (mok && (CH || gn < N)) {
+                    const float* epl = CH ? ep_scale + (kofs_now() >> 1) : nullptr;
+                    const float4 c4 = *(const float4*)(CH ? &epl[32 * j + 8 * q] : &ep_scale[gn]);
+                    const float4 h4 = *(const float4*)(CH ? &epl[32 * TN + 32 * j + 8 * q] : &ep_shift[gn]);
                     const float4 r4 = E.residual ? *(const float4*)&E.residual[(size_t)gm_a * E.ldr + gn] : make_float4(0.f, 0.f, 0.f, 0.f);
                     const float c[4] = {c4.x, c4.y, c4.z, c4.w}, h[4] = {h4.x, h4.y, h4.z, h4.w}, rr[4] = {r4.x, r4.y, r4.z, r4.w};
 #pragma unroll
@@ -469,21 +505,77 @@
                         v[e] = (E.leaky && !(tt > 0.f)) ? tt * E.alpha : tt;
                     }
                 }
-                *(float4*)&patch[(lane & 31) * GXR_PS + 8 * q + 4 * (lane >> 5)] = make_float4(v[0], v[1], v[2], v[3]);
+                if constexpr (CH != 2) *(float4*)&patch[(lane & 31) * GXR_PS + 8 * q + 4 * (lane >> 5)] = make_float4(v[0], v[1], v[2], v[3]);
+                if constexpr (CH != 0) { fv[4 * q] = v[0]; fv[4 * q + 1] = v[1]; fv[4 * q + 2] = v[2]; fv[4 * q + 3] = v[3]; }
                 acc[j][4 * q] = acc[j][4 * q + 1] = acc[j][4 * q + 2] = acc[j][4 * q + 3] = 0.f;
             }
-            __builtin_amdgcn_fence(__ATOMIC_RELEASE, "wavefront");
-            __builtin_amdgcn_wave_barrier();
-            const int cc = 32 * j + 4 * (lane & 7);
-#pragma unroll
-            for (int i = 0; i < 4; ++i) {
-                const int r = (lane >> 3) + 8 * i;
-                const float4 o = *(const float4*)&patch[r * GXR_PS + 4 * (lane & 7)];
-                const int gm = c_tile * 32 + r;
-                if (gm < M && cc < N) *(float4*)&C[(size_t)gm * ldc + cc] = o;
-            }
-            __builtin_amdgcn_fence(__ATOMIC_ACQUIRE, "wavefront");
-            __builtin_amdgcn_wave_barrier();
+            if constexpr (CH != 0) {
+                const unsigned short* bp2 = (const unsigned short*)(gxr_w + w2_ofs) + j * GX_CHUNK + (lane & 31) * GX_LS + kofs_now();
+                constexpr int PA2[6] = {2, 1, 0, 1, 0, 0}, PB2[6] = {0, 1, 2, 0, 1, 0};
+#pragma unroll
+                for (int s = 0; s < 2; ++s) {
+                    const gx_f4 x0 = {fv[8 * s], fv[8 * s + 1], fv[8 * s + 2], fv[8 * s + 3]};
+                    const gx_f4 x1 = {fv[8 * s + 4], fv[8 * s + 5], fv[8 * s + 6], fv[8 * s + 7]};
+                    uint4 pl[3], b2[3];
+#pragma unroll
+                    for (int p = 0; p < 3; ++p) b2[p] = *(const uint4*)(bp2 + p * (32 * GX_LS) + 16 * s);
+                    gx_split8(x0, x1, pl);
+#pragma unroll
+                    for (int prod = 0; prod < 6; ++prod)
+                        acc2 = __builtin_amdgcn_mfma_f32_32x32x16_bf16(__builtin_bit_cast(gb_bf16x8, b2[PB2[prod]]),
+                                                                       __builtin_bit_cast(gb_bf16x8, pl[PA2[prod]]), acc2, 0, 0, 0);
+                }
+            }
+            if constexpr (CH != 2) {
+                __builtin_amdgcn_fence(__ATOMIC_RELEASE, "wavefront");
+                __builtin_amdgcn_wave_barrier();
+                const int sl = CH ? lane_now() : lane;
+                const int cc = 32 * j + 4 * (sl & 7);
+#pragma unroll
+                for (int i = 0; i < 4; ++i) {
+                    const int r = (sl >> 3) + 8 * i;
+                    const float4 o = *(const float4*)&patch[r * GXR_PS + 4 * (sl & 7)];
+                    const int gm = c_tile * 32 + r;
+                    if (gm < M && (CH || cc < N)) *(float4*)&C[(size_t)gm * ldc + cc] = o;
+                }
+                __builtin_amdgcn_fence(__ATOMIC_ACQUIRE, "wavefront");
+                __builtin_amdgcn_wave_barrier();
+            }
+        }
+        if constexpr (CH != 0) {
+            const float* ep2 = ep_scale + 64 * TN;
+#pragma unroll
+            for (int q = 0; q < 4; ++q) {
+                const int gn = 8 * q + 4 * (lane >> 5);
+                float v[4] = {acc2[4 * q], acc2[4 * q + 1], acc2[4 * q + 2], acc2[4 * q + 3]};
+                const float4 c4 = *(const float4*)&ep2[gn];
+                const float4 h4 = *(const float4*)&ep2[32 + gn];
+                const float c[4] = {c4.x, c4.y, c4.z, c4.w}, h[4] = {h4.x, h4.y, h4.z, h4.w};
+#pragma unroll
+                for (int e = 0; e < 4; ++e) {
+                    const float tt = v[e] * c[e] + h[e];
+                    v[e] = (H.leaky && !(tt > 0.f)) ? tt * H.alpha : tt;
+                }
+                if constexpr (CH == 2) {
+                    if (mok) *(float4*)&H.C2[(size_t)gm_a * H.ldc2 + gn] = make_float4(v[0], v[1], v[2], v[3]);
+                } else {
+                    *(float4*)&patch[(lane & 31) * GXR_PS + gn] = make_float4(v[0], v[1], v[2], v[3]);
+                }
+            }
+            if constexpr (CH == 1) {
+                __builtin_amdgcn_fence(__ATOMIC_RELEASE, "wavefront");
+                __builtin_amdgcn_wave_barrier();
+                const int sl = lane_now();
+#pragma unroll
+                for (int i = 0; i < 4; ++i) {
+                    const int r = (sl >> 3) + 8 * i;
+                    const float4 o = *(const float4*)&patch[r * GXR_PS + 4 * (sl & 7)];
+                    const int gm = c_tile * 32 + r;
+                    if (gm < M) *(float4*)&H.C2[(size_t)gm * H.ldc2 + 4 * (sl & 7)] = o;
+                }
+                __builtin_amdgcn_fence(__ATOMIC_ACQUIRE, "wavefront");
+                __builtin_amdgcn_wave_barrier();
+            }
         }
         c_tile += tstride;
     };
@@ -515,3 +607,17 @@
     asm volatile("s_waitcnt vmcnt(0)" : "+v"(rA0), "+v"(rA1), "+v"(rA2), "+v"(rA3), "+v"(rB0), "+v"(rB1), "+v"(rB2), "+v"(rB3), "+v"(rC0),
                  "+v"(rC1), "+v"(rC2), "+v"(rC3) : : "memory");
 }
+
+template <int TN>
+__global__ void __launch_bounds__(512) __attribute__((amdgpu_waves_per_eu(2, 2)))
+gemm_x3r_kernel(const float* __restrict__ A, int lda, const unsigned short* __restrict__ Wx, int nkt, float* __restrict__ C, int ldc,
+                int M, int N, GemmEpi E, const int* __restrict__ M_dev, GemmGather G) {
+    gemm_x3r_body<TN, 0>(A, lda, Wx, nkt, C, ldc, M, N, E, M_dev, G, GemmChain{});
+}
+
+template <int TN, bool STORE>
+__global__ void __launch_bounds__(512) __attribute__((amdgpu_waves_per_eu(2, 2)))
+gemm_x3r_chain_kernel(const float* __restrict__ A, int lda, const unsigned short* __restrict__ Wx, int nkt, float* __restrict__ C,
+                      int ldc, int M, int N, GemmEpi E, const int* __restrict__ M_dev, GemmGather G, GemmChain H) {
+    gemm_x3r_body<TN, STORE ? 1 : 2>(A, lda, Wx, nkt, C, ldc, M, N, E, M_dev, G, H);
+}
diff --git a/d3feat_amd/models/network_blocks.py b/d3feat_amd/models/network_blocks.py
--- a/d3feat_amd/models/network_blocks.py
+++ b/d3feat_amd/models/network_blocks.py
@@ -131,6 +131,10 @@
 
 def last_unary_block(layer_ind, inputs, features, radius, fdim, config, training):
     w = weight_variable([int(features.shape[1]), 32])
+    if isinstance(features, ops.PendingUnary):
+        return features.chain(w)
+    if isinstance(features, ops.UpsampleCat):
+        features = features.materialize()
     with ops.f32_output():
         return conv_ops.unary_convolution(features, w)
 
@@ -141,9 +145,14 @@
         vs = _vs()
         w = vs.parameter(vs.weight_variable([int(features.shape[1]), fdim]))
         return _bn_train(unary_trainable(features, w), config.use_batch_norm, config.batch_norm_momentum, leaky=True)
+    if isinstance(features, ops.PendingUnary):
+        features = features.materialize()
     if isinstance(features, ops.UpsampleCat):
         vs = _vs()
         w = vs.weight_variable([int(features.shape[1]), fdim])
+        if ops.pending_unary_ok(features, fdim):
+            e = _epilogue(fdim, config, True)
+            return ops.PendingUnary(features, vs.tensor(w), e['col_scale'], e['col_shift'], True, 0.2)
         if ops.upsample_split_ok(features, fdim):
             if config.use_batch_norm:
                 w1, w2, shift = vs.split_decoder(w, vs.batch_norm_variables(fdim), int(features.x.shape[1]))
@@ -203,11 +212,44 @@
         return _bn_train(unary_trainable(x, w3), bn, momentum, leaky=True, residual=shortcut)
 
 
+_NEXT_RESNETB = None
+_CHAINED = '_d3f_chained_conv1'
+
+
+def _chain_next_conv1(x, shortcut, W, shift, fdim, config):
+    if _NEXT_RESNETB is None or fdim // 2 != 32 or not isinstance(x, torch.Tensor) or not isinstance(shortcut, torch.Tensor):
+        return None
+    M, K = int(x.shape[0]), int(x.shape[1]) + int(shortcut.shape[1])
+    ok = all(t.dtype == torch.float32 and t.dim() == 2 and t.stride(1) == 1 and t.stride(0) % 4 == 0 and t.data_ptr() % 16 == 0
+             and t.shape[1] % 32 == 0 for t in (x, shortcut))
+    if not ok or not ops.gemm_chain_ok(M, 2 * fdim, K, True, int(getattr(x, 'n_hint', 0) or 0)):
+        return None
+    vs = _vs()
+    depth, scope = _NEXT_RESNETB
+    saved = vs._scope
+    vs._scope = saved[:depth] + [scope, 'conv1']
+    try:
+        wn = vs.weight_variable([2 * fdim, fdim // 2])
+        e = _epilogue(fdim // 2, config, True)
+    finally:
+        vs._scope = saved
+    out, x_next = ops.gemm_chain(x, W, vs.tensor(wn), skip=shortcut, store_first=True, col_shift=shift, leaky=True, alpha=0.2,
+                                 col_scale2=e['col_scale'], col_shift2=e['col_shift'], leaky2=True, alpha2=0.2)
+    setattr(out, _CHAINED, (wn, e['col_scale'], e['col_shift'], x_next))
+    return out
+
+
 def _resnetb(layer_ind, inputs, features, radius, fdim, config, strided, deformable=False):
     cin = int(features.shape[1])
     with variable_scope('conv1'):
-        w = weight_variable([cin, fdim // 2])
-        x = conv_ops.unary_convolution(features, w, epilogue=_epilogue(fdim // 2, config, True))
+        vs = _vs()
+        wn = vs.weight_variable([cin, fdim // 2])
+        e = _epilogue(fdim // 2, config, True)
+        att = features.__dict__.pop(_CHAINED, None) if isinstance(features, torch.Tensor) else None
+        if att is not None and ops.GEMM_CHAIN and att[0] == wn and att[1] is e['col_scale'] and att[2] is e['col_shift']:
+            x = att[3]
+        else:
+            x = conv_ops.unary_convolution(features, vs.tensor(wn), epilogue=e)
     with variable_scope('conv2'):
         w = weight_variable([config.num_kernel_points, fdim // 2, fdim // 2])
         if strided:
@@ -240,7 +282,8 @@
         vs = _vs()
         if fuse:
             W, shift = vs.stacked_branches(w3, bn3, sc_w, sc_bn)
-            return ops.gemm_cat2(x, shortcut, W, col_shift=shift, leaky=True, alpha=0.2)
+            out = None if (strided or ops.BF16_CONTRACTION) else _chain_next_conv1(x, shortcut, W, shift, fdim, config)
+            return out if out is not None else ops.gemm_cat2(x, shortcut, W, col_shift=shift, leaky=True, alpha=0.2)
         return conv_ops.unary_convolution(x, vs.tensor(w3), epilogue=_epilogue(2 * fdim, config, True, residual=shortcut))
 
 
@@ -286,7 +329,7 @@
              'resnetb_strided': resnetb_strided_block, 'resnetb_deformable': resnetb_deformable_block,
              'resnetb_deformable_strided': resnetb_deformable_strided_block, 'nearest_upsample': nearest_upsample_block}
     if block_name in table:
-        return table[block_name] if block_name == 'unary' else _materialized(table[block_name])
+        return table[block_name] if block_name in ('unary', 'last_unary') else _materialized(table[block_name])
     known_unsupported = ('simple_strided', 'resnet', 'resnetb_light', 'inception_deformable',
                          'resnetb_light_strided', 'inception_deformable_strided', 'vgg',
                          'max_pool', 'max_pool_wide', 'global_average', 'simple_upsample', 'resnetb_upsample')
@@ -304,13 +347,21 @@
     F = []
     training = dropout_prob < 0.99
     block_in_layer = 0
-    for block in config.architecture:
+    global _NEXT_RESNETB
+    for i, block in enumerate(config.architecture):
         if any(tmp in block for tmp in ('pool', 'strided', 'upsample', 'global')):
             F += [features]
         if 'upsample' in block:
             break
-        with variable_scope('layer_{:d}/{:s}_{:d}'.format(layer, block.replace('_deformable', ''), block_in_layer)):
-            features = get_block_ops(block)(layer, inputs, features, r, fdim, config, training)
+        nxt = config.architecture[i + 1] if i + 1 < len(config.architecture) else ''
+        same_level = not ('pool' in block or 'strided' in block)
+        if same_level and nxt.startswith('resnetb') and not training:
+            _NEXT_RESNETB = (len(_vs()._scope), 'layer_{:d}/{:s}_{:d}'.format(layer, nxt.replace('_deformable', ''), block_in_layer + 1))
+        try:
+            with variable_scope('layer_{:d}/{:s}_{:d}'.format(layer, block.replace('_deformable', ''), block_in_layer)):
+                features = get_block_ops(block)(layer, inputs, features, r, fdim, config, training)
+        finally:
+            _NEXT_RESNETB = None
         block_in_layer += 1
         if 'pool' in block or 'strided' in block:
             layer += 1
diff --git a/d3feat_amd/ops.py b/d3feat_amd/ops.py
--- a/d3feat_amd/ops.py
+++ b/d3feat_amd/ops.py
@@ -746,6 +746,103 @@
     return _tag(out, A1)
 
 
+GEMM_CHAIN = os.environ.get("D3F_GEMM_CHAIN", "1") != "0"
+CHAIN_MIN_ROWS = None
+
+
+def packed_x3_chain_weights(W2):
+    lib = _lib.load()
+    return _packed_weights(W2, "_d3f_x3c", lambda K, N: torch.empty((int(lib.d3f_gemm_x3_packed_bytes(K, N)) // 2,), dtype=torch.int16,
+                                                                    device=W2.device), lib.d3f_gemm_pack_x3_chain, "gemm_pack_x3_chain")
+
+
+def gemm_chain_ok(M, N, K, store_first, hint=0):
+    if not (GEMM_CHAIN and GEMM_X3) or BF16_CONTRACTION or BF16_FEATURES or M > X3_MAX_ROWS:
+        return False
+    rows = hint if 0 < hint < M else M
+    if CHAIN_MIN_ROWS is not None and rows >= CHAIN_MIN_ROWS:
+        M, hint = max(M, 65536), 0
+    return bool(_lib.load().d3f_gemm_x3_chain_ok(M, N, K, 1 if store_first else 0, hint))
+
+
+def _chain_addressable(N, *operands):
+    for t, ld, cols in operands:
+        if t is not None and (t.dtype != torch.float32 or cols % 32 or ld % 4 or t.data_ptr() % 16):
+            return False
+    return N % 4 == 0
+
+
+def gemm_chain(A, W, W2, idx=None, skip=None, store_first=True, col_scale=None, col_shift=None, leaky=False, alpha=0.2,
+               col_scale2=None, col_shift2=None, leaky2=False, alpha2=0.2, out=None, out2=None):
+    lib = _lib.load()
+    A, lda = _rows(_req(A, torch.float32, "A"), "A")
+    W, _ = _rows(_req(W, torch.float32, "W"), "W")
+    W2, _ = _rows(_req(W2, torch.float32, "W2"), "W2")
+    C1, C2, lds, ldi = A.shape[1], 0, 0, 0
+    src = A
+    if idx is not None:
+        idx, ldi = _rows(_req(idx, torch.int32, "idx"), "idx")
+        src = idx
+    if skip is not None:
+        skip, lds = _rows(_req(skip, torch.float32, "skip"), "skip")
+        C2 = skip.shape[1]
+    M, K, N, dev = src.shape[0], C1 + C2, W.shape[1], A.device
+    if W.shape[0] != K or tuple(W2.shape) != (N, 32) or not (W.is_contiguous() and W2.is_contiguous()) or (skip is not None and skip.shape[0] != M):
+        raise ValueError("gemm_chain: operands %d + %d columns, W %s, W2 %s" % (C1, C2, tuple(W.shape), tuple(W2.shape)))
+    if not _chain_addressable(N, (A, lda, C1), (skip, lds, C2)):
+        raise ValueError("gemm_chain: operands must be float32, 16-byte aligned, with whole k-tiles of 32 columns")
+    for v, n, name in ((col_scale, N, "col_scale"), (col_shift, N, "col_shift"), (col_scale2, 32, "col_scale2"), (col_shift2, 32, "col_shift2")):
+        if v is not None and (_req(v, torch.float32, name).numel() != n or not v.is_contiguous() or v.data_ptr() % 16):
+            raise ValueError("gemm_chain: %s must be a contiguous, 16-byte aligned vector of %d" % (name, n))
+    Y, ldc = None, N
+    if store_first:
+        Y = torch.empty((M, N), dtype=torch.float32, device=dev) if out is None else out
+        Y, ldc = _rows(_req(Y, torch.float32, "out"), "out")
+        if tuple(Y.shape) != (M, N):
+            raise ValueError("gemm_chain: out must be [%d, %d]" % (M, N))
+    out2 = torch.empty((M, 32), dtype=torch.float32, device=dev) if out2 is None else out2
+    out2, ldc2 = _rows(_req(out2, torch.float32, "out2"), "out2")
+    if tuple(out2.shape) != (M, 32):
+        raise ValueError("gemm_chain: out2 must be [%d, 32]" % M)
+    Wp, W2p = packed_x3_weights(W), packed_x3_chain_weights(W2)
+    with _timed("gemm_x3r", dict(M=M, N=N, K=K), dev):
+        rc = lib.d3f_gemm_x3_chain(A.data_ptr(), A.shape[0], lda, C1, _ptr(idx), ldi, _ptr(skip), lds, C2, Wp.data_ptr(), _ptr(Y), ldc, M, N,
+                                   None, _ptr(col_scale), _ptr(col_shift), None, 0, 1 if leaky else 0, float(alpha), W2p.data_ptr(),
+                                   _ptr(col_scale2), _ptr(col_shift2), 1 if leaky2 else 0, float(alpha2), out2.data_ptr(), ldc2,
+                                   _nd(src), _nd(A), _stream(dev))
+    _lib.check(rc, "gemm_x3_chain")
+    return (_tag(Y, src) if Y is not None else None), _tag(out2, src)
+
+
+class PendingUnary(UpsampleCat):
+
+    def __init__(self, u, W, col_scale, col_shift, leaky, alpha):
+        self.u, self.W, self.col_scale, self.col_shift, self.leaky, self.alpha = u, W, col_scale, col_shift, leaky, alpha
+        self.shape = (u.shape[0], W.shape[1])
+        self.device = u.device
+        self.dtype = torch.float32
+        _tag(self, u.inds)
+
+    def materialize(self):
+        return gemm_upsample_cat(self.u, self.W, col_scale=self.col_scale, col_shift=self.col_shift, leaky=self.leaky, alpha=self.alpha)
+
+    def chain(self, W2):
+        u = self.u
+        return gemm_chain(u.x, self.W, W2, idx=u.inds, skip=u.skip, store_first=False, col_scale=self.col_scale,
+                          col_shift=self.col_shift, leaky=self.leaky, alpha=self.alpha)[1]
+
+
+def pending_unary_ok(u, N):
+    if not isinstance(u, UpsampleCat) or isinstance(u, PendingUnary) or u.x.dim() != 2 or u.inds.dim() != 2:
+        return False
+    C1, C2 = u.x.shape[1], (u.skip.shape[1] if u.skip is not None else 0)
+    if u.skip is not None and (u.skip.dim() != 2 or u.skip.stride(1) != 1):
+        return False
+    if u.x.stride(1) != 1 or u.inds.dtype != torch.int32 or not _chain_addressable(N, (u.x, u.x.stride(0), C1), (u.skip, u.skip.stride(0) if C2 else 0, C2)):
+        return False
+    return gemm_chain_ok(u.inds.shape[0], N, C1 + C2, False, int(getattr(u.inds, "n_hint", 0) or 0))
+
+
 def _kp_front(what, query_points, support_points, neighbors_indices, features, K_points, K_values, KP_extent, KP_influence,
               aggregation_mode, col_scale=None, col_shift=None, residual=None, leaky=False, alpha=0.2, row_pos=True, feat=_feat):
     lib = _lib.load()
@@ -888,6 +985,7 @@
 
 
 _PACKERS = (("_d3f_bf16t", packed_bf16_weights), ("_d3f_f32t", packed_f32t_weights), ("_d3f_x3", packed_x3_weights),
+            ("_d3f_x3c", packed_x3_chain_weights),
             ("_d3f_packed", packed_kpconv_weights), ("_d3f_packed_x3", packed_kpconv_weights_x3))
 
 
diff --git a/include/d3feat_amd.h b/include/d3feat_amd.h
--- a/include/d3feat_amd.h
+++ b/include/d3feat_amd.h
@@ -198,6 +198,14 @@
                      const int* res_rows_dev, int leaky, float alpha, void* workspace, size_t workspace_bytes, const int* M_dev,
                      const int* N1_dev, int M_hint, void* stream);
 
+int d3f_gemm_pack_x3_chain(const float* W2, int ldb, int K, int N, void* W2x, void* stream);
+int d3f_gemm_x3_chain_ok(int M, int N, int K, int store_first, int M_hint);
+int d3f_gemm_x3_chain(const float* A, int N1, int lda, int C1, const int* idx, int ld_idx, const float* skip, int lds, int C2cols,
+                      const void* Wx, float* C, int ldc, int M, int N, const float* row_scale, const float* col_scale,
+                      const float* col_shift, const float* residual, int ldr, int leaky, float alpha, const void* W2x,
+                      const float* col_scale2, const float* col_shift2, int leaky2, float alpha2, float* C2, int ldc2,
+                      const int* M_dev, const int* N1_dev, void* stream);
+
 size_t d3f_gemm_bf16_workspace_bytes(int M, int N, int K, int M_hint);
 int d3f_gemm_pack_bf16(const float* W, int ldb, int K, int N, void* W_packed, void* stream);
 int d3f_gemm_bf16(const void* A, int N1, int lda, int C1, const int* idx, int ld_idx, const void* skip, int lds, int C2,
```

After: 1982 fragments/s (median of 6 runs). 1.3% higher.
